# tobixdev/rdf-fusion

Hardware: AMD Instinct MI355X
Metric: solution bindings/sec + achieved HBM GB/s, BSBM Q5 at 1/2/4/8 GPUs (higher is better)
Workload: dtype u32 ids / i64 typed values; 1 GPU; BSBM-shaped store, 285000 products (98101452 triples), Explore Q5 (7 triple patterns -> scans, hash joins, FILTERs), 262144 instances per step, batched into one operator tree (shared scans); steady state: the join tables of the predicate slices are cached per store version (cold start and the no-cache step are under config.cold_start); mode=batched, triples_per_gpu=98100423, exchange_overlapped_with_next_step=False, bindings=56629082633

## Files before the change

include/rdfgpu.h:

```cpp
#ifndef RDFGPU_H
#define RDFGPU_H

#include <stddef.h>
#include <stdint.h>

#ifdef __cplusplus
extern "C" {
#endif

#define RDFGPU_ABI_VERSION 4u

typedef enum rdfgpu_status {
  RDFGPU_OK = 0,
  RDFGPU_END = 1,
  RDFGPU_ERR_INVALID = -1,
  RDFGPU_ERR_DEVICE = -2,
  RDFGPU_ERR_UNSUPPORTED = -3,
  RDFGPU_ERR_OOM = -4,
  RDFGPU_ERR_NO_DEVICE = -5
} rdfgpu_status;

const char* rdfgpu_last_error(void);
uint32_t rdfgpu_abi_version(void);

// ... 237 lines not shown
  uint32_t n_regexes;
  uint32_t reserved;
} rdfgpu_plan_desc;
#define RDFGPU_PLAN_ALLOW_OPAQUE 1u
#define RDFGPU_PLAN_AGG_COLUMNS 2u
#define RDFGPU_PLAN_VALUE_KEYS 4u

typedef struct rdfgpu_plan rdfgpu_plan;

typedef struct rdfgpu_metrics {
  uint64_t output_rows;
  uint64_t input_rows;
  uint64_t intermediate_rows;
  uint64_t device_bytes;
  double elapsed_compute_ms;
  uint32_t kernels_launched;
  uint32_t host_syncs;
  uint32_t exact_reruns;
  uint32_t device_mallocs;
  double device_malloc_ms;
  uint32_t tables_built;
  uint32_t reserved;
} rdfgpu_metrics;

int rdfgpu_plan_compile(rdfgpu_store* store, const rdfgpu_plan_desc* desc, rdfgpu_plan** out);
void rdfgpu_plan_destroy(rdfgpu_plan* plan);

int rdfgpu_plan_bind_table(rdfgpu_plan* plan, uint32_t slot, const uint32_t* const* cols,
                           uint32_t n_cols, uint64_t n_rows);

int rdfgpu_plan_execute(rdfgpu_plan* plan);

int rdfgpu_plan_result_info(rdfgpu_plan* plan, uint64_t* n_rows, uint32_t* n_cols);
int rdfgpu_plan_result_device(rdfgpu_plan* plan, const uint32_t** cols, uint32_t cap_cols);
int rdfgpu_plan_fetch(rdfgpu_plan* plan, uint32_t* const* host_cols, uint32_t n_cols);
typedef struct rdfgpu_agg_value {
  int64_t lo;
  int64_t hi;
  uint8_t tag;
  uint8_t reserved[7];
} rdfgpu_agg_value;
int rdfgpu_plan_agg_count(rdfgpu_plan* plan, uint32_t* n_aggs);
int rdfgpu_plan_agg_fetch(rdfgpu_plan* plan, uint32_t agg, rdfgpu_agg_value* host);
int rdfgpu_plan_agg_device(rdfgpu_plan* plan, uint32_t agg, const rdfgpu_agg_value** values);
int rdfgpu_plan_result_values(rdfgpu_plan* plan, uint32_t col, const rdfgpu_agg_value** values, uint64_t* n);
int rdfgpu_plan_result_values_fetch(rdfgpu_plan* plan, uint32_t col, rdfgpu_agg_value* host);
int rdfgpu_plan_next(rdfgpu_plan* plan, struct ArrowArray* out, struct ArrowSchema* schema);
int rdfgpu_plan_rewind(rdfgpu_plan* plan);
int rdfgpu_plan_metrics(rdfgpu_plan* plan, rdfgpu_metrics* out);
int rdfgpu_plan_selected_index(const rdfgpu_plan* plan, uint32_t node, uint32_t* components);
int rdfgpu_plan_stream(rdfgpu_plan* plan, void** hip_stream);
int rdfgpu_plan_decode_terms(rdfgpu_plan* plan, uint32_t col, uint64_t first_row, uint64_t n_rows,
                             struct ArrowArray* out, struct ArrowSchema* schema);

enum { RDFGPU_PUSH_UNSUPPORTED = 0,
       RDFGPU_PUSH_TRUE = 1,
       RDFGPU_PUSH_BINARY = 2,
       RDFGPU_PUSH_BETWEEN = 3 };
typedef struct rdfgpu_pushdown_filter {
  uint32_t kind;
  uint32_t var;
  uint32_t op;
  uint32_t value;
  uint32_t from, to;
} rdfgpu_pushdown_filter;
int rdfgpu_plan_pushdown_filters(rdfgpu_plan* plan, uint32_t node, const rdfgpu_pushdown_filter* filters, uint32_t n, uint8_t* pushed);
// ... 19 lines not shown
  RDFGPU_OPT_NO_FIRST_RUN_SPECULATION,
  RDFGPU_OPT_NO_STRING_VERDICTS,
  RDFGPU_OPT_NO_TABLE_CACHE,
  RDFGPU_OPT_NO_INDEX_JOIN,
  RDFGPU_OPT_NO_CHAIN_FUSION,
  RDFGPU_OPT_NO_VALUE_TABLES,
  RDFGPU_OPT_NO_RANGE_INDEX,
  RDFGPU_OPT_NO_FILTER_FUSION,
  RDFGPU_OPT_NO_LDS_JOIN,
  RDFGPU_OPT_NO_GLOBAL_TABLE_JOIN,
  RDFGPU_OPT_NO_DIRECT_TABLE,
  RDFGPU_OPT_NO_BAND_JOIN,
  RDFGPU_OPT_NO_PARTITIONED_JOIN,
  RDFGPU_OPT_NO_VALUE_VERDICTS,
  RDFGPU_OPT_NO_PRIMING,
  RDFGPU_OPT_NO_ORDERED_JOIN,
  RDFGPU_OPT_NO_BAND_PACK16,
  RDFGPU_OPT_NO_RUN_COPY,
  RDFGPU_OPT_NO_RANGE_PARTITION,
  RDFGPU_OPT_LDS_MAX_BUILD,
  RDFGPU_OPT_CSR_ROW_LANES_LOG2,
  RDFGPU_OPT_JOIN_WAVE_Q,
  RDFGPU_OPT_PARTITION_MIN_BUILD,
  RDFGPU_OPT_PARTITION_TWO_PASS_ROWS,
  RDFGPU_OPT_NO_OWN_PARTITION_PASS,
  RDFGPU_OPT_NO_BAND_COMPACT,
  RDFGPU_OPT_NO_PROBE_OUTER_JOIN,
  RDFGPU_OPT_NO_STREAM_JOIN,
  RDFGPU_OPT_PARTITION_ROWS,
  RDFGPU_OPT_PARTITION_SLOTS,
  RDFGPU_OPT_NO_SEMI_LDS,
  RDFGPU_OPT_NO_BAND_PAIR_COUNTS,
  RDFGPU_OPT_BAND_PAIR_COUNT_BLOCKS,
  RDFGPU_OPT_NO_BAND_ROW_CACHE,
  RDFGPU_OPT_NO_BAND_PAIR_LIST,
  RDFGPU_OPT_NO_BAND_PAIR_CACHE,
  RDFGPU_OPT_BAND_PAIR_CACHE_BLOCKS,
  RDFGPU_OPT_NO_AGG_LDS,
  RDFGPU_OPT__COUNT
};
int rdfgpu_store_set_option(rdfgpu_store* store, uint32_t option, uint64_t value);
int rdfgpu_store_get_option(const rdfgpu_store* store, uint32_t option, uint64_t* value);
int rdfgpu_plan_set_option(rdfgpu_plan* plan, uint32_t option, uint64_t value);
const char* rdfgpu_option_name(uint32_t option);

uint64_t rdfgpu_scan_score(const rdfgpu_scan_instruction instr[4]);
uint32_t rdfgpu_choose_index(const rdfgpu_scan_instruction gspo[4], uint32_t available);
int rdfgpu_band_row_cache_eligible(uint32_t in_place, uint32_t compact, uint32_t pack16, uint32_t option_set, uint32_t n_win,
                                   const uint32_t operand_src[4], const uint32_t operand_keyed_by_join_key[4]);
int rdfgpu_band_pair_cache_eligible(uint32_t row_windows, uint32_t neq_self, uint32_t pack16, uint32_t option_set, uint64_t n_blocks, uint64_t cap_blocks);
int rdfgpu_band_pair_list_eligible(uint32_t pair_cached, uint32_t option_set, uint64_t survivors, uint64_t n_blocks);
int rdfgpu_band_pair_count_eligible(uint32_t has_list, uint32_t option_set, uint64_t n_blocks, uint64_t min_blocks);
int rdfgpu_band_step_form(uint32_t row_static, uint32_t has_verdicts, uint32_t has_list, uint32_t list_option_set, uint32_t counts_option_set,
                          uint32_t n_row_cols, uint64_t n_blocks, uint64_t min_blocks);
int rdfgpu_oj_probe_form(uint32_t held, uint32_t in_place, uint32_t row_cache, uint32_t option_set, uint32_t row_static);
typedef struct rdfgpu_predicate {
  uint32_t pred;
  uint32_t from, to;
  const uint32_t* ids;
  uint32_t n_ids;
  uint32_t equal_to;
} rdfgpu_predicate;
int rdfgpu_predicate_and(const rdfgpu_predicate* lhs, const rdfgpu_predicate* rhs,
                         rdfgpu_predicate* out, uint32_t* out_ids);
enum { RDFGPU_OP_EQ = 0, RDFGPU_OP_GT = 1, RDFGPU_OP_GTEQ = 2, RDFGPU_OP_LT = 3, RDFGPU_OP_LTEQ = 4 };
int rdfgpu_pushdown_to_scan_predicate(uint32_t op, uint32_t value, rdfgpu_predicate* out);

int rdfgpu_regex_check(const char* pattern, uint32_t pattern_len, const char* flags, uint32_t flags_len, uint32_t* positions);

typedef struct rdfgpu_comm rdfgpu_comm;
#define RDFGPU_COMM_ID_BYTES 128
int rdfgpu_comm_unique_id(uint8_t id[RDFGPU_COMM_ID_BYTES]);
int rdfgpu_comm_create(const uint8_t id[RDFGPU_COMM_ID_BYTES], uint32_t rank, uint32_t world, int32_t device, rdfgpu_comm** out);
typedef int (*rdfgpu_host_alltoallv_fn)(void* ctx, const void* send, const uint64_t* send_bytes, void* recv, const uint64_t* recv_bytes);
int rdfgpu_comm_create_host(uint32_t rank, uint32_t world, int32_t device, rdfgpu_host_alltoallv_fn fn, void* ctx, rdfgpu_comm** out);
void rdfgpu_comm_destroy(rdfgpu_comm* comm);
int rdfgpu_exchange_allgatherv(rdfgpu_comm* comm, const uint32_t* const* cols, uint32_t n_cols, uint64_t n_rows,
                               const uint32_t** out_cols, uint64_t* out_rows);
int rdfgpu_exchange_repartition(rdfgpu_comm* comm, const uint32_t* const* cols, uint32_t n_cols, uint64_t n_rows, uint32_t key_col,
                                const uint32_t** out_cols, uint64_t* out_rows);
uint32_t rdfgpu_shard_of(uint32_t id, uint32_t world);

typedef struct rdfgpu_ntriples rdfgpu_ntriples;
int rdfgpu_ntriples_parse(int32_t device, const char* text, uint64_t text_bytes, uint32_t first_id, rdfgpu_ntriples** out);
int rdfgpu_ntriples_info(const rdfgpu_ntriples* nt, uint64_t* n_triples, uint32_t* n_terms, uint64_t* term_bytes);
int rdfgpu_ntriples_terms(const rdfgpu_ntriples* nt, uint64_t* offsets, uint8_t* bytes);
int rdfgpu_ntriples_decoded_info(const rdfgpu_ntriples* nt, uint64_t* lex_bytes, uint64_t* suffix_bytes);
int rdfgpu_ntriples_decoded(const rdfgpu_ntriples* nt, uint8_t* kind, uint64_t* lex_off, uint8_t* lex_bytes, uint64_t* suffix_off,
// ... 9 lines not shown
```

rdf-fusion_amd/__init__.py:

```python
from . import abi, plan
from .engine import (RdfGpuError, GpuQuadStore, GpuPlan, Comm, NTriples, load_library, library_path, kernel_source_sha16,
                     choose_index, scan_score, predicate_and, pushdown_to_scan_predicate, shard_of, band_row_cache_eligible,
                     band_pair_cache_eligible, band_pair_list_eligible, band_pair_count_eligible, band_step_form, BAND_FORMS, oj_probe_form, OJ_PROBE_FORMS)

__all__ = ["abi", "plan", "RdfGpuError", "GpuQuadStore", "GpuPlan", "Comm", "NTriples", "shard_of", "load_library", "library_path", "kernel_source_sha16",
           "choose_index", "scan_score", "predicate_and", "pushdown_to_scan_predicate", "band_row_cache_eligible", "band_pair_cache_eligible", "band_pair_list_eligible", "band_pair_count_eligible", "band_step_form", "BAND_FORMS", "oj_probe_form", "OJ_PROBE_FORMS"]
```

rdf-fusion_amd/abi.py:

```python
import ctypes as C

ABI_VERSION = 4

OK, END = 0, 1
ERR_INVALID, ERR_DEVICE, ERR_UNSUPPORTED, ERR_OOM, ERR_NO_DEVICE = -1, -2, -3, -4, -5

GSPO, GPOS, GOSP = 0, 1, 2
INDEX_NAMES = {GSPO: "GSPO", GPOS: "GPOS", GOSP: "GOSP"}

TRAVERSE, SCAN = 0, 1
PRED_NONE, PRED_FALSE, PRED_IN, PRED_BETWEEN, PRED_EQUAL_TO = 0, 1, 2, 3, 4

(TV_NULL, TV_NAMED_NODE, TV_BLANK_NODE, TV_STRING, TV_BOOLEAN, TV_FLOAT, TV_DOUBLE, TV_DECIMAL,
 TV_INT, TV_INTEGER, TV_DATE_TIME, TV_TIME, TV_DATE, TV_DURATION, TV_OTHER) = range(15)
TVF_EMPTY_STRING = 1
TVF_NEEDS_HOST = 0x80
NT_IRI, NT_BNODE, NT_SIMPLE, NT_LANG, NT_TYPED = 1, 2, 3, 4, 5

(EX_COLUMN, EX_LIT_ID, EX_LIT_TV, EX_ENC_TV, EX_GT, EX_LT, EX_GEQ, EX_LEQ, EX_EQ, EX_ADD, EX_SUB,
 EX_EBV, EX_ID_EQ, EX_ID_NEQ, EX_AND, EX_OR, EX_NOT, EX_IS_COMPATIBLE, EX_BOUND, EX_BOOL_AS_TV,
 EX_LIT_BOOL, EX_NEQ, EX_REGEX, EX_CONTAINS, EX_STRSTARTS, EX_STRENDS, EX_LANG_IN, EX_REGEX_VAR,
 EX_STR, EX_LIT_STR, EX_STRLEN, EX_SUBSTR, EX_UCASE, EX_LCASE, EX_STRBEFORE, EX_STRAFTER,
 EX_MUL, EX_DIV, EX_NEG, EX_PLUS, EX_ABS, EX_ROUND, EX_CEIL, EX_FLOOR, EX_CAST, EX_CAST_STRING, EX_CAST_LEX,
 EX_YEAR, EX_MONTH, EX_DAY, EX_HOURS, EX_MINUTES, EX_SECONDS) = range(1, 54)
# ... 2 lines not shown
CAST_TARGETS = (TV_BOOLEAN, TV_INT, TV_INTEGER, TV_DECIMAL, TV_FLOAT, TV_DOUBLE)

(NODE_DATA_SOURCE, NODE_FILTER, NODE_HASH_JOIN, NODE_CROSS_JOIN, NODE_NESTED_LOOP_JOIN,
 NODE_PROJECTION, NODE_TABLE, NODE_TOPK, NODE_UNION, NODE_CLOSURE, NODE_AGGREGATE) = range(1, 12)
NODE_SORT = 13
NODE_EXTEND = 12
(AGG_COUNT_STAR, AGG_COUNT, AGG_COUNT_DISTINCT, AGG_SUM, AGG_AVG, AGG_MIN, AGG_MAX, AGG_SAMPLE, AGG_GROUP_CONCAT,
 AGG_SUM_DISTINCT, AGG_AVG_DISTINCT, AGG_COUNT_DISTINCT_STAR) = range(1, 13)
AGG_NAMES = {AGG_COUNT_STAR: "COUNT(*)", AGG_COUNT: "COUNT", AGG_COUNT_DISTINCT: "COUNT(DISTINCT)", AGG_SUM: "SUM", AGG_AVG: "AVG",
             AGG_MIN: "MIN", AGG_MAX: "MAX", AGG_SAMPLE: "SAMPLE", AGG_GROUP_CONCAT: "GROUP_CONCAT", AGG_SUM_DISTINCT: "SUM(DISTINCT)",
             AGG_AVG_DISTINCT: "AVG(DISTINCT)", AGG_COUNT_DISTINCT_STAR: "COUNT(DISTINCT *)"}
MAX_AGGREGATES = 8
AGG_INPUT_EXPR = 0x80000000
SORT_BY_ID, SORT_BY_TERM, SORT_BY_DOUBLE = 0, 1, 2
SORT_BY_VALUE = 3
SORT_DESC = 0x100
JOIN_INNER, JOIN_LEFT, JOIN_LEFT_SEMI, JOIN_LEFT_ANTI = 0, 1, 2, 3
JOIN_LEFT_MARK = 4
MAX_KEYS = 4
MAX_GROUP_KEYS = 8
MAX_COLUMNS = 16
NO_PROJECTION = 0xFFFFFFFF
PLAN_ALLOW_OPAQUE = 1
PLAN_AGG_COLUMNS = 2

PLAN_VALUE_KEYS = 4

OP_EQ, OP_GT, OP_GTEQ, OP_LT, OP_LTEQ = range(5)

OPTION_NAMES = ["FORCE_GENERIC_VM", "NO_JOIN_REORDER", "NO_SPECULATION", "NO_FIRST_RUN_SPECULATION", "NO_STRING_VERDICTS",
                "NO_TABLE_CACHE", "NO_INDEX_JOIN", "NO_CHAIN_FUSION", "NO_VALUE_TABLES", "NO_RANGE_INDEX", "NO_FILTER_FUSION",
                "NO_LDS_JOIN", "NO_GLOBAL_TABLE_JOIN", "NO_DIRECT_TABLE", "NO_BAND_JOIN", "NO_PARTITIONED_JOIN", "NO_VALUE_VERDICTS", "NO_PRIMING", "NO_ORDERED_JOIN", "NO_BAND_PACK16", "NO_RUN_COPY", "NO_RANGE_PARTITION",
                "LDS_MAX_BUILD", "CSR_ROW_LANES_LOG2", "JOIN_WAVE_Q", "PARTITION_MIN_BUILD", "PARTITION_TWO_PASS_ROWS", "NO_OWN_PARTITION_PASS", "NO_BAND_COMPACT", "NO_PROBE_OUTER_JOIN", "NO_STREAM_JOIN", "PARTITION_ROWS", "PARTITION_SLOTS",
                "NO_SEMI_LDS", "NO_BAND_PAIR_COUNTS", "BAND_PAIR_COUNT_BLOCKS", "NO_BAND_ROW_CACHE", "NO_BAND_PAIR_LIST", "NO_BAND_PAIR_CACHE", "BAND_PAIR_CACHE_BLOCKS", "NO_AGG_LDS"]
OPTIONS = {name: i for i, name in enumerate(OPTION_NAMES)}


class Config(C.Structure):
    _fields_ = [("device", C.c_int32), ("batch_size", C.c_uint32), ("flags", C.c_uint32),
                ("reserved", C.c_uint32)]


class TypedValue(C.Structure):
    _fields_ = [("lo", C.c_int64), ("aux", C.c_uint32), ("tag", C.c_uint8), ("flags", C.c_uint8),
                ("tz_minutes", C.c_int16)]


class AggValue(C.Structure):
    _fields_ = [("lo", C.c_int64), ("hi", C.c_int64), ("tag", C.c_uint8), ("reserved", C.c_uint8 * 7)]


class ScanInstruction(C.Structure):
    _fields_ = [("kind", C.c_uint8), ("pred", C.c_uint8), ("reserved", C.c_uint16),
                ("var", C.c_uint32), ("a", C.c_uint32), ("b", C.c_uint32)]


class ExprNode(C.Structure):
    _fields_ = [("op", C.c_uint8), ("tag", C.c_uint8), ("flags", C.c_uint8), ("reserved", C.c_uint8),
                ("u", C.c_uint32), ("lo", C.c_int64), ("hi", C.c_int64)]


class PlanNode(C.Structure):
    _fields_ = [("kind", C.c_uint32), ("left", C.c_int32), ("right", C.c_int32),
                ("join_type", C.c_uint32), ("scan", ScanInstruction * 4), ("n_keys", C.c_uint32),
                ("left_keys", C.c_uint32 * MAX_KEYS), ("right_keys", C.c_uint32 * MAX_KEYS),
                ("expr_off", C.c_uint32), ("expr_len", C.c_uint32), ("proj_off", C.c_uint32),
                ("n_proj", C.c_uint32), ("table_slot", C.c_uint32), ("table_cols", C.c_uint32)]
# ... 46 lines not shown
    ("n_children", C.c_int64), ("children", C.POINTER(C.POINTER(ArrowSchema))),
    ("dictionary", C.POINTER(ArrowSchema)), ("release", C.c_void_p), ("private_data", C.c_void_p)]


class ArrowArray(C.Structure):
    pass


ArrowArray._fields_ = [
    ("length", C.c_int64), ("null_count", C.c_int64), ("offset", C.c_int64), ("n_buffers", C.c_int64),
    ("n_children", C.c_int64), ("buffers", C.POINTER(C.c_void_p)),
    ("children", C.POINTER(C.POINTER(ArrowArray))), ("dictionary", C.POINTER(ArrowArray)),
    ("release", C.c_void_p), ("private_data", C.c_void_p)]

assert C.sizeof(TypedValue) == 16
assert C.sizeof(ScanInstruction) == 16
assert C.sizeof(ExprNode) == 24
assert C.sizeof(AggValue) == 24

EXPORTED_SYMBOLS = [
    "rdfgpu_last_error", "rdfgpu_abi_version",
    "rdfgpu_store_create", "rdfgpu_store_destroy", "rdfgpu_store_extend", "rdfgpu_store_extend_device",
    "rdfgpu_store_remove", "rdfgpu_store_clear", "rdfgpu_store_drop_tables", "rdfgpu_store_remove_graph", "rdfgpu_store_len", "rdfgpu_store_set_typed_values", "rdfgpu_store_set_strings",
    "rdfgpu_store_read_index",
    "rdfgpu_plan_compile", "rdfgpu_plan_destroy", "rdfgpu_plan_bind_table", "rdfgpu_plan_execute",
    "rdfgpu_plan_result_info", "rdfgpu_plan_result_device", "rdfgpu_plan_fetch", "rdfgpu_plan_next",
    "rdfgpu_plan_agg_count", "rdfgpu_plan_agg_fetch", "rdfgpu_plan_agg_device",
    "rdfgpu_plan_result_values", "rdfgpu_plan_result_values_fetch",
    "rdfgpu_plan_rewind", "rdfgpu_plan_decode_terms", "rdfgpu_ntriples_parse", "rdfgpu_ntriples_info", "rdfgpu_ntriples_terms", "rdfgpu_ntriples_decoded_info", "rdfgpu_ntriples_decoded", "rdfgpu_ntriples_columns", "rdfgpu_ntriples_destroy", "rdfgpu_plan_metrics", "rdfgpu_plan_selected_index", "rdfgpu_plan_stream",
    "rdfgpu_plan_enable_kernel_timing", "rdfgpu_plan_kernel_stats",
    "rdfgpu_plan_pushdown_filters", "rdfgpu_plan_set_dynamic_filters", "rdfgpu_plan_source_predicate",
    "rdfgpu_store_set_option", "rdfgpu_store_get_option", "rdfgpu_plan_set_option", "rdfgpu_option_name",
    "rdfgpu_scan_score", "rdfgpu_choose_index", "rdfgpu_predicate_and", "rdfgpu_band_row_cache_eligible", "rdfgpu_band_pair_cache_eligible", "rdfgpu_band_pair_list_eligible", "rdfgpu_band_pair_count_eligible", "rdfgpu_band_step_form", "rdfgpu_oj_probe_form",
    "rdfgpu_pushdown_to_scan_predicate", "rdfgpu_regex_check",
    "rdfgpu_comm_unique_id", "rdfgpu_comm_create", "rdfgpu_comm_create_host", "rdfgpu_comm_destroy",
    "rdfgpu_exchange_allgatherv", "rdfgpu_exchange_repartition", "rdfgpu_shard_of",
]
COMM_ID_BYTES = 128
HOST_ALLTOALLV_FN = C.CFUNCTYPE(C.c_int, C.c_void_p, C.c_void_p, C.POINTER(C.c_uint64), C.c_void_p, C.POINTER(C.c_uint64))
```

rdf-fusion_amd/csrc/abi.cpp:

```cpp
#include <cstdlib>
#include <cstring>
#include <mutex>
#include <shared_mutex>
#include <string>

#include "exchange.hpp"
#include "host_logic.hpp"
#include "ntriples.hpp"
#include "plan.hpp"
#include "regex_compile.hpp"
#include "store.hpp"

namespace rdfgpu {
static thread_local std::string g_last_error;
void set_last_error(const std::string& msg) { g_last_error = msg; }
}

using namespace rdfgpu;

#define ABI_BEGIN try {
#define ABI_END                                              \
  }                                                          \
  catch (const Error& e) { set_last_error(e.what()); return e.status; } \
  catch (const std::bad_alloc&) { set_last_error("host allocation failed"); return RDFGPU_ERR_OOM; } \
// ... 101 lines not shown
  P(plan)->opt.v[option] = value;
  ABI_END
}
const char* rdfgpu_option_name(uint32_t option) { return engine_option_name(option); }

int rdfgpu_plan_compile(rdfgpu_store* store, const rdfgpu_plan_desc* desc, rdfgpu_plan** out) {
  ABI_BEGIN
  if (!out) fail(RDFGPU_ERR_INVALID, "null out pointer");
  *out = reinterpret_cast<rdfgpu_plan*>(plan_compile(S(store), desc));
  ABI_END
}
void rdfgpu_plan_destroy(rdfgpu_plan* plan) { delete reinterpret_cast<Plan*>(plan); }

int rdfgpu_plan_bind_table(rdfgpu_plan* plan, uint32_t slot, const uint32_t* const* cols, uint32_t n_cols, uint64_t n_rows) {
  ABI_BEGIN
  Plan* p = P(plan);
  if (slot >= p->tables.size()) fail(RDFGPU_ERR_INVALID, "plan has no table slot %u", slot);
  if (n_cols && !cols) fail(RDFGPU_ERR_INVALID, "null column array");
  BoundTable& b = p->tables[slot];
  b.cols.assign(cols, cols + n_cols);
  b.n_rows = n_rows; b.bound = true;
  ABI_END
}
int rdfgpu_plan_execute(rdfgpu_plan* plan) { ABI_BEGIN P(plan)->execute(); ABI_END }

int rdfgpu_plan_result_info(rdfgpu_plan* plan, uint64_t* n_rows, uint32_t* n_cols) {
  ABI_BEGIN
  Plan* p = P(plan);
  if (!p->executed) fail(RDFGPU_ERR_INVALID, "plan has not been executed");
  if (n_rows) *n_rows = p->result_rows;
  if (n_cols) *n_cols = p->result.n_cols;
  ABI_END
}
int rdfgpu_plan_result_device(rdfgpu_plan* plan, const uint32_t** cols, uint32_t cap_cols) {
  ABI_BEGIN
  Plan* p = P(plan);
  if (!p->executed) fail(RDFGPU_ERR_INVALID, "plan has not been executed");
  if (cap_cols < p->result.n_cols) fail(RDFGPU_ERR_INVALID, "room for %u columns, result has %u", cap_cols, p->result.n_cols);
  for (u32 c = 0; c < p->result.n_cols; c++) cols[c] = p->result_rows ? p->result.cols[c] : nullptr;
  ABI_END
}
int rdfgpu_plan_fetch(rdfgpu_plan* plan, uint32_t* const* host_cols, uint32_t n_cols) {
  ABI_BEGIN
  Plan* p = P(plan);
  if (!p->executed) fail(RDFGPU_ERR_INVALID, "plan has not been executed");
  if (n_cols != p->result.n_cols) fail(RDFGPU_ERR_INVALID, "caller passed %u columns, result has %u", n_cols, p->result.n_cols);
  p->store->activate();
  for (u32 c = 0; c < n_cols; c++)
    if (p->result_rows) RDFGPU_HIP(hipMemcpyAsync(host_cols[c], p->result.cols[c], p->result_rows * 4, hipMemcpyDeviceToHost, p->stream));
  RDFGPU_HIP(hipStreamSynchronize(p->stream));
  ABI_END
}

int rdfgpu_plan_agg_count(rdfgpu_plan* plan, uint32_t* n_aggs) {
  ABI_BEGIN
  Plan* p = P(plan);
  if (!p->executed) fail(RDFGPU_ERR_INVALID, "plan has not been executed");
  if (n_aggs) *n_aggs = (uint32_t)p->agg_out.size();
  ABI_END
}
int rdfgpu_plan_agg_fetch(rdfgpu_plan* plan, uint32_t agg, rdfgpu_agg_value* host) {
  ABI_BEGIN
  Plan* p = P(plan);
  if (!p->executed) fail(RDFGPU_ERR_INVALID, "plan has not been executed");
  if (agg >= p->agg_out.size()) fail(RDFGPU_ERR_INVALID, "aggregate %u of %zu", agg, p->agg_out.size());
  p->store->activate();
  if (p->result_rows) {
    if (!host) fail(RDFGPU_ERR_INVALID, "null host buffer");
    RDFGPU_HIP(hipMemcpyAsync(host, p->agg_out[agg], p->result_rows * sizeof(rdfgpu_agg_value), hipMemcpyDeviceToHost, p->stream));
  }
  RDFGPU_HIP(hipStreamSynchronize(p->stream));
  ABI_END
}
int rdfgpu_plan_result_values(rdfgpu_plan* plan, uint32_t col, const rdfgpu_agg_value** values, uint64_t* n) {
  ABI_BEGIN
  Plan* p = P(plan);
  if (!p->executed) fail(RDFGPU_ERR_INVALID, "plan has not been executed");
  if (col >= p->result.n_cols) fail(RDFGPU_ERR_INVALID, "column %u of a %u-column result", col, p->result.n_cols);
  if (!values) fail(RDFGPU_ERR_INVALID, "null out pointer");
  *values = p->result_values(col, n);
  ABI_END
}
int rdfgpu_plan_result_values_fetch(rdfgpu_plan* plan, uint32_t col, rdfgpu_agg_value* host) {
  ABI_BEGIN
  Plan* p = P(plan);
  if (!p->executed) fail(RDFGPU_ERR_INVALID, "plan has not been executed");
  if (col >= p->result.n_cols) fail(RDFGPU_ERR_INVALID, "column %u of a %u-column result", col, p->result.n_cols);
  if (!p->result_values(col, nullptr)) fail(RDFGPU_ERR_INVALID, "result column %u holds object ids, not aggregate values", col);
  p->ensure_host_copy();
  if (p->result_rows) {
    if (!host) fail(RDFGPU_ERR_INVALID, "null host buffer");
    std::memcpy(host, p->host_values[col].data(), p->result_rows * sizeof(rdfgpu_agg_value));
  }
  ABI_END
}
int rdfgpu_plan_agg_device(rdfgpu_plan* plan, uint32_t agg, const rdfgpu_agg_value** values) {
  ABI_BEGIN
  Plan* p = P(plan);
  if (!p->executed) fail(RDFGPU_ERR_INVALID, "plan has not been executed");
  if (agg >= p->agg_out.size()) fail(RDFGPU_ERR_INVALID, "aggregate %u of %zu", agg, p->agg_out.size());
  if (!values) fail(RDFGPU_ERR_INVALID, "null out pointer");
  *values = p->result_rows ? p->agg_out[agg] : nullptr;
  ABI_END
}

namespace {
struct ChildPriv { void* buffers[3] = {nullptr, nullptr, nullptr}; };
void release_child_array(struct ArrowArray* a) {
  if (!a || !a->release) return;
  ChildPriv* pr = static_cast<ChildPriv*>(a->private_data);
  std::free(pr->buffers[0]); std::free(pr->buffers[1]); std::free(pr->buffers[2]);
  delete pr;
  a->release = nullptr;
}
struct StructPriv { const void* buffers[1]; struct ArrowArray** children; u32 n; };
void release_struct_array(struct ArrowArray* a);
void release_agg_array(struct ArrowArray* a) {
  if (!a || !a->release) return;
  std::free(const_cast<void*>(static_cast<StructPriv*>(a->private_data)->buffers[0]));
  static_cast<StructPriv*>(a->private_data)->buffers[0] = nullptr;
  release_struct_array(a);
}
void release_struct_array(struct ArrowArray* a) {
  if (!a || !a->release) return;
  StructPriv* pr = static_cast<StructPriv*>(a->private_data);
  for (u32 i = 0; i < pr->n; i++) { if (pr->children[i]->release) pr->children[i]->release(pr->children[i]); delete pr->children[i]; }
  delete[] pr->children;
  delete pr;
  a->release = nullptr;
}
struct SchemaPriv { struct ArrowSchema** children; u32 n; std::string* names; };
void release_schema(struct ArrowSchema* s) {
// ... 92 lines not shown
      ch->release = release_child_array; ch->private_data = cp;
      sp->children[c] = ch;
    }
    std::memset(out, 0, sizeof *out);
    out->length = (int64_t)len; out->n_buffers = 1; out->buffers = sp->buffers;
    out->n_children = nc; out->children = sp->children;
    out->release = release_struct_array; out->private_data = sp;
    if (schema) {
      std::memset(schema, 0, sizeof *schema);
      SchemaPriv* pr = new SchemaPriv();
      pr->n = nc; pr->children = new ArrowSchema*[nc ? nc : 1]; pr->names = new std::string[nc ? nc : 1];
      for (u32 c = 0; c < nc; c++) {
        pr->names[c] = "c" + std::to_string(c);
        if (c >= nk || p->result_values(c, nullptr)) { pr->children[c] = agg_schema(pr->names[c].c_str()); continue; }
        ArrowSchema* cs = new ArrowSchema();
        std::memset(cs, 0, sizeof *cs);
        cs->format = "I"; cs->name = pr->names[c].c_str(); cs->flags = 2 ;
        cs->release = release_schema; cs->private_data = nullptr;
        pr->children[c] = cs;
      }
      schema->format = "+s"; schema->name = ""; schema->n_children = nc; schema->children = pr->children;
      schema->release = release_schema; schema->private_data = pr;
    }
    p->cursor += len;
    return RDFGPU_OK;
  } catch (const Error& e) { set_last_error(e.what()); return e.status; }
  catch (const std::exception& e) { set_last_error(e.what()); return RDFGPU_ERR_INVALID; }
}
int rdfgpu_plan_decode_terms(rdfgpu_plan* plan, uint32_t col, uint64_t first_row, uint64_t n_rows, struct ArrowArray* out, struct ArrowSchema* schema) {
  try {
    Plan* p = P(plan);
    if (!out) fail(RDFGPU_ERR_INVALID, "null out array");
    if (!p->executed) fail(RDFGPU_ERR_INVALID, "plan has not been executed");
    if (col >= p->result.n_cols) fail(RDFGPU_ERR_INVALID, "column %u of a %u-column result", col, p->result.n_cols);
    if (const ValueOrigin& o = p->nodes[p->root].origin[col]; o.node >= 0)
      fail(RDFGPU_ERR_UNSUPPORTED, "ENC_PT of result column %u: it is %s value column (%s %u of node %d), its entries are not object ids (rdfgpu_plan_result_values)", col, o.mark ? "a mark" : o.extend ? "a computed" : "an aggregate", o.mark ? "mark" : o.extend ? "expression" : "aggregate", o.agg, o.node);
    if (first_row > p->result_rows || n_rows > p->result_rows - first_row) fail(RDFGPU_ERR_INVALID, "rows %llu .. + %llu of a %llu-row result", (unsigned long long)first_row, (unsigned long long)n_rows, (unsigned long long)p->result_rows);
    Store* st = p->store;
    st->activate();
    std::shared_lock<std::shared_mutex> lock(st->mu);
    if (!st->str_off) fail(RDFGPU_ERR_INVALID, "ENC_PT needs the lexical forms (rdfgpu_store_set_strings)");
    const u64 n = n_rows;
    hipStream_t s = p->stream;
    DevicePool& pool = st->pool;
    std::vector<void*> dev;
    auto dalloc = [&](size_t bytes) { void* q = pool.alloc(bytes ? bytes : 4); dev.push_back(q); return q; };
    struct Guard { DevicePool& pool; std::vector<void*>& v; ~Guard() { for (void* q : v) pool.free(q); } } guard{pool, dev};
    DecodeArgs a{};
    a.ids = p->result.cols[col] + first_row; a.n = n; a.tt = st->typed_table();
    u32* len = static_cast<u32*>(dalloc((n + 1) * 4)); u32* off = static_cast<u32*>(dalloc((n + 1) * 4));
    a.len = len; a.off = off;
    a.term_type = static_cast<unsigned char*>(dalloc(n)); a.tag = static_cast<unsigned char*>(dalloc(n)); a.aux = static_cast<u32*>(dalloc(n * 4));
    RDFGPU_HIP(hipMemsetAsync(len + n, 0, 4, s));
    launch_decode_lengths(a, s);
    std::vector<u32> h_len(n + 1);
    RDFGPU_HIP(hipMemcpyAsync(h_len.data(), len, (n + 1) * 4, hipMemcpyDeviceToHost, s));
    RDFGPU_HIP(hipStreamSynchronize(s));
    u64 total = 0;
    for (u64 i = 0; i < n; i++) total += h_len[i];
    if (total > 0x7FFFFFFFull) fail(RDFGPU_ERR_UNSUPPORTED, "ENC_PT: %llu bytes of lexical forms in one call (utf8 offsets are int32): decode fewer rows", (unsigned long long)total);
    const size_t tb = scan_temp_bytes(n + 1);
    void* temp = dalloc(tb);
    exclusive_scan_u32(len, off, n + 1, temp, tb, s);
    a.bytes = static_cast<unsigned char*>(dalloc(total));
    launch_decode_bytes(a, s);
    auto halloc = [](size_t bytes) { void* q = std::malloc(bytes ? bytes : 1); if (!q) fail(RDFGPU_ERR_OOM, "host allocation of %zu bytes failed", bytes); return q; };
// ... 24 lines not shown
      return ch;
    };
    sp->children[0] = child(h_tt, nullptr, 2);
    sp->children[1] = child(h_off, h_bytes, 3);
    sp->children[2] = child(h_tag, nullptr, 2);
    sp->children[3] = child(h_aux, nullptr, 2);
    static_cast<ChildPriv*>(sp->children[0]->private_data)->buffers[2] = valid;
    sp->buffers[0] = nulls ? valid : nullptr;
    std::memset(out, 0, sizeof *out);
    out->length = (int64_t)n; out->null_count = nulls; out->n_buffers = 1; out->buffers = sp->buffers;
    out->n_children = 4; out->children = sp->children;
    out->release = release_struct_array; out->private_data = sp;
    if (schema) {
      std::memset(schema, 0, sizeof *schema);
      SchemaPriv* pr = new SchemaPriv();
      pr->n = 4; pr->children = new ArrowSchema*[4]; pr->names = new std::string[4];
      const char* names[4] = {"term_type", "value", "tag", "aux"};
      const char* formats[4] = {"C", "u", "C", "I"};
      for (u32 c = 0; c < 4; c++) {
        ArrowSchema* cs = new ArrowSchema();
        std::memset(cs, 0, sizeof *cs);
        pr->names[c] = names[c];
        cs->format = formats[c]; cs->name = pr->names[c].c_str(); cs->flags = 0;
        cs->release = release_schema; cs->private_data = nullptr;
        pr->children[c] = cs;
      }
      schema->format = "+s"; schema->name = ""; schema->flags = 2 ; schema->n_children = 4; schema->children = pr->children;
      schema->release = release_schema; schema->private_data = pr;
    }
    return RDFGPU_OK;
  } catch (const Error& e) { set_last_error(e.what()); return e.status; }
  catch (const std::exception& e) { set_last_error(e.what()); return RDFGPU_ERR_INVALID; }
}
int rdfgpu_plan_rewind(rdfgpu_plan* plan) { ABI_BEGIN P(plan)->cursor = 0; ABI_END }
int rdfgpu_plan_metrics(rdfgpu_plan* plan, rdfgpu_metrics* out) {
  ABI_BEGIN
  if (!out) fail(RDFGPU_ERR_INVALID, "null out pointer");
  *out = P(plan)->metrics;
  ABI_END
}
int rdfgpu_plan_selected_index(const rdfgpu_plan* plan, uint32_t node, uint32_t* components) {
  ABI_BEGIN
  const Plan* p = reinterpret_cast<const Plan*>(plan);
  if (!p) fail(RDFGPU_ERR_INVALID, "null plan handle");
  if (node >= p->nodes.size() || p->nodes[node].source < 0) fail(RDFGPU_ERR_INVALID, "node %u is not a data source", node);
  if (components) *components = p->sources[p->nodes[node].source].components;
  ABI_END
}
int rdfgpu_plan_pushdown_filters(rdfgpu_plan* plan, uint32_t node, const rdfgpu_pushdown_filter* filters, uint32_t n, uint8_t* pushed) {
  ABI_BEGIN
  if (n && !filters) fail(RDFGPU_ERR_INVALID, "null filter array");
  P(plan)->pushdown_filters(node, filters, n, pushed);
  ABI_END
}
int rdfgpu_plan_set_dynamic_filters(rdfgpu_plan* plan, uint32_t node, const rdfgpu_pushdown_filter* filters, uint32_t n) {
  ABI_BEGIN
  if (n && !filters) fail(RDFGPU_ERR_INVALID, "null filter array");
  P(plan)->set_dynamic_filters(node, filters, n);
  ABI_END
}
int rdfgpu_plan_source_predicate(const rdfgpu_plan* plan, uint32_t node, uint32_t level, rdfgpu_predicate* pred) {
  ABI_BEGIN
  const Plan* p = reinterpret_cast<const Plan*>(plan);
  if (!p || !pred) fail(RDFGPU_ERR_INVALID, "null pointer");
  if (node >= p->nodes.size() || p->nodes[node].source < 0 || level > 3) fail(RDFGPU_ERR_INVALID, "node %u level %u is not a data-source level", node, level);
  const SourceInfo& src = p->sources[p->nodes[node].source];
  ScanPredicate sp;
  for (int k = 0; k < 4; k++) if ((u32)PERM[src.components][k] == level) sp = src.ix.in[k].pred;
  std::memset(pred, 0, sizeof *pred);
  pred->pred = sp.kind; pred->from = sp.from; pred->to = sp.to; pred->equal_to = sp.equal_to;
  if (sp.kind == RDFGPU_PRED_IN) { pred->n_ids = (u32)sp.ids.size(); if (sp.ids.size() == 1) pred->from = pred->to = sp.ids[0]; }
  ABI_END
}
int rdfgpu_plan_stream(rdfgpu_plan* plan, void** hip_stream) {
  ABI_BEGIN
  if (!hip_stream) fail(RDFGPU_ERR_INVALID, "null out pointer");
  *hip_stream = P(plan)->stream;
  ABI_END
}

int rdfgpu_plan_enable_kernel_timing(rdfgpu_plan* plan, int on) {
  ABI_BEGIN
  Plan* p = P(plan);
  p->timing = on != 0;
  p->timing_focus = on >= 2 ? p->last_top_kc : -1;
  ABI_END
}
int rdfgpu_plan_kernel_stats(rdfgpu_plan* plan, rdfgpu_kernel_stat* out, uint32_t cap, uint32_t* n) {
  ABI_BEGIN
  Plan* p = P(plan);
  if (!n || (cap && !out)) fail(RDFGPU_ERR_INVALID, "null out pointer");
  u32 w = 0;
  for (int k = 0; k < KC__N; k++) {
    const KernelStat& s = p->kstats[k];
    if (!s.launches) continue;
    if (w < cap) { out[w].kernel = kernel_class_name(k); out[w].launches = s.launches; out[w].reserved = 0; out[w].total_ms = s.ms; out[w].algorithmic_bytes = s.bytes; out[w].rows_in = s.rows; }
    w++;
  }
  *n = w < cap ? w : cap;
  ABI_END
}

static void decode4(const rdfgpu_scan_instruction raw[4], ScanInstruction out[4]) {
  for (int i = 0; i < 4; i++) {
    rdfgpu_scan_instruction r = raw[i];
    if (r.pred == RDFGPU_PRED_IN) {
      out[i].kind = r.kind; out[i].var = r.var; out[i].pred.kind = RDFGPU_PRED_IN;
      out[i].pred.ids.clear();
      for (u32 q = 0; q < (r.b ? r.b : 1); q++) out[i].pred.ids.push_back(q);
    } else out[i] = decode_instruction(r, nullptr, 0);
  }
}
uint64_t rdfgpu_scan_score(const rdfgpu_scan_instruction instr[4]) {
  try { ScanInstruction in[4]; decode4(instr, in); return scan_score(in); }
  catch (const std::exception& e) { set_last_error(e.what()); return 0; }
}
uint32_t rdfgpu_choose_index(const rdfgpu_scan_instruction gspo[4], uint32_t available) {
  try {
    ScanInstructions g; g.components = RDFGPU_GSPO; decode4(gspo, g.in);
    return choose_index(g, available);
  } catch (const std::exception& e) { set_last_error(e.what()); return 0xFFFFFFFFu; }
}
int rdfgpu_band_row_cache_eligible(uint32_t in_place, uint32_t compact, uint32_t pack16, uint32_t option_set, uint32_t n_win,
// ... 5 lines not shown
    for (u32 w = 0; w < n_win; w++) {
      s.y0[w] = BandRowOperandShape{operand_src[2 * w], operand_keyed_by_join_key[2 * w] != 0};
      s.y1[w] = BandRowOperandShape{operand_src[2 * w + 1], operand_keyed_by_join_key[2 * w + 1] != 0};
    }
    return band_row_cache_eligible(s) ? 1 : 0;
  } catch (const Error& e) { set_last_error(e.what()); return e.status; }
}
int rdfgpu_band_pair_cache_eligible(uint32_t row_windows, uint32_t neq_self, uint32_t pack16, uint32_t option_set, uint64_t n_blocks, uint64_t cap_blocks) {
  BandPairCacheShape s;
  s.row_windows = row_windows != 0; s.neq_self = neq_self != 0; s.pack16 = pack16 != 0; s.option_off = option_set == 0; s.n_blocks = n_blocks; s.cap = cap_blocks;
  return band_pair_cache_eligible(s) ? 1 : 0;
}
int rdfgpu_band_pair_list_eligible(uint32_t pair_cached, uint32_t option_set, uint64_t survivors, uint64_t n_blocks) {
  BandPairListShape s;
  s.pair_cached = pair_cached != 0; s.option_off = option_set == 0; s.survivors = survivors; s.n_blocks = n_blocks;
  return band_pair_list_eligible(s) ? 1 : 0;
}
int rdfgpu_band_pair_count_eligible(uint32_t has_list, uint32_t option_set, uint64_t n_blocks, uint64_t min_blocks) {
  BandPairCountShape s;
  s.has_list = has_list != 0; s.option_off = option_set == 0; s.n_blocks = n_blocks; s.min_blocks = min_blocks;
  return band_pair_count_eligible(s) ? 1 : 0;
}
int rdfgpu_band_step_form(uint32_t row_static, uint32_t has_verdicts, uint32_t has_list, uint32_t list_option_set, uint32_t counts_option_set,
                          uint32_t n_row_cols, uint64_t n_blocks, uint64_t min_blocks) {
  BandStepShape s;
  s.row_static = row_static != 0; s.has_verdicts = has_verdicts != 0; s.has_list = has_list != 0; s.list_option_off = list_option_set == 0;
  s.counts_option_off = counts_option_set == 0; s.n_row_cols = n_row_cols; s.n_blocks = n_blocks; s.min_blocks = min_blocks;
  return (int)band_step_form(s);
}
int rdfgpu_oj_probe_form(uint32_t held, uint32_t in_place, uint32_t row_cache, uint32_t option_set, uint32_t row_static) {
  OjProbeShape s;
  s.held = held != 0; s.in_place = in_place != 0; s.row_cache = row_cache != 0; s.option_off = option_set == 0; s.row_static = row_static != 0;
  return (int)oj_probe_form(s);
}
static ScanPredicate from_abi(const rdfgpu_predicate* p) {
  ScanPredicate r; r.kind = p->pred; r.from = p->from; r.to = p->to; r.equal_to = p->equal_to;
  if (p->pred == RDFGPU_PRED_IN) { if (p->ids) r.ids.assign(p->ids, p->ids + p->n_ids); else r.ids = {p->from}; }
  return r;
}
int rdfgpu_predicate_and(const rdfgpu_predicate* lhs, const rdfgpu_predicate* rhs, rdfgpu_predicate* out, uint32_t* out_ids) {
  try {
    if (!lhs || !rhs || !out) fail(RDFGPU_ERR_INVALID, "null predicate");
    ScanPredicate r;
    if (!predicate_and(from_abi(lhs), from_abi(rhs), &r)) return 0;
    std::memset(out, 0, sizeof *out);
    out->pred = r.kind; out->from = r.from; out->to = r.to;
    if (r.kind == RDFGPU_PRED_IN) {
      if (!out_ids) fail(RDFGPU_ERR_INVALID, "null out_ids");
      for (size_t i = 0; i < r.ids.size(); i++) out_ids[i] = r.ids[i];
      out->ids = out_ids; out->n_ids = (u32)r.ids.size();
    }
    return 1;
  } catch (const Error& e) { set_last_error(e.what()); return e.status; }
}
int rdfgpu_pushdown_to_scan_predicate(uint32_t op, uint32_t value, rdfgpu_predicate* out) {
  try {
    if (!out) fail(RDFGPU_ERR_INVALID, "null out predicate");
    const ScanPredicate r = pushdown_to_scan_predicate(op, value);
    std::memset(out, 0, sizeof *out);
    out->pred = r.kind; out->from = r.from; out->to = r.to;
    if (r.kind == RDFGPU_PRED_IN) { out->from = out->to = r.ids[0]; out->n_ids = 1; }
    return 1;
  } catch (const Error& e) { set_last_error(e.what()); return e.status; }
}

static Comm* CM(rdfgpu_comm* c) { if (!c) fail(RDFGPU_ERR_INVALID, "null communicator"); return reinterpret_cast<Comm*>(c); }
// ... 95 lines not shown
```

rdf-fusion_amd/csrc/band_join.hip:

```cpp
#include <hip/hip_runtime.h>
#include <cstring>
#include <rocprim/rocprim.hpp>

#include "join_device.hpp"

namespace rdfgpu {

static inline dim3 grid256(u64 n) { const u64 g = (n + 255) / 256; return dim3((unsigned)(g ? g : 1)); }
constexpr u32 kBandInvalidLo = 0xFFFFFFFFu;

__global__ __launch_bounds__(256) void band_bounds_kernel(const u32* skey_sorted, u64 n, u32 kn, u32* poff) {
  const u64 i = (u64)blockIdx.x * blockDim.x + threadIdx.x;
  if (i > n) return;
  const u32 prev = i > 0 ? skey_sorted[i - 1] + 1u : 0u;
  const u32 cur = i < n ? skey_sorted[i] : kn;
  for (u32 k = prev; k <= cur && k <= kn; k++) poff[k] = (u32)i;
}

__device__ __forceinline__ bool band_window_of(const TypedTable& tt, const BandWin& w, u32 iy0, u32 iy1, long long& lo, long long& hi) {
  lo = INT64_MIN + 1; hi = INT64_MAX;
  if (tt.n_ids == 0 || iy0 == 0 || iy1 == 0 || iy0 >= tt.n_ids || iy1 >= tt.n_ids) return false;
  if (w.l0.tag != RDFGPU_TV_INTEGER || w.l1.tag != RDFGPU_TV_INTEGER) return false;
  const int4* tv = reinterpret_cast<const int4*>(tt.tv);
  const int4 r0 = tv[iy0];
// ... 863 lines not shown
    case 6: hipLaunchKernelGGL((band_emit_kernel<FORM, 6>), g, dim3(256), 0, s, b); return true;
  }
  return false;
}
static bool launch_band_emit_list(const BandArgs& b, dim3 g, hipStream_t s) {
  constexpr BandForm L = BandForm::VERDICTS_LIST;
  switch (b.n_out_cols * 2 + b.n_row_cols) {
    case 3: hipLaunchKernelGGL((band_emit_kernel<L, 1, 1>), g, dim3(256), 0, s, b); return true;
    case 5: hipLaunchKernelGGL((band_emit_kernel<L, 2, 2>), g, dim3(256), 0, s, b); return true;
    case 7: hipLaunchKernelGGL((band_emit_kernel<L, 3, 3>), g, dim3(256), 0, s, b); return true;
    case 9: hipLaunchKernelGGL((band_emit_kernel<L, 4, 4>), g, dim3(256), 0, s, b); return true;
    case 11: hipLaunchKernelGGL((band_emit_kernel<L, 5, 5>), g, dim3(256), 0, s, b); return true;
    case 2: hipLaunchKernelGGL((band_emit_kernel<L, 1, 2>), g, dim3(256), 0, s, b); return true;
    case 4: hipLaunchKernelGGL((band_emit_kernel<L, 2, 3>), g, dim3(256), 0, s, b); return true;
    case 6: hipLaunchKernelGGL((band_emit_kernel<L, 3, 4>), g, dim3(256), 0, s, b); return true;
    case 8: hipLaunchKernelGGL((band_emit_kernel<L, 4, 5>), g, dim3(256), 0, s, b); return true;
  }
  return false;
}
void launch_band_emit(const BandArgs& b, BandForm form, hipStream_t s) {
  band_form_check(b, form);
  const dim3 g = grid_waves(b.launch_blocks);
  bool launched = false;
  switch (form) {
    case BandForm::RECORDS: launched = launch_band_emit_cols<BandForm::RECORDS>(b, g, s); break;
    case BandForm::ROW_WINDOWS: launched = launch_band_emit_cols<BandForm::ROW_WINDOWS>(b, g, s); break;
    case BandForm::VERDICTS: launched = launch_band_emit_cols<BandForm::VERDICTS>(b, g, s); break;
    case BandForm::VERDICTS_LIST: case BandForm::COUNTS_LIST:
      launched = launch_band_emit_list(b, grid_waves((b.max_blocks + kBandEmitGroup - 1) / kBandEmitGroup), s); break;
  }
  if (!launched) fail(RDFGPU_ERR_INVALID, "band join: form %s with %u output columns (%u from the row)", band_form_name(form), b.n_out_cols, b.n_row_cols);
}

struct BandBlocksOfKey {
  const u32* csr_off; const u32* poff; u32 kn;
  __host__ __device__ u32 operator()(u32 k) const {
    if (k >= kn) return 0u;
    const u32 e = csr_off[k + 1] - csr_off[k], r = poff[k + 1] - poff[k];
    return (e && r) ? ((e + 63) >> 6) * ((r + 63) >> 6) : 0u;
  }
  __device__ __forceinline__ uint4 group(u32 g, u32 n) const {
    const u32 k = 4u * g;
    if (k + 4u <= kn && !((reinterpret_cast<uintptr_t>(csr_off) | reinterpret_cast<uintptr_t>(poff)) & 15u)) {
      const uint4 c = reinterpret_cast<const uint4*>(csr_off)[g], p = reinterpret_cast<const uint4*>(poff)[g];
      const u32 c4 = csr_off[k + 4u], p4 = poff[k + 4u];
      auto blocks = [](u32 e, u32 r) { return (e && r) ? ((e + 63u) >> 6) * ((r + 63u) >> 6) : 0u; };
      return make_uint4(blocks(c.y - c.x, p.y - p.x), blocks(c.z - c.y, p.z - p.y), blocks(c.w - c.z, p.w - p.z), blocks(c4 - c.w, p4 - p.w));
    }
    return make_uint4(k < n ? (*this)(k) : 0u, k + 1u < n ? (*this)(k + 1u) : 0u, k + 2u < n ? (*this)(k + 2u) : 0u, k + 3u < n ? (*this)(k + 3u) : 0u);
  }
};
size_t band_blocks_scan_temp_bytes(u32 kn) {
  size_t bytes = 0;
  auto in = rocprim::make_transform_iterator(rocprim::make_counting_iterator<u32>(0u), BandBlocksOfKey{nullptr, nullptr, kn});
  (void)rocprim::exclusive_scan(nullptr, bytes, in, (u32*)nullptr, 0u, (size_t)kn + 1, rocprim::plus<u32>());
  return bytes + 256;
}
void band_blocks_scan(const u32* csr_off, const u32* poff, u32 kn, u32* boff, void* temp, size_t temp_bytes, hipStream_t s) {
  if (launch_small_scan<false>(BandBlocksOfKey{csr_off, poff, kn}, boff, (u64)kn + 1, s)) return;
  auto in = rocprim::make_transform_iterator(rocprim::make_counting_iterator<u32>(0u), BandBlocksOfKey{csr_off, poff, kn});
  RDFGPU_HIP(rocprim::exclusive_scan(temp, temp_bytes, in, boff, 0u, (size_t)kn + 1, rocprim::plus<u32>(), s));
}

size_t sort_u32_temp_bytes(u64 n, u32 bits) {
  size_t bytes = 0;
  (void)rocprim::radix_sort_pairs(nullptr, bytes, (const u32*)nullptr, (u32*)nullptr, (const u32*)nullptr, (u32*)nullptr, (size_t)(n ? n : 1), 0, bits);
// ... 37 lines not shown
```

rdf-fusion_amd/csrc/host_logic.cpp:

```cpp
#include "host_logic.hpp"

#include <algorithm>

namespace rdfgpu {

ScanInstruction decode_instruction(const rdfgpu_scan_instruction& raw, const u32* pool, u32 n_pool) {
  ScanInstruction out;
  if (raw.kind != RDFGPU_TRAVERSE && raw.kind != RDFGPU_SCAN) fail(RDFGPU_ERR_INVALID, "scan instruction: bad kind %u", raw.kind);
  out.kind = raw.kind;
  out.var = raw.var;
  out.pred.kind = raw.pred;
  switch (raw.pred) {
    case RDFGPU_PRED_NONE: case RDFGPU_PRED_FALSE: break;
    case RDFGPU_PRED_IN:
      if (raw.b == 0) fail(RDFGPU_ERR_INVALID, "scan instruction: empty In set");
      if ((u64)raw.a + raw.b > n_pool) fail(RDFGPU_ERR_INVALID, "scan instruction: In set outside the pool");
      out.pred.ids.assign(pool + raw.a, pool + raw.a + raw.b);
      std::sort(out.pred.ids.begin(), out.pred.ids.end());
      out.pred.ids.erase(std::unique(out.pred.ids.begin(), out.pred.ids.end()), out.pred.ids.end());
      break;
    case RDFGPU_PRED_BETWEEN: out.pred.from = raw.a; out.pred.to = raw.b; break;
    case RDFGPU_PRED_EQUAL_TO: out.pred.equal_to = raw.a; break;
    default: fail(RDFGPU_ERR_INVALID, "scan instruction: bad predicate %u", raw.pred);
  }
// ... 126 lines not shown
      if (op->src < 2 || !op->stage_keyed_by_join_key) return false;
  return true;
}

bool band_pair_cache_eligible(const BandPairCacheShape& s) {
  if (!s.row_windows || !s.neq_self || !s.pack16 || !s.option_off) return false;
  return s.n_blocks <= (s.cap ? s.cap : kBandPairCacheBlocks);
}

bool band_pair_list_eligible(const BandPairListShape& s) {
  if (!s.pair_cached || !s.option_off || s.n_blocks >= kBandPairListBlocks) return false;
  return s.survivors <= 256 * s.n_blocks;
}

bool band_pair_count_eligible(const BandPairCountShape& s) {
  if (!s.has_list || !s.option_off) return false;
  return s.n_blocks >= (s.min_blocks ? s.min_blocks : kBandPairCountBlocks);
}

BandForm band_step_form(const BandStepShape& s) {
  if (!s.row_static) return BandForm::RECORDS;
  if (!s.has_verdicts) return BandForm::ROW_WINDOWS;
  if (!s.has_list || !s.list_option_off || s.n_row_cols > 1) return BandForm::VERDICTS;
  BandPairCountShape c;
  c.has_list = true; c.option_off = s.counts_option_off; c.n_blocks = s.n_blocks; c.min_blocks = s.min_blocks;
  return band_pair_count_eligible(c) ? BandForm::COUNTS_LIST : BandForm::VERDICTS_LIST;
}

OjProbeForm oj_probe_form(const OjProbeShape& s) {
  if (!s.held || !s.in_place || !s.row_cache || !s.option_off) return OjProbeForm::FULL;
  return s.row_static ? OjProbeForm::LEAN : OjProbeForm::FULL_NOW;
}

}
```

rdf-fusion_amd/csrc/host_logic.hpp:

```cpp
#pragma once
#include <vector>

#include "common.hpp"

namespace rdfgpu {

struct ScanPredicate {
  u32 kind = RDFGPU_PRED_NONE;
  std::vector<u32> ids;
  u32 from = 0, to = 0;
  u32 equal_to = 0;
};
struct ScanInstruction {
  u32 kind = RDFGPU_TRAVERSE;
  u32 var = 0;
  ScanPredicate pred;
};
struct ScanInstructions {
  u32 components = RDFGPU_GSPO;
  ScanInstruction in[4];
};

ScanInstruction decode_instruction(const rdfgpu_scan_instruction& raw, const u32* pool, u32 n_pool);
ScanInstructions make_gspo(const rdfgpu_scan_instruction raw[4], const u32* pool, u32 n_pool);
// ... 11 lines not shown
PrunePlan plan_pruning(const ScanInstructions& ix);

struct BandRowOperandShape { u32 src = 0; bool stage_keyed_by_join_key = false; };
struct BandRowCacheShape {
  bool in_place = false, compact = false, pack16 = false, option_off = false;
  u32 n_win = 0; BandRowOperandShape y0[2], y1[2];
};
bool band_row_cache_eligible(const BandRowCacheShape& s);
constexpr u64 kBandPairCacheBlocks = 1ull << 21;
struct BandPairCacheShape { bool row_windows = false, neq_self = false, pack16 = false, option_off = false; u64 n_blocks = 0, cap = 0; };
bool band_pair_cache_eligible(const BandPairCacheShape& s);
constexpr u64 kBandPairListBlocks = 1ull << 20;
struct BandPairListShape { bool pair_cached = false, option_off = false; u64 survivors = 0, n_blocks = 0; };
bool band_pair_list_eligible(const BandPairListShape& s);
constexpr u64 kBandPairCountBlocks = 1ull << 16;
struct BandPairCountShape { bool has_list = false, option_off = false; u64 n_blocks = 0, min_blocks = 0; };
bool band_pair_count_eligible(const BandPairCountShape& s);

enum class BandForm : u32 { RECORDS, ROW_WINDOWS, VERDICTS, VERDICTS_LIST, COUNTS_LIST };
constexpr const char* band_form_name(BandForm f) {
  return f == BandForm::RECORDS ? "RECORDS" : f == BandForm::ROW_WINDOWS ? "ROW_WINDOWS" : f == BandForm::VERDICTS ? "VERDICTS" : f == BandForm::VERDICTS_LIST ? "VERDICTS_LIST" : "COUNTS_LIST";
}
struct BandStepShape {
  bool row_static = false, has_verdicts = false, has_list = false, list_option_off = false, counts_option_off = false;
  u32 n_row_cols = 0; u64 n_blocks = 0, min_blocks = 0;
};
BandForm band_step_form(const BandStepShape& s);

enum class OjProbeForm : u32 { FULL, LEAN, FULL_NOW };
constexpr const char* oj_probe_form_name(OjProbeForm f) { return f == OjProbeForm::FULL ? "FULL" : f == OjProbeForm::LEAN ? "LEAN" : "FULL_NOW"; }
struct OjProbeShape { bool held = false, in_place = false, row_cache = false, option_off = false, row_static = false; };
OjProbeForm oj_probe_form(const OjProbeShape& s);

}
```

rdf-fusion_amd/csrc/kernels.hpp:

```cpp
#pragma once
#include <functional>
#include "common.hpp"
#include "expr_device.hpp"
#include "host_logic.hpp"

namespace rdfgpu {

constexpr u32 kNil = 0xFFFFFFFFu;
constexpr int kMaxCols = RDFGPU_MAX_COLUMNS;

struct DevTable {
  u32 n_cols = 0;
  const u32* cols[kMaxCols] = {};
  u64 cap = 0;
  const u64* n_dev = nullptr;
  u64 stable_id = 0;
  int sorted_col = -1;
  u32 key_min = 0, key_max = 0;
};

struct LocateJob {
  const u32* col[4];
  u64 n;
  u32 n_levels;
// ... 424 lines not shown
  ColRef entry_col[kBandMaxSideCols]; const u32* row_col[kBandMaxSideCols];
  u8 out_from_row[kMaxCols];
  u8 out_sel[kMaxCols];
  const uint2* row_win; const u32* row_val;
  u64* bvalid;
  const unsigned short* pair_list; const u32* pair_list_off;
  const unsigned char* pair_cnt;
};
struct BandPairListArgs { const u64* bits; u32 n_blocks; u32* counts; const u32* off; unsigned short* list; u64 cap; u32* total_out; unsigned char* pair_cnt; };
void launch_band_pair_list_count(const BandPairListArgs& a, hipStream_t s);
void launch_band_pair_list_write(const BandPairListArgs& a, hipStream_t s);
struct BandRowOperand { const u32* direct; u32 kmin, kn; const u32* val; };
struct BandRowWinArgs {
  BandRowOperand y0[2], y1[2];
  u32 kmin, kn; uint2* by_key;
  u32* slow_keys;
  const u32* build_key; u64 n_rows; uint2* row_win;
};
void launch_band_row_win_keys(const BandArgs& b, const BandRowWinArgs& w, hipStream_t s);
void launch_band_row_win_rows(const BandRowWinArgs& w, hipStream_t s);
void launch_band_pair_bits(const BandArgs& b, hipStream_t s);
void launch_band_pt(const BandArgs& b, hipStream_t s);
void launch_band_entries(const BandArgs& b, hipStream_t s);
void launch_band_rows(const BandArgs& b, hipStream_t s);
void launch_band_scatter(const BandArgs& b, hipStream_t s);
void launch_band_desc(const BandArgs& b, hipStream_t s);
void launch_band_decode(const BandArgs& b, hipStream_t s);
void launch_band_bounds(const u32* skey_sorted, u64 n, u32 kn, u32* poff, hipStream_t s);
size_t band_blocks_scan_temp_bytes(u32 kn);
void band_blocks_scan(const u32* csr_off, const u32* poff, u32 kn, u32* boff, void* temp, size_t temp_bytes, hipStream_t s);
void launch_band_mask(const BandArgs& b, BandForm form, hipStream_t s);
void launch_band_slow(const LdsJoinArgs* a_dev, const BandArgs& b, hipStream_t s);
void launch_band_emit(const BandArgs& b, BandForm form, hipStream_t s);
size_t sort_u32_temp_bytes(u64 n, u32 bits);
void sort_pairs_u32_u32(const u32* kin, u32* kout, const u32* vin, u32* vout, u64 n, u32 bits, void* temp, size_t temp_bytes, hipStream_t s);
void launch_val_minmax(const long long* val, u64 n, long long* out_minmax , hipStream_t s);
void launch_csr_max_group(const u32* off, u32 kn, u32* out_dev , hipStream_t s);
void launch_gjoin_build(const LdsJoinArgs& a, hipStream_t s);
int lds_join_items(u64 n_probe_cap, bool global);
enum { kJoinTableLds = 0, kJoinTableHash = 1, kJoinTableDirect = 2, kJoinTableCsr = 3 };
int lds_join_mode(const LdsJoinArgs& a);
void launch_minmax_u32(const u32* col, u64 n, u32* out_dev , hipStream_t s);
void launch_direct_values(const u32* keys, const u32* valcol, u64 n, u32 kmin, u32 kn, const TypedTable& tt, long long* val, u32* bad_dev, hipStream_t s);
void launch_fill_i64(long long* p, long long v, u64 n, hipStream_t s);
void launch_range_minmax(const u32* stage_key_col, const u32* csr_rows, u64 n, const long long* val, u32 vmin_key, u32 vn, long long* out_minmax , hipStream_t s);
void launch_range_keys(const u32* group_col, u32 gmin, const u32* stage_key_col, const u32* csr_rows, u64 n, const long long* val, u32 vmin_key, u32 vn,
                       long long vbase, u64* key64, u32* rows_in, hipStream_t s);
void launch_range_decode(const u64* key64_sorted, u64 n, u32* biased_vals_out, hipStream_t s);
void launch_gdirect_build(const u32* keys, u64 n, u32* direct , u32 kmin, u32 kn, u32* dup_dev, hipStream_t s);

struct TopkArgs {
  const u32* in[kMaxCols];
  const u64* n_in_dev; u64 n_in_cap;
  u32 has_group, group_col;
  u32 n_keys, key_col[4], key_by_term[4];
  u32 k, n_groups;
  TypedTable tt;
  u32* counts;
  u32* offsets;
  u32* cursor;
  u32* perm;
  u32* picked;
  u32* out_counts;
  u32* out_offsets;
  u32* out[kMaxCols]; u32 n_out_cols; u32 proj[kMaxCols];
  u64* n_out_dev;
// ... 50 lines not shown
```

rdf-fusion_amd/csrc/plan.cpp:

```cpp
#include "plan_exec.hpp"

#include <functional>

namespace rdfgpu {

void Plan::derive_source(SourceInfo& src, const ScanInstructions& gspo) {
  src.components = choose_index(gspo, 0b111);
  src.ix = reorder(gspo, src.components);
  src.prune = plan_pruning(src.ix);
  src.n_out = 0; src.has_residual = false;
  for (int k = 0; k < 4; k++) {
    if (gspo.in[k].kind != RDFGPU_SCAN) continue;
    bool first = true;
    for (int j = 0; j < k; j++) if (gspo.in[j].kind == RDFGPU_SCAN && gspo.in[j].var == gspo.in[k].var) first = false;
    if (!first) continue;
    for (int lvl = 0; lvl < 4; lvl++)
      if (src.ix.in[lvl].kind == RDFGPU_SCAN && src.ix.in[lvl].var == gspo.in[k].var) src.out_level[src.n_out] = lvl;
    src.n_out++;
  }
  for (int k = 0; k < 4; k++)
    if (src.ix.in[k].pred.kind != RDFGPU_PRED_NONE && !(src.prune.dropped_mask & (1u << k))) src.has_residual = true;
}
void Plan::upload_pool() {
  pool.clear();
// ... 43 lines not shown
    const bool yes = filters[i].kind != RDFGPU_PUSH_UNSUPPORTED;
    if (pushed) pushed[i] = yes ? 1 : 0;
    if (!yes) continue;
    any = true;
    ScanPredicate p;
    if (filter_to_predicate(filters[i], &p)) and_into_instructions(gspo, filters[i].var, p);
  }
  if (!any) return;
  src.gspo = gspo;
  derive_source(src, src.gspo);
  src.dynamic_dirty = !src.dynamic.empty();
  upload_pool();
  located_version = ~0ull;
  for (NodeInfo& nd : nodes) { nd.has_last = false; nd.last_rows = 0; }
}

void Plan::set_dynamic_filters(u32 node, const rdfgpu_pushdown_filter* filters, u32 n) {
  if (node >= nodes.size() || nodes[node].source < 0) fail(RDFGPU_ERR_INVALID, "node %u is not a data source", node);
  SourceInfo& src = sources[nodes[node].source];
  std::vector<std::pair<u32, ScanPredicate>> dyn;
  for (u32 i = 0; i < n; i++) {
    if (filters[i].kind == RDFGPU_PUSH_UNSUPPORTED) continue;
    ScanPredicate p;
    if (filter_to_predicate(filters[i], &p)) dyn.emplace_back(filters[i].var, p);
  }
  ScanInstructions probe = src.gspo;
  for (auto& d : dyn) and_into_instructions(probe, d.first, d.second);
  src.dynamic = dyn;
  src.dynamic_dirty = true;
}

Plan::~Plan() {
  if (store) (void)hipSetDevice(store->device);
  if (stream) (void)hipStreamSynchronize(stream);
  release_intermediates();
  if (pool_dev) (void)hipFree(pool_dev);
  if (regex_dev) (void)hipFree(regex_dev);
  if (str_consts_dev) (void)hipFree(str_consts_dev);
  if (mark_values_dev) (void)hipFree(mark_values_dev);

  if (store && ctx) store->release_context(ctx);
  if (store) store->release();
}

const char* kernel_class_name(int kc) {
  static const char* const fixed[KC_LDS_JOIN0] = {
      "rdfgpu::locate_kernel", "rdfgpu::scan_count_kernel", "rdfgpu::scan_write_kernel",
      "void rdfgpu::filter_kernel<1>", "void rdfgpu::filter_kernel<2>", "void rdfgpu::filter_kernel<0>",
      "rdfgpu::cross_kernel", "rdfgpu::join_build_kernel", "void rdfgpu::join_probe_kernel<false>",
      "void rdfgpu::join_probe_kernel<true>", "rdfgpu::join_left_unmatched_kernel", "void rdfgpu::nlj_kernel<false>",
      "void rdfgpu::nlj_kernel<true>", "rocprim device scan", "rdfgpu::gjoin_build_kernel", "rdfgpu::gdirect_build_kernel",
      "rdfgpu::minmax_u32_kernel", "rdfgpu::csr_rel_keys_kernel", "rocprim radix sort (CSR rows)",
      "rdfgpu::topk_max_kernel", "rdfgpu::topk_hist_kernel", "rdfgpu::topk_scatter_kernel", "rdfgpu::topk_select_kernel",
      "rdfgpu::topk_write_kernel", "void rdfgpu::filter_kernel<3>", "rdfgpu::regex_verdict_kernel", "rdfgpu::union_kernel",
      "rdfgpu::band_slow_kernel", "rocprim radix sort", "rdfgpu::band_bounds_kernel", "rdfgpu::band_blocks_kernel",
      "rdfgpu::band_decode_kernel", "void rdfgpu::band_mask_kernel", "void rdfgpu::band_emit_kernel", "rdfgpu::band_entries_kernel",
      "rdfgpu::band_desc_kernel", "rdfgpu::band_pt_kernel", "rdfgpu::band_rows_kernel",
      "void rdfgpu::filter_bits_kernel<1>", "void rdfgpu::filter_bits_kernel<2>", "void rdfgpu::filter_bits_kernel<3>", "void rdfgpu::filter_bits_kernel<4>", "rdfgpu::value_verdict_kernel",
      "rdfgpu::value_runs_kernel", "void rdfgpu::run_scan_kernel", "rdfgpu::run_copy_kernel",
      "rdfgpu::oj_probe_kernel", "rdfgpu::oj_count_kernel", "void rdfgpu::oj_write_kernel",
      "void rdfgpu::filter_write_kernel", "rdfgpu::part_keys_kernel", "void rdfgpu::part_join_kernel",
      "rdfgpu::oj_band_records_kernel", "rdfgpu::oj_write_band_kernel", "void rdfgpu::small_scan_kernel",
      "rdfgpu::part_pass (hist + scan + scatter)", "void rdfgpu::stream_join_kernel",
      "rdfgpu::oj_write_band_kernel(rdfgpu::OrderedJoinArgs, rdfgpu::OjBandFuse, rdfgpu::OjInPlace)", "void rdfgpu::semi_build_kernel",
      "void rdfgpu::semi_join_kernel<0, false", "void rdfgpu::semi_join_kernel<0, true", "void rdfgpu::semi_join_kernel<1, false",
      "void rdfgpu::semi_join_kernel<1, true", "void rdfgpu::semi_nested_kernel<false", "void rdfgpu::semi_nested_kernel<true",
      "rdfgpu::agg_groups_kernel", "void rdfgpu::agg_accum_kernel<false>", "void rdfgpu::agg_accum_kernel<true>", "rdfgpu::agg_final_kernel",
// ... 18 lines not shown
                                                       items[w] + ", " + std::to_string(m) + ", " + (c ? "true" : "false");
  });
  return names[kc - KC_LDS_JOIN0].c_str();
}

void Plan::resolve_timing() {
  for (KernelStat& k : kstats) k = KernelStat{};
  if (!timing) return;
  auto live = [&](const u64* dev, u64 fallback) -> u64 {
    if (!dev) return fallback;
    const u64 v = ctx->counters_host[dev - counters];
    return v < fallback || fallback == 0 ? v : fallback;
  };
  for (const PendingLaunch& p : pending) {
    float ms = 0;
    RDFGPU_HIP(hipEventElapsedTime(&ms, p.start, p.stop));
    KernelStat& k = kstats[p.kc];
    const u64 rows = live(p.rows_dev, p.rows_cap);
    const u64 out = p.out_dev ? ctx->counters_host[p.out_dev - counters] : p.out_rows;
    k.launches++; k.ms += ms; k.rows += rows;
    k.bytes += p.fixed_bytes + rows * p.bytes_per_row + out * p.bytes_per_out;
  }
  pending.clear();
  if (timing_focus < 0) {
    double top = 0;
    for (int kc = 0; kc < (int)(sizeof kstats / sizeof kstats[0]); kc++) if (kstats[kc].ms > top) { top = kstats[kc].ms; last_top_kc = kc; }
  }
}

void Plan::release_intermediates() {
  for (void* p : allocs) store->pool.free(p);
  allocs.clear();
}
const ExprProgram* Plan::upload_program(const ExprProgram& p) {
  if (progs_used >= ExecContext::kProgSlots) fail(RDFGPU_ERR_UNSUPPORTED, "plan needs more than %u device expression programs", ExecContext::kProgSlots);
  const u32 slot = progs_used++;
  ctx->progs_host[slot] = p;
  bind_values(ctx->progs_host[slot]);
  RDFGPU_HIP(hipMemcpyAsync(ctx->progs_dev + slot, ctx->progs_host + slot, sizeof(ExprProgram), hipMemcpyHostToDevice, stream));
  return ctx->progs_dev + slot;
}
void Plan::bind_values(ExprProgram& p) const {
  if (!agg_columns) return;
  for (u32 i = 0; i < p.n; i++) {
    rdfgpu_expr_node& e = p.nodes[i];
    if (e.op != kExAggValue) continue;
    const u32 node = e.u >> 8, agg = e.u & 0xffu;
    if (node >= nodes.size() || nodes[node].values_run != run) fail(RDFGPU_ERR_INVALID, "a value column of node %u is read before the node ran", node);
    e.lo = (int64_t)reinterpret_cast<uintptr_t>(nodes[node].values[agg]);
    e.hi = (int64_t)nodes[node].n_values;
  }
}
const rdfgpu_agg_value* Plan::result_values(u32 col, u64* n) const {
  const ValueOrigin& o = nodes[root].origin[col];
  if (n) *n = o.node < 0 ? 0 : nodes[o.node].n_values;
  return o.node < 0 ? nullptr : nodes[o.node].values[o.agg];
}
u64* Plan::new_counter() {
  if (counters_used >= 255) fail(RDFGPU_ERR_UNSUPPORTED, "plan needs more than 255 cardinality counters");
  return counters + counters_used++;
}
void Plan::read_back(void* host, const void* dev, size_t bytes) {
  RDFGPU_HIP(hipMemcpyAsync(host, dev, bytes, hipMemcpyDeviceToHost, stream));
  RDFGPU_HIP(hipStreamSynchronize(stream));
  metrics.host_syncs++;
}
// ... 20 lines not shown
    if (nd.d.kind == RDFGPU_NODE_TABLE) d = true;
    else if (nd.d.kind != RDFGPU_NODE_DATA_SOURCE) {
      const bool binary = is_binary(nd.d.kind);
      if (nd.d.left >= 0) d = depends((u32)nd.d.left);
      if (binary && nd.d.right >= 0) d = depends((u32)nd.d.right) || d;
    }
    dep[i] = d ? 1 : 0;
    return d;
  };
  const u64 ratio = (full + kPrimeRows - 1) / kPrimeRows;
  for (u32 i = 0; i < nodes.size(); i++) {
    NodeInfo& nd = nodes[i];
    if (nd.has_last && depends(i)) { nd.last_rows = nd.last_rows * ratio + 1024; nd.last_scaled = true; }
  }
}

bool Plan::record_band_history() {
  bool missed = false;
  for (const BandFeedback& f : band_feedback) {
    BandHistory& h = f.node->band;
    h.ran = true; h.blocks = f.known_blocks ? f.known_blocks : ctx->counters_host[f.blocks];
    h.slow_rows = ctx->counters_host[f.slow_rows] & 0xFFFFFFFFull; h.run_stats = ctx->counters_host[f.run_stats];
    if (f.slow_skipped && h.slow_rows) missed = true;
    if (f.multi_rows >= 0) h.multi_rows = ctx->counters_host[f.multi_rows] & 0xFFFFFFFFull;
    if (f.multi_rows >= 0 && f.in_place && h.multi_rows) missed = true;
  }
  return missed;
}

void Plan::execute() {
  if (!primed && !priming) prime();
  store->activate();
  std::shared_lock<std::shared_mutex> lock(store->mu);
  RDFGPU_HIP(hipStreamSynchronize(stream));
  release_intermediates();
  store->pool.trim_to(2 * std::max(std::max(scratch_hist[0], scratch_hist[1]), std::max(store->scratch_recent[0].load(), store->scratch_recent[1].load())) + (1ull << 30));
  held = store->gen;
  metrics = rdfgpu_metrics{};
  const u64 mallocs0 = store->pool.mallocs() + store->table_pool.mallocs();
  const double malloc_ms0 = store->pool.malloc_ms() + store->table_pool.malloc_ms();
  run++;
  counters_used = 0;
  progs_used = 0;
  arg_slots_used = 0;
  events_used = 2;
  pending.clear();
  host_valid = false; cursor = 0; executed = false;
  agg_out.clear();
  const hipEvent_t ev_start = ctx->event(0), ev_stop = ctx->event(1);
  RDFGPU_HIP(hipEventRecord(ev_start, stream));
  RDFGPU_HIP(hipMemsetAsync(counters, 0, 256 * sizeof(u64), stream));

  spec_checks.clear();
  pending_oj.active = false;
  band_feedback.clear();
  memo.assign(nodes.size(), DevTable{}); memo_valid.assign(nodes.size(), 0);
  speculative = allow_speculation && !opt.on(RDFGPU_OPT_NO_SPECULATION);

  refresh_dynamic_sources(lock);
  locate_sources();

  result = exec_node(root);
  flush_pending_oj();
  RDFGPU_HIP(hipMemcpyAsync(ctx->counters_host, counters, 256 * sizeof(u64), hipMemcpyDeviceToHost, stream));
  RDFGPU_HIP(hipEventRecord(ev_stop, stream));
  RDFGPU_HIP(hipStreamSynchronize(stream)); metrics.host_syncs++;
  RDFGPU_HIP(hipGetLastError());
  if (const u32 rt = (u32)(ctx->counters_host[255] & 0xFFFFFFFFull)) {
    if (rt & 1u) fail(RDFGPU_ERR_UNSUPPORTED, "REGEX with \\d \\w \\s or \\b over a string with non-ASCII characters needs the regex crate's Unicode tables (not restated)");
    if (rt & 8u) fail(RDFGPU_ERR_UNSUPPORTED, "a numeric CAST met a simple literal: the lexical forms of numbers are not parsed on the device");
    if (rt & kRtExtendKind) fail(RDFGPU_ERR_UNSUPPORTED, "a computed column (ProjectionExec with expressions) met a value that is a string, IRI, blank node, dateTime, date, time or duration: "
                                                         "its 24-byte value has no room for the language / datatype (numeric and boolean values are carried)");
    if (rt & kRtLexParse) fail(RDFGPU_ERR_UNSUPPORTED, "a lexical cast (RDFGPU_EX_CAST_LEX, xsd:float / xsd:double of a simple literal) met a literal the device cannot decide: "
                                                       "its value lies at a rounding boundary where Eisel-Lemire declines (the big-decimal path is not restated), or it is a signed NaN");
    if (rt & kRtMinMaxKind) fail(RDFGPU_ERR_UNSUPPORTED, "MIN / MAX met a bound value that is not numeric (a string, IRI, blank node, boolean, dateTime, date, time or duration): "
                                                         "the reference's order between those kinds is partial and its 24-byte value has no room for them (numeric values are answered)");
    if (rt & kRtSortTerm) fail(RDFGPU_ERR_UNSUPPORTED, "SortExec: SORT_BY_TERM over a column that is not all strings / IRIs / blank nodes");
    if (rt & 4u) fail(RDFGPU_ERR_UNSUPPORTED, "a string expression met what the device does not restate: UCASE / LCASE of a string with non-ASCII characters (Unicode case tables), "
                                               "a float / double / decimal SUBSTR position, or a comparison with a string that has no bytes on the device");
    fail(RDFGPU_ERR_UNSUPPORTED, "REGEX with a per-row pattern: a row's pattern literal was not announced in the plan's pattern table");
  }
  bool spec_failed = record_band_history();
  for (const SpecCheck& c : spec_checks) {
    if ((ctx->counters_host[c.counter + 1] & 0xFFFFFFFFull) != 0) spec_failed = true;
    else { c.node->last_rows = ctx->counters_host[c.counter]; c.node->has_last = true; c.node->last_scaled = false; }
  }
  if (spec_failed) {
    metrics.host_syncs++;
    lock.unlock();
    allow_speculation = false;
    try { execute(); } catch (...) { allow_speculation = true; throw; }
    allow_speculation = true;
    metrics.exact_reruns = 1;
    return;
  }
  result_rows = result.n_dev ? ctx->counters_host[result.n_dev - counters] : result.cap;
  if (result_rows > result.cap) result_rows = result.cap;
  for (NodeInfo& nd : nodes)
    if (nd.values_run == run && nd.n_values_dev) { nd.n_values = std::min<u64>(nd.n_values, ctx->counters_host[nd.n_values_dev - counters]); nd.n_values_dev = nullptr; }
  float ms = 0;
  RDFGPU_HIP(hipEventElapsedTime(&ms, ev_start, ev_stop));
  metrics.elapsed_compute_ms = ms;
  metrics.output_rows = result_rows;
  metrics.device_mallocs = (u32)(store->pool.mallocs() + store->table_pool.mallocs() - mallocs0);
  metrics.device_malloc_ms = store->pool.malloc_ms() + store->table_pool.malloc_ms() - malloc_ms0;
  resolve_timing();
  executed = true;
  scratch_hist[1] = scratch_hist[0]; scratch_hist[0] = metrics.device_bytes;
  store->scratch_recent[1] = store->scratch_recent[0].load(); store->scratch_recent[0] = metrics.device_bytes;
}

void Plan::refresh_dynamic_sources(std::shared_lock<std::shared_mutex>& lock) {
  bool changed = false;
  for (SourceInfo& s : sources) {
    if (!s.dynamic_dirty) continue;
    ScanInstructions eff = s.gspo;
    for (auto& dflt : s.dynamic) and_into_instructions(eff, dflt.first, dflt.second);
    derive_source(s, eff);
    s.dynamic_dirty = false;
    changed = true;
  }
  if (changed) {
    lock.unlock();
    upload_pool();
    lock.lock();
    located_version = ~0ull;
    for (NodeInfo& nd : nodes) { nd.has_last = false; nd.last_rows = 0; }
    speculative = false;
  }
}

void Plan::locate_sources() {
  if (!sources.empty() && located_version == store->version.load()) {
    for (const SourceInfo& s : sources) metrics.input_rows += s.hi - s.lo;
  } else if (!sources.empty()) {
    located_version = store->version.load();
    LocateJob* jobs = static_cast<LocateJob*>(ctx->jobs_host);
    for (size_t i = 0; i < sources.size(); i++) {
      const SourceInfo& s = sources[i];
      const Permutation& ix = store->idx[s.components];
      LocateJob& j = jobs[i];
      for (int k = 0; k < 4; k++) j.col[k] = ix.col[k];
// ... 195 lines not shown
  t.n_dev = n_out;
  return t;
}

constexpr int kExtendGuard = 0xA5;
DevTable Plan::exec_extend(NodeInfo& nd) {
  const DevTable in = exec_sub_plan((u32)nd.d.left);
  flush_pending_oj();
  if (in.cap >= 0xFFFFFFFFull) fail(RDFGPU_ERR_UNSUPPORTED, "ProjectionExec with expressions over %llu rows (fewer than 2^32 - 1)", (unsigned long long)in.cap);
  const u32 k = (u32)nd.agg_progs.size();
  DevTable t = project(in, nd);
  t.n_cols = nd.width;
  ExtendArgs a{};
  a.n_dev = in.n_dev; a.cap = in.cap;
  for (u32 c = 0; c < in.n_cols; c++) a.col[c] = in.cols[c];
  a.n_exprs = k;
  a.tt = typed_table();
  for (u32 q = 0; q < k; q++) {
    a.out[q] = scratch<rdfgpu_agg_value>(in.cap + 1); a.out_val[q] = scratch<u32>(in.cap + 1);
    RDFGPU_HIP(hipMemsetAsync(a.out[q] + in.cap, kExtendGuard, sizeof(rdfgpu_agg_value), stream));
    RDFGPU_HIP(hipMemsetAsync(a.out_val[q] + in.cap, kExtendGuard, sizeof(u32), stream));
    nd.values[q] = a.out[q]; t.cols[nd.n_proj + q] = a.out_val[q];
  }
  nd.n_values = in.cap; nd.n_values_dev = in.cap ? in.n_dev : nullptr; nd.values_run = run;
  if (in.cap == 0) return t;
  for (u32 q = 0; q < k; q++) a.prog[q] = upload_program(nd.agg_progs[q]);
  timed(KC_EXTEND, 0, in.cap, in.n_dev, 4ull * nd.n_cols_read + 16ull * nd.n_enc_tv + 28ull * k, nullptr, 0, 0, [&] { launch_extend(a, nd.lex, stream); });
  return t;
}

void Plan::ensure_host_copy() {
  if (host_valid) return;
  if (!executed) fail(RDFGPU_ERR_INVALID, "plan has not been executed");
  store->activate();
  host_cols.assign(result.n_cols, std::vector<u32>());
  for (u32 c = 0; c < result.n_cols; c++) {
    host_cols[c].resize(result_rows);
    if (result_rows) RDFGPU_HIP(hipMemcpyAsync(host_cols[c].data(), result.cols[c], result_rows * 4, hipMemcpyDeviceToHost, stream));
  }
  host_aggs.assign(agg_out.size(), std::vector<rdfgpu_agg_value>());
  for (size_t i = 0; i < agg_out.size(); i++) {
    host_aggs[i].resize(result_rows);
    if (result_rows) RDFGPU_HIP(hipMemcpyAsync(host_aggs[i].data(), agg_out[i], result_rows * sizeof(rdfgpu_agg_value), hipMemcpyDeviceToHost, stream));
  }
  RDFGPU_HIP(hipStreamSynchronize(stream));
  host_values.assign(result.n_cols, std::vector<rdfgpu_agg_value>());
  std::vector<const rdfgpu_agg_value*> origins; std::vector<std::vector<rdfgpu_agg_value>> copies;
  std::vector<int> copy_of(result.n_cols, -1);
  for (u32 c = 0; c < result.n_cols; c++) {
    u64 n = 0;
    const rdfgpu_agg_value* dev = result_values(c, &n);
    if (!dev) continue;
    const size_t at = std::find(origins.begin(), origins.end(), dev) - origins.begin();
    if (at == origins.size()) { origins.push_back(dev); copies.emplace_back(result_rows ? n : 0); }
    copy_of[c] = (int)at;
  }
  for (size_t i = 0; i < origins.size(); i++)
    if (!copies[i].empty()) RDFGPU_HIP(hipMemcpyAsync(copies[i].data(), origins[i], copies[i].size() * sizeof(rdfgpu_agg_value), hipMemcpyDeviceToHost, stream));
  if (!origins.empty()) RDFGPU_HIP(hipStreamSynchronize(stream));
  for (u32 c = 0; c < result.n_cols; c++) {
    if (copy_of[c] < 0) continue;
    const std::vector<rdfgpu_agg_value>& all = copies[copy_of[c]];
    host_values[c].assign(result_rows, rdfgpu_agg_value{});
    for (u64 r = 0; r < result_rows; r++) { const u32 id = host_cols[c][r]; if (id != 0 && id <= all.size()) host_values[c][r] = all[id - 1]; }
  }
  host_valid = true;
// ... 4 lines not shown
```

rdf-fusion_amd/csrc/plan.hpp:

```cpp
#pragma once
#include <memory>
#include <shared_mutex>
#include <string>
#include <vector>

#include "host_logic.hpp"
#include "kernels.hpp"
#include "store.hpp"

namespace rdfgpu {

struct SourceInfo {
  u32 node = 0;
  u32 components = RDFGPU_GSPO;
  ScanInstructions ix;
  PrunePlan prune;
  bool has_residual = false;
  u32 n_out = 0;
  u32 out_level[4] = {};
  u64 lo = 0, hi = 0;
  u32 sorted_level = 4, key_min = 0, key_max = 0;
  ScanInstructions gspo;
  std::vector<std::pair<u32, ScanPredicate>> dynamic;
  bool dynamic_dirty = false;
// ... 47 lines not shown

struct BoundTable { std::vector<const u32*> cols; u64 n_rows = 0; bool bound = false; };

enum class JoinTable {
  Lds,
  SliceCsr, SliceDirect, SliceHash,
  Partitioned,
  TransientDirect, ScratchHash
};

struct LdsJoin {
  NodeInfo& nd;
  const DevTable& L; const DevTable& R;
  const bool build_left;
  const DevTable& B; const DevTable& P;
  const NodeInfo* probe_filter;
  const NodeInfo* post_filter;
  const bool probe_outer, left_join;
  LdsJoinArgs a{};
  u32 build_keys[RDFGPU_MAX_KEYS] = {}, probe_keys[RDFGPU_MAX_KEYS] = {};
  u32 probe_cols = 0, build_payload = 0;
  u64 build_bytes = 0;
  u32 slots = 64;
  bool global_table = false;
  JoinTable table = JoinTable::Lds;
  SliceTable* slice = nullptr;
  PartArgs part{};
  u64 tail = 0;
  bool stream_values_tried = false;
  u64 stage_bytes = 0;
  std::vector<ColRef> chain_cols; SliceTable::ValueColumn chain_vc[kMaxChain] = {};
  BandArgs band{}; bool use_band = false;
  DevTable t;
  LdsJoin(NodeInfo& n, const DevTable& l, const DevTable& r, bool bl, const NodeInfo* pf, const NodeInfo* post)
      : nd(n), L(l), R(r), build_left(bl), B(bl ? l : r), P(bl ? r : l), probe_filter(pf), post_filter(post),
        probe_outer(n.d.join_type == RDFGPU_JOIN_LEFT && !bl), left_join(n.d.join_type == RDFGPU_JOIN_LEFT && bl) {}
};

struct BandJoin {
  LdsJoin& j; const u32 kn; const u64 np, nb, cmax;
  bool presorted = false;
  bool skip_slow = false;
  bool counting = false;
  bool fused = false;
  bool in_place = false;
  bool cache_entries = false;
  OjBandFuse fuse{};
  std::string ekey; SliceTable::BandEntries lay{};
  SliceTable::BandRowWindows rw{};
  BandForm form = BandForm::RECORDS;
  bool row_static() const { return form != BandForm::RECORDS; }
  u64 nrows = 0, max_blocks = 0;
  u32* skey = nullptr; u32* perm = nullptr; u32 sort_bits = 1; void* sort_temp = nullptr; size_t sort_temp_bytes = 0;
  BandJoin(LdsJoin& join) : j(join), kn(join.a.direct_n), np(join.P.cap), nb(join.B.cap), cmax((join.slice->csr_max_group + 63) / 64) {}
};

struct BandRowTiers { bool build_windows = false, build_verdicts = false, build_list = false, use_verdicts = false, use_list = false; };

enum KernelClass {
  KC_LOCATE, KC_SCAN_COUNT, KC_SCAN_WRITE, KC_FILTER_ID, KC_FILTER_TV, KC_FILTER_VM, KC_CROSS, KC_JOIN_BUILD,
  KC_JOIN_COUNT, KC_JOIN_WRITE, KC_LEFT_TAIL, KC_NLJ_COUNT, KC_NLJ_WRITE, KC_DEVICE_SCAN,
  KC_GJOIN_BUILD,
  KC_GDIRECT_BUILD, KC_MINMAX, KC_CSR_HIST, KC_CSR_SCATTER,
  KC_TOPK_MAX, KC_TOPK_HIST, KC_TOPK_SCATTER, KC_TOPK_SELECT, KC_TOPK_WRITE,
  KC_FILTER_VERDICT, KC_REGEX_VERDICTS, KC_UNION,
  KC_BAND_SLOW, KC_RADIX_SORT, KC_BAND_BOUNDS, KC_BAND_BLOCKS, KC_BAND_DECODE, KC_BAND_MASK, KC_BAND_EMIT, KC_BAND_ENTRIES, KC_BAND_DESC, KC_BAND_PT, KC_BAND_ROWS,
// ... 49 lines not shown
};

struct AggNode {
  NodeInfo& nd; const DevTable& in;
  AggArgs a{};
  bool wide = false; AggWideArgs w{};
  u64 slots = 64;
  u64 G = 1;
  u64 accum_row_bytes = 0, refine_row_bytes = 0;
  u64 group_row_bytes = 0;
  AggNode(NodeInfo& n, const DevTable& t) : nd(n), in(t) {}
};

struct Plan {
  Store* store = nullptr;
  EngineOptions opt;
  std::vector<NodeInfo> nodes;
  std::vector<SourceInfo> sources;
  std::vector<u32> pool;
  u32* pool_dev = nullptr;
  RegexProg* regex_dev = nullptr;
  unsigned char* str_consts_dev = nullptr;
  rdfgpu_agg_value* mark_values_dev = nullptr;
  std::vector<std::string> regex_strings; std::vector<rdfgpu_regex> regex_text;
  u32 root = 0;
  u64 run = 0;
  bool agg_columns = false;
  bool value_keys = false;
  ExecContext* ctx = nullptr;
  hipStream_t stream = nullptr;
  std::vector<BoundTable> tables;

  std::vector<void*> allocs;
  u64* counters = nullptr;
  u32 counters_used = 0;
  u32 progs_used = 0;
  u32 arg_slots_used = 0;
  DevTable result; u64 result_rows = 0; bool executed = false;
  std::shared_ptr<IndexGeneration> held;
  rdfgpu_metrics metrics{};
  bool timing = false;
  int timing_focus = -1;
  int last_top_kc = -1;
  u64 located_version = ~0ull;
  bool allow_speculation = true, speculative = false;
  u64 scratch_hist[2] = {0, 0};
  bool priming = false, primed = false;
  void prime();
  std::vector<SpecCheck> spec_checks;
  struct BandFeedback { NodeInfo* node; u32 blocks, slow_rows, run_stats; int multi_rows; bool slow_skipped, in_place; u64 known_blocks; };
  std::vector<BandFeedback> band_feedback;
  bool record_band_history();
  std::vector<PendingLaunch> pending;
  std::vector<DevTable> memo; std::vector<char> memo_valid;
  ChainRequest* pending_chain = nullptr;
  PendingOj pending_oj;
  void flush_pending_oj();
  void count_pending_oj();
  void count_ordered_join(OrderedJoinArgs& o);
  void probe_ordered_join(OrderedJoinArgs& o);
  u32 events_used = 0;
  KernelStat kstats[KC__N];
  std::vector<std::vector<u32>> host_cols; bool host_valid = false; u64 cursor = 0;
  std::vector<rdfgpu_agg_value*> agg_out; std::vector<std::vector<rdfgpu_agg_value>> host_aggs;
  std::vector<std::vector<rdfgpu_agg_value>> host_values;
  const rdfgpu_agg_value* result_values(u32 col, u64* n) const;
// ... 78 lines not shown
```

rdf-fusion_amd/csrc/plan_band.cpp:

```cpp
#include "plan_exec.hpp"

namespace rdfgpu {

namespace {
bool range_op(u8 op) { return op == RDFGPU_EX_GT || op == RDFGPU_EX_LT || op == RDFGPU_EX_GEQ || op == RDFGPU_EX_LEQ; }
}

bool Plan::plan_chain(NodeInfo& top, ChainRequest& req) {
  if (!speculative || !top.has_last || opt.on(RDFGPU_OPT_NO_CHAIN_FUSION) || opt.on(RDFGPU_OPT_NO_TABLE_CACHE)) return false;
  req.top = &top;
  std::vector<ChainLink> down;
  NodeInfo* cur = &top;
  while ((int)down.size() < kMaxChain) {
    const rdfgpu_plan_node& d = cur->d;
    if (d.kind != RDFGPU_NODE_HASH_JOIN || d.join_type != RDFGPU_JOIN_INNER || d.n_keys != 1) break;
    if (cur->prog.n != 0 && cur->shape != 2 && cur->shape != 3) break;
    bool found = false;
    for (int side = 0; side < 2 && !found; side++) {
      const u32 cs = (u32)(side == 0 ? d.left : d.right), co = (u32)(side == 0 ? d.right : d.left);
      const NodeInfo& sn = nodes[cs]; const NodeInfo& on = nodes[co];
      if (sn.d.kind != RDFGPU_NODE_DATA_SOURCE || sources[sn.source].has_residual) continue;
      if (on.d.kind != RDFGPU_NODE_HASH_JOIN || on.d.join_type > RDFGPU_JOIN_LEFT || on.refs != 1) continue;
      const DevTable S = exec_node(cs);
      if (S.cap == 0 || S.stable_id == 0) continue;
// ... 478 lines not shown
void Plan::band_blocks_and_emit(BandJoin& bj) {
  const LdsJoinArgs& a = bj.j.a; BandArgs& b = bj.j.band;
  const u32 kn = bj.kn; const u64 np = bj.np, max_blocks = bj.max_blocks;
  if (!bj.presorted && !bj.counting) timed(KC_RADIX_SORT, 0, np, nullptr, 0, nullptr, 0, 0, [&] { sort_pairs_u32_u32(b.skey_in, bj.skey, b.sval_in, bj.perm, np, bj.sort_bits, bj.sort_temp, bj.sort_temp_bytes, stream); });
  b.boff = bj.in_place ? bj.lay.boff : scratch<u32>((u64)kn + 1); b.n_blocks_out = new_counter();
  band_feedback.push_back({&bj.j.nd, (u32)(b.n_blocks_out - counters), (u32)(reinterpret_cast<u64*>(b.slow_rows) - counters), (u32)(reinterpret_cast<u64*>(b.run_stats) - counters),
                           bj.fused ? (int)(reinterpret_cast<u64*>(pending_oj.o.multi_rows) - counters) : -1, bj.skip_slow, bj.in_place, bj.in_place ? max_blocks : 0});
  const u64 hist = bj.j.nd.band.blocks; b.launch_blocks = (u32)(bj.in_place ? max_blocks : std::min<u64>(max_blocks, hist ? hist + hist / 4 + 1024 : max_blocks));
  b.bdesc = bj.in_place ? bj.lay.bdesc : scratch<uint4>(max_blocks);
  const size_t tb = std::max(scan_temp_bytes(std::max<u64>((u64)kn + 1, max_blocks + 1)), band_blocks_scan_temp_bytes(kn)); void* temp = scratch<unsigned char>(tb);
  if (bj.counting) {
    timed(scan_class((u64)kn + 1), 0, (u64)kn + 1, nullptr, 8, nullptr, 0, 0, [&] { exclusive_scan_u32(b.key_hist, b.poff, (u64)kn + 1, temp, tb, stream); });
    RDFGPU_HIP(hipMemcpyAsync(b.key_cursor, b.poff, ((size_t)kn + 1) * sizeof(u32), hipMemcpyDeviceToDevice, stream));
    timed(KC_BAND_ROWS, 0, np, bj.j.P.n_dev, 8 + 32 + 32, nullptr, 0, 0, [&] { launch_band_scatter(b, stream); });
  } else if (!bj.presorted) timed(KC_BAND_BOUNDS, 0, np, nullptr, 4, nullptr, 0, 0, [&] { launch_band_bounds(bj.skey, np, kn, b.poff, stream); });
  if (!bj.in_place) {
    timed(scan_class((u64)kn + 1), 12ull * kn, (u64)kn + 1, nullptr, 4, nullptr, 0, 0, [&] { band_blocks_scan(a.csr_off, b.poff, kn, b.boff, temp, tb, stream); });
    timed(KC_BAND_DESC, 12ull * kn, 0, nullptr, 0, nullptr, 0, 0, [&] { launch_band_desc(b, stream); });
  }
  if (!bj.presorted && !bj.counting) timed(KC_BAND_ROWS, 0, np, bj.j.P.n_dev, 4 + 32 + 32, nullptr, 0, 0, [&] { launch_band_rows(b, stream); });
  const u64* const nrows_dev = bj.in_place ? nullptr : bj.j.P.n_dev;
  const BandPassBytes bytes = band_pass_bytes(bj);
  timed(KC_BAND_MASK, bytes.mask_fixed, bj.nrows, nrows_dev, bytes.mask_row, nullptr, 0, 0, [&] { launch_band_mask(b, bj.form, stream); });
  if (!bj.skip_slow) {
    if (bj.row_static()) fail(RDFGPU_ERR_INVALID, "band join: the full-semantics pass over a step of form %s", band_form_name(bj.form));
    static_assert(sizeof(LdsJoinArgs) <= ExecContext::kArgBytes, "argument staging slot too small");
    const u32 slot = arg_slots_used++;
    LdsJoinArgs* a_host = reinterpret_cast<LdsJoinArgs*>(ctx->args_host + (size_t)slot * ExecContext::kArgBytes);
    LdsJoinArgs* a_dev = reinterpret_cast<LdsJoinArgs*>(ctx->args_dev + (size_t)slot * ExecContext::kArgBytes);
    *a_host = a; RDFGPU_HIP(hipMemcpyAsync(a_dev, a_host, sizeof(LdsJoinArgs), hipMemcpyHostToDevice, stream));
    timed(KC_BAND_SLOW, 0, 0, nullptr, 0, nullptr, 0, 0, [&] { launch_band_slow(a_dev, b, stream); });
  }
  timed(scan_class(max_blocks + 1), 0, max_blocks + 1, nullptr, 8, nullptr, 0, 0, [&] { exclusive_scan_u32(b.bcount, b.bofs, max_blocks + 1, temp, tb, stream); });
  timed(KC_BAND_EMIT, bytes.emit_fixed, bj.nrows, nrows_dev, 4 + 4ull * b.n_row_cols, a.n_out_dev, 0, 4ull * a.n_out_cols, [&] { launch_band_emit(b, bj.form, stream); });
}

}
```

rdf-fusion_amd/csrc/plan_exec.hpp:

```cpp
#pragma once
#include <algorithm>
#include <cstdlib>
#include <cstring>
#include <memory>
#include <mutex>
#include <shared_mutex>

#include "plan.hpp"

namespace rdfgpu {

inline bool is_binary(u32 kind) {
  return kind == RDFGPU_NODE_HASH_JOIN || kind == RDFGPU_NODE_CROSS_JOIN || kind == RDFGPU_NODE_NESTED_LOOP_JOIN || kind == RDFGPU_NODE_UNION;
}

inline u32 columns_read(const ExprProgram& p) {
  static_assert(2 * kMaxCols <= 32, "one bit per column of a join's two sides");
  u32 cols = 0;
  for (u32 i = 0; i < p.n; i++) if (p.nodes[i].op == RDFGPU_EX_COLUMN) cols |= 1u << p.nodes[i].u;
  return cols;
}

inline DevTable project(const DevTable& in, const NodeInfo& nd) {
  DevTable t;
  t.n_cols = nd.n_proj; t.cap = in.cap; t.n_dev = in.n_dev;
  for (u32 c = 0; c < nd.n_proj; c++) t.cols[c] = in.cols[nd.proj[c]];
  return t;
}

inline bool on_build_side(const LdsJoinArgs& a, u32 c) { return (c < a.n_left_cols) == (a.build_is_left != 0); }

inline TvLiteral window_literal(const rdfgpu_expr_node* e, u32 o) {
  TvLiteral l{};
  l.lo = e[o + 4].lo; l.hi = e[o + 4].hi; l.aux = e[o + 4].u; l.tag = e[o + 4].tag; l.flags = e[o + 4].flags;
  l.arith_sub = e[o + 5].op == RDFGPU_EX_SUB; l.cmp_op = e[o + 6].op;
  return l;
}

inline int scan_class(u64 n) { return n <= kSmallScanElems ? KC_SMALL_SCAN : KC_DEVICE_SCAN; }

template <class F>
void Plan::timed(int kc, u64 fixed_bytes, u64 rows_cap, const u64* rows_dev, u64 bytes_per_row,
                 const u64* out_dev, u64 out_rows, u64 bytes_per_out, F&& launch) {
  metrics.kernels_launched++;
  if (!timing || (timing_focus >= 0 && kc != timing_focus)) { launch(); return; }
  PendingLaunch p{kc, ctx->event(events_used), ctx->event(events_used + 1), fixed_bytes, rows_cap, rows_dev, bytes_per_row, out_dev, out_rows, bytes_per_out};
  events_used += 2;
  RDFGPU_HIP(hipEventRecord(p.start, stream));
  launch();
  RDFGPU_HIP(hipEventRecord(p.stop, stream));
  pending.push_back(p);
}

template <class T> T* Plan::scratch(u64 n) {
  void* p = store->pool.alloc((n ? n : 1) * sizeof(T));
  allocs.push_back(p);
  metrics.device_bytes += (n ? n : 1) * sizeof(T);
  return (T*)p;
}

template <class F> void Plan::device_minmax_i64(long long (&got)[2], F&& launch) {
  long long* mm = reinterpret_cast<long long*>(new_counter()); (void)new_counter();
  const long long init[2] = {INT64_MAX, INT64_MIN + 1};
  RDFGPU_HIP(hipMemcpyAsync(mm, init, sizeof init, hipMemcpyHostToDevice, stream));
  launch(mm);
  read_back(got, mm, sizeof got);
}

}
```

rdf-fusion_amd/csrc/plan_join.cpp:

```cpp
#include "plan_exec.hpp"

namespace rdfgpu {

namespace {
u32 pow2_at_least(u64 v) { u64 p = 1024; while (p < v && p < (1ull << 31)) p <<= 1; return (u32)p; }
}

bool Plan::keeps_pending_oj(const NodeInfo& nd, const DevTable& L, const DevTable& R, bool left_join, bool lf, bool rf) const {
  if (!nd.band.takes_records || nd.d.kind != RDFGPU_NODE_HASH_JOIN || left_join || lf || rf || opt.on(RDFGPU_OPT_NO_LDS_JOIN) || nd.lex) return false;
  const bool build_left = choose_build_left(nd, L, R, false, false, false);
  const DevTable& B = build_left ? L : R; const DevTable& P = build_left ? R : L;
  return (B.cap <= kLdsJoinMaxBuild || !opt.on(RDFGPU_OPT_NO_GLOBAL_TABLE_JOIN)) && P.cols[0] == pending_oj.first_col && B.cols[0] != pending_oj.first_col;
}

void Plan::flush_pending_oj() {
  if (!pending_oj.active) return;
  count_pending_oj();
  pending_oj.active = false;
  const OrderedJoinArgs& o = pending_oj.o;
  timed(KC_OJ_WRITE, 0, pending_oj.n_build, nullptr, 4, o.n_out_dev, 0, 8ull * o.n_out_cols, [&] { launch_ordered_join_write(o, stream); });
}

void Plan::probe_ordered_join(OrderedJoinArgs& o) {
  o.head = scratch<uint2>(o.kn); o.next = scratch<u32>(o.n_probe_cap);
// ... 566 lines not shown
  if (j.table == JoinTable::Partitioned) {
    timed(KC_PART_JOIN, j.build_bytes, P.cap, P.n_dev, 4ull * j.probe_cols + 8, a.n_out_dev, 0, out_bytes_per_row, [&] { launch_part_join(a, j.part, stream); });
    return;
  }
  const bool streamed = a.stream_direct && direct_stream_join_ok(a);
  if (streamed && !j.stream_values_tried && a.direct && a.has_filter == 3 && a.has_probe_filter == 0 && B.n_dev == nullptr && a.tt.n_ids != 0 &&
      direct_stream_join_items(P.cap) == 8 && P.cap >= (1ull << 22) && !opt.on(RDFGPU_OPT_NO_VALUE_TABLES)) {
    j.stream_values_tried = true;
    if (a.win.x0 == a.win.x1 && on_build_side(a, a.win.x0) && !on_build_side(a, a.win.y0) && !on_build_side(a, a.win.y1)) {
      long long* vals = scratch<long long>(a.direct_n);
      u32* bad = reinterpret_cast<u32*>(new_counter());
      launch_fill_i64(vals, INT64_MIN, a.direct_n, stream);
      launch_direct_values(a.build_key[0], a.cols[a.win.x0], B.cap, a.direct_min, a.direct_n, a.tt, vals, bad, stream);
      if (!read_back<u32>(bad)) {
        a.key_vals = vals; metrics.tables_built++;
        a.stream_need_build_row = (a.has_post && on_build_side(a, a.post.col)) ? 1u : 0u;
        for (u32 c = 0; c < j.nd.n_proj; c++) if (on_build_side(a, j.nd.proj[c])) a.stream_need_build_row = 1u;
      }
    }
  }
  const int kc = streamed ? (int)KC_STREAM_JOIN
                          : lds_join_class(a.has_filter, a.has_probe_filter, lds_join_items(P.cap << a.row_lanes_log2, j.global_table), lds_join_mode(a), a.n_chain != 0);
  timed(kc, (j.global_table ? 0 : j.build_bytes) + stage_bytes, P.cap, P.n_dev, 4ull * j.probe_cols + 8, a.n_out_dev, 0, out_bytes_per_row, [&] { launch_lds_join(a, stream); });
}

DevTable Plan::run_speculative(LdsJoin& j, u64 first_guess, NodeInfo& size_node) {
  LdsJoinArgs& a = j.a;
  DevTable& t = j.t;
  const u64 spec_cap = j.nd.has_last ? std::max<u64>(1024, size_node.last_rows + size_node.last_rows / (size_node.last_scaled ? 2 : 4) + 256)
                                     : std::max<u64>(1024, first_guess);
  a.out_cap = spec_cap;
  for (u32 c = 0; c < a.n_out_cols; c++) { a.out[c] = scratch<u32>(spec_cap + j.tail); t.cols[c] = a.out[c]; }
  if (j.left_join) RDFGPU_HIP(hipMemsetAsync(a.visited, 0, j.L.cap, stream));
  if (j.use_band) exec_band_join(j);
  else if (!run_ordered_join(j, size_node, spec_cap)) run_join_kernel(j, j.stage_bytes, 4ull * a.n_out_cols);
  const SpecCheck check{&size_node, (u32)(a.n_out_dev - counters), j.left_join};
  if (pending_oj.active && !pending_oj.counted && pending_oj.o.n_out_dev == a.n_out_dev) pending_oj.check = check;
  else spec_checks.push_back(check);
  t.cap = spec_cap + j.tail; t.n_dev = a.n_out_dev;
  if (j.left_join) left_join_tail(j.nd, j.L, j.R, a.out, a.visited, a.n_out_dev, spec_cap + j.tail);
  return t;
}

bool Plan::run_ordered_join(LdsJoin& j, const NodeInfo& size_node, u64 spec_cap) {
  const LdsJoinArgs& a = j.a;
  const DevTable& B = j.B; const DevTable& P = j.P;
  if (j.probe_outer || opt.on(RDFGPU_OPT_NO_ORDERED_JOIN) || !a.csr_off || a.range_rows || j.left_join || a.has_filter != 0 || a.has_probe_filter || a.has_post ||
      a.n_keys != 1 || B.sorted_col < 0 || (u32)B.sorted_col == j.build_keys[0] || B.n_dev || !B.stable_id || B.cap >= (1ull << 32) || P.cap > (1ull << 24) ||
      !size_node.has_last || size_node.last_rows * 8 < B.cap)
    return false;
  for (u32 s = 0; s < a.n_chain; s++) if (a.chain[s].key.src != 0 || a.chain[s].fs != 0) return false;
  u32 from_table = 0;
  for (u32 c = 0; c < a.n_out_cols; c++) from_table += a.n_chain ? a.chain_out[c].src != 1 : !on_build_side(a, a.proj[c]);
  if (from_table > 8 || a.n_out_cols > kOjMaxOutCols) return false;
  DevTable& t = j.t;
  OrderedJoinArgs o{};
  o.build_key = a.build_key[0]; o.n_build = B.cap;
  o.probe_key = a.probe_key[0]; o.n_probe_dev = P.n_dev; o.n_probe_cap = P.cap;
  o.kmin = a.direct_min; o.kn = a.direct_n;
  o.n_stages = a.n_chain;
  for (u32 s = 0; s < a.n_chain; s++) o.stage[s] = OrderedJoinStage{a.chain[s].key.ptr, a.chain[s].direct, a.chain[s].kmin, a.chain[s].kn, nullptr};
  o.n_out_cols = a.n_out_cols;
  u32 n_words = 0;
  for (u32 c = 0; c < a.n_out_cols; c++) {
    if (a.n_chain) o.out_ref[c] = a.chain_out[c];
    else { const u32 pc = a.proj[c]; o.out_ref[c] = ColRef{a.cols[pc], on_build_side(a, pc) ? 1u : 0u, 0u}; }
// ... 131 lines not shown
```

rdf-fusion_amd/csrc/store.cpp:

```cpp
#include "store.hpp"

#include <chrono>
#include <cstdlib>
#include <string>
#include <vector>

#include "kernels.hpp"

namespace rdfgpu {

static size_t bucket_of(size_t bytes) {
  size_t b = 256;
  while (b < bytes) b <<= 1;
  if (bytes > (64ull << 20)) b = (bytes + (16ull << 20) - 1) / (16ull << 20) * (16ull << 20);
  return b;
}
static std::mutex g_pools_mu;
static std::vector<DevicePool*> g_pools;
DevicePool::DevicePool() { std::lock_guard<std::mutex> g(g_pools_mu); g_pools.push_back(this); }
DevicePool::~DevicePool() {
  { std::lock_guard<std::mutex> g(g_pools_mu); for (size_t i = 0; i < g_pools.size(); i++) if (g_pools[i] == this) { g_pools.erase(g_pools.begin() + i); break; } }
  trim();
  for (auto& kv : live_) (void)hipFree(kv.first);
}
// ... 7 lines not shown
  if (it != free_.end()) { p = it->second.p; got = it->first; free_.erase(it); cached_ -= got; }
  else {
    const auto t0 = std::chrono::steady_clock::now();
    struct Tally { DevicePool* self; std::chrono::steady_clock::time_point t0; ~Tally() { self->n_mallocs_++; self->malloc_ns_ += (u64)std::chrono::duration_cast<std::chrono::nanoseconds>(std::chrono::steady_clock::now() - t0).count(); } } tally{this, t0};
    hipError_t e = hipMalloc(&p, b);
    if (e != hipSuccess) {
      for (auto& kv : free_) (void)hipFree(kv.second.p);
      free_.clear(); cached_ = 0;
      (void)hipGetLastError();
      e = hipMalloc(&p, b);
      if (e != hipSuccess) {
        (void)hipGetLastError();
        std::lock_guard<std::mutex> gp(g_pools_mu);
        for (DevicePool* other : g_pools) if (other != this && other->mu_.try_lock()) {
          for (auto& kv : other->free_) (void)hipFree(kv.second.p);
          other->free_.clear(); other->cached_ = 0;
          other->mu_.unlock();
        }
        e = hipMalloc(&p, b);
      }
      if (e != hipSuccess) {
        size_t free_b = 0, total_b = 0;
        (void)hipMemGetInfo(&free_b, &total_b);
        (void)hipGetLastError();
        fail(RDFGPU_ERR_OOM, "device allocation of %zu bytes failed (%s): %zu of %zu bytes free, %zu bytes held by this pool",
             b, hipGetErrorString(e), free_b, total_b, in_use_);
      }
    }
  }
  live_[p] = got;
  in_use_ += got;
  return p;
}
void DevicePool::free(void* p) {
  if (!p) return;
  std::lock_guard<std::mutex> g(mu_);
  auto it = live_.find(p);
  if (it == live_.end()) return;
  in_use_ -= it->second;
  cached_ += it->second;
  free_.emplace(it->second, Cached{p, epoch_});
  live_.erase(it);
}
void DevicePool::trim_to(u64 keep_bytes) {
  std::lock_guard<std::mutex> g(mu_);
  epoch_++;
  while (cached_ > keep_bytes && !free_.empty()) {
    auto victim = free_.begin();
    for (auto it = free_.begin(); it != free_.end(); ++it)
      if (it->second.epoch < victim->second.epoch || (it->second.epoch == victim->second.epoch && it->first > victim->first)) victim = it;
    (void)hipFree(victim->second.p);
    cached_ -= victim->first;
    free_.erase(victim);
  }
}
void DevicePool::trim() {
  std::lock_guard<std::mutex> g(mu_);
  cached_ = 0;
  for (auto& kv : free_) (void)hipFree(kv.second.p);
  free_.clear();
}

static const char* const kOptionNames[RDFGPU_OPT__COUNT] = {
    "FORCE_GENERIC_VM", "NO_JOIN_REORDER", "NO_SPECULATION", "NO_FIRST_RUN_SPECULATION", "NO_STRING_VERDICTS",
    "NO_TABLE_CACHE", "NO_INDEX_JOIN", "NO_CHAIN_FUSION", "NO_VALUE_TABLES", "NO_RANGE_INDEX", "NO_FILTER_FUSION",
    "NO_LDS_JOIN", "NO_GLOBAL_TABLE_JOIN", "NO_DIRECT_TABLE", "NO_BAND_JOIN", "NO_PARTITIONED_JOIN", "NO_VALUE_VERDICTS", "NO_PRIMING", "NO_ORDERED_JOIN", "NO_BAND_PACK16", "NO_RUN_COPY", "NO_RANGE_PARTITION",
    "LDS_MAX_BUILD", "CSR_ROW_LANES_LOG2", "JOIN_WAVE_Q", "PARTITION_MIN_BUILD", "PARTITION_TWO_PASS_ROWS", "NO_OWN_PARTITION_PASS", "NO_BAND_COMPACT", "NO_PROBE_OUTER_JOIN", "NO_STREAM_JOIN", "PARTITION_ROWS", "PARTITION_SLOTS",
    "NO_SEMI_LDS", "NO_BAND_PAIR_COUNTS", "BAND_PAIR_COUNT_BLOCKS", "NO_BAND_ROW_CACHE", "NO_BAND_PAIR_LIST", "NO_BAND_PAIR_CACHE", "BAND_PAIR_CACHE_BLOCKS", "NO_AGG_LDS"};
const char* engine_option_name(u32 option) { return option < RDFGPU_OPT__COUNT ? kOptionNames[option] : nullptr; }
const EngineOptions& default_engine_options() {
  static const EngineOptions defaults = [] {
    EngineOptions o;
    o.v[RDFGPU_OPT_LDS_MAX_BUILD] = 1024;
    o.v[RDFGPU_OPT_PARTITION_MIN_BUILD] = 1ull << 21;
    o.v[RDFGPU_OPT_PARTITION_TWO_PASS_ROWS] = 50ull << 20;
    for (u32 i = 0; i < RDFGPU_OPT__COUNT; i++) {
      const std::string name = std::string("RDFGPU_") + kOptionNames[i];
      if (const char* e = std::getenv(name.c_str())) {
        const bool is_value = i >= RDFGPU_OPT_LDS_MAX_BUILD;
        o.v[i] = is_value ? std::strtoull(e, nullptr, 10) + (i == RDFGPU_OPT_CSR_ROW_LANES_LOG2 ? 1 : 0) : 1;
      }
    }
    return o;
  }();
  return defaults;
}

Store* store_create(const rdfgpu_config* cfg) {
  int count = 0;
  hipError_t e = hipGetDeviceCount(&count);
  if (e != hipSuccess || count == 0) {
    (void)hipGetLastError();
    fail(RDFGPU_ERR_NO_DEVICE, "no usable HIP device (%s); this library has no CPU fallback",
         e != hipSuccess ? hipGetErrorString(e) : "device count is 0");
  }
  int dev = cfg ? cfg->device : -1;
  if (dev < 0) RDFGPU_HIP(hipGetDevice(&dev));
  if (dev >= count) fail(RDFGPU_ERR_NO_DEVICE, "device %d does not exist (%d devices)", dev, count);
  RDFGPU_HIP(hipSetDevice(dev));
  hipDeviceProp_t prop;
  RDFGPU_HIP(hipGetDeviceProperties(&prop, dev));
// ... 15 lines not shown
    preload_tu_kernels();
    preload_tu_band_join();
    preload_tu_ordered_join();
    preload_tu_ntriples();
    preload_tu_part_join();
    preload_tu_part_pass();
    preload_tu_stream_join();
    preload_tu_exchange();
    preload_tu_topk();
    preload_tu_closure();
    preload_tu_semi_join();
    preload_tu_aggregate();
    preload_tu_extend();
    preload_tu_sort();
    preload_tu_join_fs0();
    preload_tu_join_fs1();
    preload_tu_join_fs2();
    preload_tu_join_fs3();
  });
}

void Store::activate() const { RDFGPU_HIP(hipSetDevice(device)); }

hipEvent_t ExecContext::event(u32 i) {
  while (events.size() <= i) {
    hipEvent_t e;
    RDFGPU_HIP(hipEventCreate(&e));
    events.push_back(e);
  }
  return events[i];
}
ExecContext::~ExecContext() {
  for (hipEvent_t e : events) (void)hipEventDestroy(e);
  if (counters) (void)hipFree(counters);
  if (counters_host) (void)hipHostFree(counters_host);
  if (progs_dev) (void)hipFree(progs_dev);
  if (progs_host) (void)hipHostFree(progs_host);
  if (args_dev) (void)hipFree(args_dev);
  if (args_host) (void)hipHostFree(args_host);
  if (jobs_dev) (void)hipFree(jobs_dev);
  if (lohi_dev) (void)hipFree(lohi_dev);
  if (jobs_host) (void)hipHostFree(jobs_host);
  if (lohi_host) (void)hipHostFree(lohi_host);
  if (stream) (void)hipStreamDestroy(stream);
}
ExecContext* Store::acquire_context(u32 n_sources) {
  activate();
  ExecContext* c = nullptr;
  {
    std::lock_guard<std::mutex> g(ctx_mu);
    if (!free_ctx.empty()) { c = free_ctx.back(); free_ctx.pop_back(); }
  }
  if (!c) {
    c = new ExecContext();
    RDFGPU_HIP(hipStreamCreateWithFlags(&c->stream, hipStreamNonBlocking));
    RDFGPU_HIP(hipMalloc((void**)&c->counters, 256 * sizeof(u64)));
    RDFGPU_HIP(hipHostMalloc((void**)&c->counters_host, 256 * sizeof(u64), hipHostMallocDefault));
    RDFGPU_HIP(hipMalloc((void**)&c->progs_dev, ExecContext::kProgSlots * sizeof(ExprProgram)));
    RDFGPU_HIP(hipHostMalloc((void**)&c->progs_host, ExecContext::kProgSlots * sizeof(ExprProgram), hipHostMallocDefault));
    RDFGPU_HIP(hipMalloc((void**)&c->args_dev, (size_t)ExecContext::kArgSlots * ExecContext::kArgBytes));
    RDFGPU_HIP(hipHostMalloc((void**)&c->args_host, (size_t)ExecContext::kArgSlots * ExecContext::kArgBytes, hipHostMallocDefault));
  }
  const u32 need = n_sources ? n_sources : 1;
  if (c->job_cap < need) {
    if (c->jobs_dev) { (void)hipFree(c->jobs_dev); (void)hipFree(c->lohi_dev); (void)hipHostFree(c->jobs_host); (void)hipHostFree(c->lohi_host); }
    const u32 cap = need < 16 ? 16 : need;
    RDFGPU_HIP(hipMalloc(&c->jobs_dev, cap * 128));
    RDFGPU_HIP(hipMalloc((void**)&c->lohi_dev, cap * kLocateWords * sizeof(u64)));
    RDFGPU_HIP(hipHostMalloc(&c->jobs_host, cap * 128, hipHostMallocDefault));
    RDFGPU_HIP(hipHostMalloc((void**)&c->lohi_host, cap * kLocateWords * sizeof(u64), hipHostMallocDefault));
    c->job_cap = cap;
  }
  return c;
}
void Store::release_context(ExecContext* c) {
  if (!c) return;
  std::lock_guard<std::mutex> g(ctx_mu);
  free_ctx.push_back(c);
}

SliceTable* Store::slice_table(const SliceKey& k) {
  std::lock_guard<std::mutex> lock(slice_mu);
  return &slice_tables[k];
}
const SliceTable* Store::find_slice_table(const SliceKey& k) {
  std::lock_guard<std::mutex> lock(slice_mu);
  auto it = slice_tables.find(k);
  return it == slice_tables.end() ? nullptr : &it->second;
}
void Store::drop_slice_tables() {
  std::lock_guard<std::mutex> lock(slice_mu);
  for (auto& kv : slice_tables) {
    SliceTable& t = kv.second;
    table_free(t.direct); table_free(t.csr_off); table_free(t.csr_rows); table_free(t.slots);
    for (auto& v : t.values) table_free(v.val);
    for (auto& r : t.ranges) { table_free(r.rows); table_free(r.vals); table_free(r.link); }
    for (auto& e : t.band_entries) { table_free(e.et); for (u32* p : e.eo) table_free(p); table_free(e.boff); table_free(e.bdesc); }
    for (auto& e : t.band_row_windows) { table_free(e.row_win); table_free(e.pair_bits); table_free(e.pair_list); table_free(e.pair_list_off); table_free(e.pair_cnt); }
    for (auto& v : t.value_starts) table_free(v.lo);
  }
  slice_tables.clear();
}
void Store::drop_tables() {
  std::unique_lock<std::shared_mutex> lock(mu);
  activate();
  RDFGPU_HIP(hipDeviceSynchronize());
  version++;
  drop_slice_tables();
}

void Store::drop_string_verdicts() {
  std::lock_guard<std::mutex> lock(slice_mu);
  for (auto& kv : string_verdicts) if (kv.second) (void)hipFree(kv.second);
  string_verdicts.clear();
}

Store::~Store() {
  (void)hipSetDevice(device);
  drop_slice_tables();
  drop_string_verdicts();
  for (ExecContext* c : free_ctx) delete c;
  gen.reset();
  if (tv) (void)hipFree(tv);
  if (dec) (void)hipFree(dec);
  if (str_off) (void)hipFree(str_off);
  if (heap) (void)hipFree(heap);
  if (stream) (void)hipStreamDestroy(stream);
}

IndexGeneration::~IndexGeneration() {
  (void)hipSetDevice(device);
  for (auto& ix : idx) for (auto& c : ix.col) if (c) (void)hipFree(c);
}
void Store::adopt(std::shared_ptr<IndexGeneration> fresh) {
  version++;
  drop_slice_tables();
  gen = std::move(fresh);
  for (u32 k = 0; k < RDFGPU_N_INDEXES; k++) idx[k] = gen->idx[k];
}

void Store::clear() {
  std::unique_lock<std::shared_mutex> lock(mu);
  activate();
  auto fresh = std::make_shared<IndexGeneration>();
  fresh->device = device;
  adopt(fresh);
}

namespace {
struct Scratch {
  DevicePool& pool; std::vector<void*> ptrs;
  explicit Scratch(DevicePool& p) : pool(p) {}
  template <class T> T* get(u64 n) { void* p = pool.alloc((n ? n : 1) * sizeof(T)); ptrs.push_back(p); return (T*)p; }
  ~Scratch() { for (void* p : ptrs) pool.free(p); }
};
}

static u64 compact_columns(Store& st, Scratch& sc, u32* const src[4], const u32* flags, u64 n, Permutation& dst) {
  hipStream_t s = st.stream;
  u32* excl = sc.get<u32>(n);
  const size_t tb = scan_temp_bytes(n);
  void* temp = sc.get<u8>(tb);
  exclusive_scan_u32(flags, excl, n, temp, tb, s);
  u32 last_excl = 0, last_flag = 0;
  if (n) {
    RDFGPU_HIP(hipMemcpyAsync(&last_excl, excl + n - 1, 4, hipMemcpyDeviceToHost, s));
    RDFGPU_HIP(hipMemcpyAsync(&last_flag, flags + n - 1, 4, hipMemcpyDeviceToHost, s));
    RDFGPU_HIP(hipStreamSynchronize(s));
  }
  const u64 total = (u64)last_excl + (last_flag ? 1 : 0);
  for (int k = 0; k < 4; k++) {
    dst.col[k] = nullptr;
    if (total) {
      RDFGPU_HIP(hipMalloc((void**)&dst.col[k], total * sizeof(u32)));
      launch_scatter_if(src[k], flags, excl, dst.col[k], n, s);
    }
  }
  dst.n = total;
  RDFGPU_HIP(hipStreamSynchronize(s));
  return total;
}

u64 Store::extend_device(const u32* g, const u32* s_, const u32* p, const u32* o, u64 n) {
  std::unique_lock<std::shared_mutex> lock(mu);
  activate();
  if (n == 0) return 0;
  const u32* in[4] = {g, s_, p, o};
  hipStream_t s = stream;
  u64 inserted = 0;
  auto fresh_gen = std::make_shared<IndexGeneration>();
  fresh_gen->device = device;
  for (u32 comp = 0; comp < RDFGPU_N_INDEXES; comp++) {
    const Permutation& ix = idx[comp];
    const u64 N = ix.n + n;
    if (N >= 0xFFFFFFFFull) fail(RDFGPU_ERR_UNSUPPORTED, "index would exceed 2^32-1 rows");
    Scratch sc(pool);
    u32* cat[4];
    for (int k = 0; k < 4; k++) {
      cat[k] = sc.get<u32>(N);
      if (ix.n) RDFGPU_HIP(hipMemcpyAsync(cat[k], ix.col[k], ix.n * 4, hipMemcpyDeviceToDevice, s));
      RDFGPU_HIP(hipMemcpyAsync(cat[k] + ix.n, in[PERM[comp][k]], n * 4, hipMemcpyDeviceToDevice, s));
    }
    u64* key_a = sc.get<u64>(N); u64* key_b = sc.get<u64>(N);
    u32* idx_a = sc.get<u32>(N); u32* idx_b = sc.get<u32>(N);
    const size_t tb = sort_temp_bytes(N);
    void* temp = sc.get<u8>(tb);
    launch_iota_u32(idx_a, N, s);
    launch_pack_key(cat[2], cat[3], nullptr, key_a, N, s);
    sort_pairs_u64_u32(key_a, key_b, idx_a, idx_b, N, temp, tb, s);
    launch_pack_key(cat[0], cat[1], idx_b, key_a, N, s);
    sort_pairs_u64_u32(key_a, key_b, idx_b, idx_a, N, temp, tb, s);
    u32* sorted[4];
    for (int k = 0; k < 4; k++) { sorted[k] = sc.get<u32>(N); launch_gather_u32(cat[k], idx_a, sorted[k], N, s); }
    u32* flags = sc.get<u32>(N);
    launch_unique_flags(sorted[0], sorted[1], sorted[2], sorted[3], flags, N, s);
    const u64 total = compact_columns(*this, sc, sorted, flags, N, fresh_gen->idx[comp]);
    if (comp && total - ix.n != inserted) fail(RDFGPU_ERR_DEVICE, "extend: the permutations disagree on the number of new quads (%llu vs %llu)", (unsigned long long)(total - ix.n), (unsigned long long)inserted);
    inserted = total - ix.n;
  }
  adopt(fresh_gen);
  pool.trim();
  return inserted;
}

u64 Store::extend_host(const u32* g, const u32* s_, const u32* p, const u32* o, u64 n) {
  activate();
  if (n == 0) return 0;
  u32* d[4];
  const u32* h[4] = {g, s_, p, o};
  for (int k = 0; k < 4; k++) {
    d[k] = (u32*)pool.alloc(n * 4);
    RDFGPU_HIP(hipMemcpy(d[k], h[k], n * 4, hipMemcpyHostToDevice));
  }
  u64 r = 0;
  try { r = extend_device(d[0], d[1], d[2], d[3], n); } catch (...) { for (auto q : d) pool.free(q); throw; }
  for (auto q : d) pool.free(q);
  pool.trim();
  return r;
}

u64 Store::remove_host(const u32* g, const u32* s_, const u32* p, const u32* o, u64 n) {
  std::unique_lock<std::shared_mutex> lock(mu);
  activate();
  if (n == 0 || idx[0].n == 0) return 0;
  hipStream_t s = stream;
  const u32* h[4] = {g, s_, p, o};
  u64 removed = 0;
  auto fresh_gen = std::make_shared<IndexGeneration>();
  fresh_gen->device = device;
  for (u32 comp = 0; comp < RDFGPU_N_INDEXES; comp++) {
    const Permutation& ix = idx[comp];
    Scratch sc(pool);
    u32* rm[4];
    for (int k = 0; k < 4; k++) {
      rm[k] = sc.get<u32>(n);
      RDFGPU_HIP(hipMemcpyAsync(rm[k], h[PERM[comp][k]], n * 4, hipMemcpyHostToDevice, s));
    }
    u32* keep = sc.get<u32>(ix.n);
    launch_fill_u32(keep, 1u, ix.n, s);
    const u32* ixc[4] = {ix.col[0], ix.col[1], ix.col[2], ix.col[3]};
    const u32* rmc[4] = {rm[0], rm[1], rm[2], rm[3]};
    launch_mark_removed(ixc, ix.n, rmc, n, keep, s);
    const u64 total = compact_columns(*this, sc, ix.col, keep, ix.n, fresh_gen->idx[comp]);
    if (comp && ix.n - total != removed) fail(RDFGPU_ERR_DEVICE, "remove: the permutations disagree on the number of removed quads");
    removed = ix.n - total;
  }
  adopt(fresh_gen);
  pool.trim();
  return removed;
}

u64 Store::remove_graph(u32 graph) {
  std::unique_lock<std::shared_mutex> lock(mu);
  activate();
  if (idx[0].n == 0) return 0;
  hipStream_t s = stream;
  u64 removed = 0;
  auto fresh_gen = std::make_shared<IndexGeneration>();
  fresh_gen->device = device;
  for (u32 comp = 0; comp < RDFGPU_N_INDEXES; comp++) {
    const Permutation& ix = idx[comp];
    Scratch sc(pool);
    u32* keep = sc.get<u32>(ix.n);
    launch_mark_not_equal(ix.col[0], graph, keep, ix.n, s);
    const u64 total = compact_columns(*this, sc, ix.col, keep, ix.n, fresh_gen->idx[comp]);
    if (comp && ix.n - total != removed) fail(RDFGPU_ERR_DEVICE, "remove_graph: the permutations disagree on the number of removed quads");
    removed = ix.n - total;
  }
  if (removed) adopt(fresh_gen);
  pool.trim();
  return removed;
}

void Store::set_typed_values(const rdfgpu_typed_value* v, u64 n, const int64_t* d, u64 nd) {
  std::unique_lock<std::shared_mutex> lock(mu);
  activate();
  drop_string_verdicts();
  drop_slice_tables();
  if (tv) { RDFGPU_HIP(hipFree(tv)); tv = nullptr; }
  if (dec) { RDFGPU_HIP(hipFree(dec)); dec = nullptr; }
  n_ids = n; n_dec = nd;
  if (n) {
    RDFGPU_HIP(hipMalloc((void**)&tv, n * sizeof(rdfgpu_typed_value)));
    RDFGPU_HIP(hipMemcpy(tv, v, n * sizeof(rdfgpu_typed_value), hipMemcpyHostToDevice));
  }
  if (nd) {
    RDFGPU_HIP(hipMalloc((void**)&dec, nd * 16));
    RDFGPU_HIP(hipMemcpy(dec, d, nd * 16, hipMemcpyHostToDevice));
  }
}

void Store::set_strings(const u64* offsets, u64 n, const unsigned char* heap_host, u64 heap_bytes) {
  std::unique_lock<std::shared_mutex> lock(mu);
  activate();
  drop_string_verdicts();
  if (n && !offsets) fail(RDFGPU_ERR_INVALID, "set_strings: null offsets");
  for (u64 i = 0; i < n; i++) if (offsets[i] > offsets[i + 1] || offsets[i + 1] > heap_bytes) fail(RDFGPU_ERR_INVALID, "set_strings: offsets of id %llu are not monotone / inside the heap", (unsigned long long)i);
  if (str_off) { RDFGPU_HIP(hipFree(str_off)); str_off = nullptr; }
  if (heap) { RDFGPU_HIP(hipFree(heap)); heap = nullptr; }
  n_str_ids = n;
  if (!n) return;
  RDFGPU_HIP(hipMalloc((void**)&str_off, (n + 1) * sizeof(u64)));
  RDFGPU_HIP(hipMemcpy(str_off, offsets, (n + 1) * sizeof(u64), hipMemcpyHostToDevice));
  RDFGPU_HIP(hipMalloc((void**)&heap, heap_bytes ? heap_bytes : 1));
  if (heap_bytes) RDFGPU_HIP(hipMemcpy(heap, heap_host, heap_bytes, hipMemcpyHostToDevice));
}

}
```

rdf-fusion_amd/csrc/store.hpp:

```cpp
#pragma once
#include <atomic>
#include <map>
#include <memory>
#include <mutex>
#include <shared_mutex>
#include <string>
#include <vector>

#include "common.hpp"
#include "expr_device.hpp"

namespace rdfgpu {

class DevicePool {
 public:
  DevicePool();
  ~DevicePool();
  void* alloc(size_t bytes);
  void free(void* p);
  void trim();
  void trim_to(u64 keep_bytes);
  u64 bytes_in_use() const { return in_use_; }
  u64 bytes_cached() const { return cached_; }
  u64 mallocs() const { return n_mallocs_.load(); }
  double malloc_ms() const { return (double)malloc_ns_.load() * 1e-6; }

 private:
  std::mutex mu_;
  struct Cached { void* p; u64 epoch; };
  std::multimap<size_t, Cached> free_;
  u64 epoch_ = 0;
  std::map<void*, size_t> live_;
  u64 in_use_ = 0, cached_ = 0;
  std::atomic<u64> n_mallocs_{0}, malloc_ns_{0};
};

struct ExecContext {
  hipStream_t stream = nullptr;
  std::vector<hipEvent_t> events;
  u64* counters = nullptr;
  u64* counters_host = nullptr;
  void* jobs_dev = nullptr; u64* lohi_dev = nullptr; u32 job_cap = 0;
  void* jobs_host = nullptr; u64* lohi_host = nullptr;
  static constexpr u32 kProgSlots = 16;
  ExprProgram* progs_dev = nullptr; ExprProgram* progs_host = nullptr;
  static constexpr u32 kArgSlots = 4, kArgBytes = 4096;
  unsigned char* args_dev = nullptr; unsigned char* args_host = nullptr;
  hipEvent_t event(u32 i);
  ~ExecContext();
};

struct EngineOptions {
  u64 v[RDFGPU_OPT__COUNT] = {};
  bool on(int o) const { return v[o] != 0; }
};
const EngineOptions& default_engine_options();
const char* engine_option_name(u32 option);

struct Permutation {
  u32* col[4] = {nullptr, nullptr, nullptr, nullptr};
  u64 n = 0;
};
struct IndexGeneration {
  Permutation idx[RDFGPU_N_INDEXES];
  int device = 0;
  ~IndexGeneration();
};

struct SliceTable {
  bool dense_tried = false, dense_failed = false;
  u32* direct = nullptr; u32 kmin = 0, kn = 0;
  u32* csr_off = nullptr; u32* csr_rows = nullptr;
  u32 csr_max_group = 0;
  void* slots = nullptr; u32 mask = 0;
// ... 9 lines not shown
    u8* pair_cnt = nullptr;
  };
  std::vector<BandRowWindows> band_row_windows;
  struct ValueStarts { u32 first; u64 span; u32* lo; };
  std::vector<ValueStarts> value_starts;
};
struct SliceKey {
  const u32* key[RDFGPU_MAX_KEYS] = {}; u32 n_keys = 0; u64 rows = 0;
  bool operator<(const SliceKey& o) const {
    if (n_keys != o.n_keys) return n_keys < o.n_keys;
    if (rows != o.rows) return rows < o.rows;
    for (u32 i = 0; i < RDFGPU_MAX_KEYS; i++) if (key[i] != o.key[i]) return key[i] < o.key[i];
    return false;
  }
};

struct Store {
  int device = 0;
  u32 batch_size = 8192;
  EngineOptions opt = default_engine_options();
  std::shared_ptr<IndexGeneration> gen;
  Permutation idx[RDFGPU_N_INDEXES];
  void adopt(std::shared_ptr<IndexGeneration> fresh);
  rdfgpu_typed_value* tv = nullptr; u64 n_ids = 0;
  int64_t* dec = nullptr; u64 n_dec = 0;
  u64* str_off = nullptr; unsigned char* heap = nullptr; u64 n_str_ids = 0;
  DevicePool pool;
  std::atomic<u64> scratch_recent[2] = {{0}, {0}};
  DevicePool table_pool;
  template <class T> T* table_alloc(u64 n) { return static_cast<T*>(table_pool.alloc((n ? n : 1) * sizeof(T))); }
  void table_free(void* p) { table_pool.free(p); }
  hipStream_t stream = nullptr;
  std::shared_mutex mu;
  std::atomic<int> refs{1};
  void retain() { refs.fetch_add(1); }
  void release() { if (refs.fetch_sub(1) == 1) delete this; }
  std::atomic<u64> version{0};
  std::mutex slice_mu, slice_build_mu;
  std::map<SliceKey, SliceTable> slice_tables;
  std::map<std::string, unsigned char*> string_verdicts;
  void drop_string_verdicts();
  SliceTable* slice_table(const SliceKey& k);
  const SliceTable* find_slice_table(const SliceKey& k);
  void drop_slice_tables();
  void drop_tables();
  std::mutex ctx_mu;
  std::vector<ExecContext*> free_ctx;
  ExecContext* acquire_context(u32 n_sources);
  void release_context(ExecContext* c);

  ~Store();
  void activate() const;
  u64 extend_device(const u32* g, const u32* s, const u32* p, const u32* o, u64 n);
  u64 extend_host(const u32* g, const u32* s, const u32* p, const u32* o, u64 n);
  u64 remove_host(const u32* g, const u32* s, const u32* p, const u32* o, u64 n);
  u64 remove_graph(u32 graph);
  void clear();
  void set_typed_values(const rdfgpu_typed_value* v, u64 n_ids, const int64_t* dec, u64 n_dec);
  void set_strings(const u64* offsets, u64 n_ids, const unsigned char* heap_host, u64 heap_bytes);
  TypedTable typed_table() const { return TypedTable{tv, n_ids, dec, n_dec, str_off, heap, n_str_ids, nullptr}; }
};

Store* store_create(const rdfgpu_config* cfg);

}
```

rdf-fusion_amd/engine.py:

```python
import ctypes as C
import os

import numpy as np

from . import abi

_LIB = None
_HERE = os.path.dirname(os.path.abspath(__file__))


class RdfGpuError(RuntimeError):
    def __init__(self, status, message):
        super().__init__(f"rdfgpu status {status}: {message}")
        self.status = status


def library_path():
    return os.path.join(_HERE, "lib", "librdfgpu.so")


def kernel_source_sha16():
    import glob
    import hashlib
    h = hashlib.sha256()
# ... 60 lines not shown
    lib.rdfgpu_plan_decode_terms.argtypes = [vp, C.c_uint32, C.c_uint64, C.c_uint64, C.POINTER(abi.ArrowArray), C.POINTER(abi.ArrowSchema)]
    lib.rdfgpu_plan_metrics.argtypes = [vp, C.POINTER(abi.Metrics)]
    lib.rdfgpu_plan_selected_index.argtypes = [vp, C.c_uint32, u32p]
    lib.rdfgpu_plan_stream.argtypes = [vp, C.POINTER(vp)]
    lib.rdfgpu_plan_enable_kernel_timing.argtypes = [vp, C.c_int]
    lib.rdfgpu_plan_kernel_stats.argtypes = [vp, C.POINTER(abi.KernelStat), C.c_uint32, u32p]
    lib.rdfgpu_plan_pushdown_filters.argtypes = [vp, C.c_uint32, C.POINTER(abi.PushdownFilter), C.c_uint32, C.POINTER(C.c_uint8)]
    lib.rdfgpu_plan_set_dynamic_filters.argtypes = [vp, C.c_uint32, C.POINTER(abi.PushdownFilter), C.c_uint32]
    lib.rdfgpu_plan_source_predicate.argtypes = [vp, C.c_uint32, C.c_uint32, C.POINTER(abi.Predicate)]
    lib.rdfgpu_store_set_option.argtypes = [vp, C.c_uint32, C.c_uint64]
    lib.rdfgpu_store_get_option.argtypes = [vp, C.c_uint32, u64p]
    lib.rdfgpu_plan_set_option.argtypes = [vp, C.c_uint32, C.c_uint64]
    lib.rdfgpu_option_name.argtypes = [C.c_uint32]
    lib.rdfgpu_option_name.restype = C.c_char_p
    lib.rdfgpu_comm_unique_id.argtypes = [C.c_void_p]
    lib.rdfgpu_comm_create.argtypes = [C.c_void_p, C.c_uint32, C.c_uint32, C.c_int32, C.POINTER(vp)]
    lib.rdfgpu_comm_create_host.argtypes = [C.c_uint32, C.c_uint32, C.c_int32, abi.HOST_ALLTOALLV_FN, C.c_void_p, C.POINTER(vp)]
    lib.rdfgpu_comm_destroy.argtypes = [vp]
    lib.rdfgpu_comm_destroy.restype = None
    lib.rdfgpu_exchange_allgatherv.argtypes = [vp, C.POINTER(vp), C.c_uint32, C.c_uint64, C.POINTER(vp), u64p]
    lib.rdfgpu_exchange_repartition.argtypes = [vp, C.POINTER(vp), C.c_uint32, C.c_uint64, C.c_uint32, C.POINTER(vp), u64p]
    lib.rdfgpu_shard_of.argtypes = [C.c_uint32, C.c_uint32]
    lib.rdfgpu_shard_of.restype = C.c_uint32
    lib.rdfgpu_scan_score.argtypes = [C.POINTER(abi.ScanInstruction)]
    lib.rdfgpu_scan_score.restype = C.c_uint64
    lib.rdfgpu_choose_index.argtypes = [C.POINTER(abi.ScanInstruction), C.c_uint32]
    lib.rdfgpu_choose_index.restype = C.c_uint32
    lib.rdfgpu_band_row_cache_eligible.argtypes = [C.c_uint32] * 5 + [u32p, u32p]
    lib.rdfgpu_band_pair_cache_eligible.argtypes = [C.c_uint32] * 4 + [C.c_uint64] * 2
    lib.rdfgpu_band_pair_list_eligible.argtypes = [C.c_uint32] * 2 + [C.c_uint64] * 2
    lib.rdfgpu_band_pair_count_eligible.argtypes = [C.c_uint32] * 2 + [C.c_uint64] * 2
    lib.rdfgpu_band_step_form.argtypes = [C.c_uint32] * 6 + [C.c_uint64] * 2
    lib.rdfgpu_oj_probe_form.argtypes = [C.c_uint32] * 5
    lib.rdfgpu_predicate_and.argtypes = [C.POINTER(abi.Predicate), C.POINTER(abi.Predicate),
                                         C.POINTER(abi.Predicate), u32p]
    lib.rdfgpu_pushdown_to_scan_predicate.argtypes = [C.c_uint32, C.c_uint32, C.POINTER(abi.Predicate)]
    lib.rdfgpu_regex_check.argtypes = [C.c_char_p, C.c_uint32, C.c_char_p, C.c_uint32, C.POINTER(C.c_uint32)]
    if lib.rdfgpu_abi_version() != abi.ABI_VERSION:
        raise RdfGpuError(abi.ERR_INVALID, "ABI version mismatch between abi.py and librdfgpu.so")
    _LIB = lib
    return lib


def _check(status):
    if status < 0:
        raise RdfGpuError(status, load_library().rdfgpu_last_error().decode("utf-8", "replace"))
    return status


def _u32(a):
    a = np.ascontiguousarray(a, dtype=np.uint32)
    return a, a.ctypes.data_as(C.c_void_p)


def _instr_array(builder_instrs):
    arr = (abi.ScanInstruction * 4)(*builder_instrs)
    return arr


def scan_score(instrs):
    return int(load_library().rdfgpu_scan_score(_instr_array(instrs)))


def choose_index(gspo_instrs, available=0b111):
    return int(load_library().rdfgpu_choose_index(_instr_array(gspo_instrs), available))

# ... 1 lines not shown
def band_row_cache_eligible(operands, in_place=True, compact=True, pack16=True, option_set=False):
    flat = [op for window in operands for op in window]
    n = max(4, len(flat))
    src = (C.c_uint32 * n)(*[int(s) for s, _ in flat])
    keyed = (C.c_uint32 * n)(*[int(bool(k)) for _, k in flat])
    return bool(_check(load_library().rdfgpu_band_row_cache_eligible(int(in_place), int(compact), int(pack16), int(option_set), len(operands), src, keyed)))


def band_pair_cache_eligible(n_blocks, row_windows=True, neq_self=True, pack16=True, option_set=False, cap_blocks=0):
    return bool(_check(load_library().rdfgpu_band_pair_cache_eligible(int(row_windows), int(neq_self), int(pack16), int(option_set), int(n_blocks), int(cap_blocks))))


def band_pair_list_eligible(survivors, n_blocks, pair_cached=True, option_set=False):
    return bool(_check(load_library().rdfgpu_band_pair_list_eligible(int(pair_cached), int(option_set), int(survivors), int(n_blocks))))


def band_pair_count_eligible(n_blocks, has_list=True, option_set=False, min_blocks=0):
    return bool(_check(load_library().rdfgpu_band_pair_count_eligible(int(has_list), int(option_set), int(n_blocks), int(min_blocks))))


BAND_FORMS = ("RECORDS", "ROW_WINDOWS", "VERDICTS", "VERDICTS_LIST", "COUNTS_LIST")


def band_step_form(n_blocks, row_static=True, has_verdicts=True, has_list=True, list_option_set=False, counts_option_set=False, n_row_cols=1, min_blocks=0):
    return BAND_FORMS[_check(load_library().rdfgpu_band_step_form(int(row_static), int(has_verdicts), int(has_list), int(list_option_set), int(counts_option_set),
                                                                   int(n_row_cols), int(n_blocks), int(min_blocks)))]


OJ_PROBE_FORMS = ("FULL", "LEAN", "FULL_NOW")


def oj_probe_form(held=True, in_place=True, row_cache=True, option_set=False, row_static=True):
    return OJ_PROBE_FORMS[_check(load_library().rdfgpu_oj_probe_form(int(held), int(in_place), int(row_cache), int(option_set), int(row_static)))]


def _pred_struct(p, keep):
    s = abi.Predicate()
    s.pred = p.kind
    if p.kind == abi.PRED_IN:
        ids = (C.c_uint32 * len(p.ids))(*p.ids)
        keep.append(ids)
        s.ids, s.n_ids = ids, len(p.ids)
    elif p.kind == abi.PRED_BETWEEN:
        s.from_, s.to = p.lo, p.hi
    elif p.kind == abi.PRED_EQUAL_TO:
        s.equal_to = 0
    return s


def _pred_from_struct(s, ids_buf):
    from .plan import MemIndexScanPredicate as P
    if s.pred == abi.PRED_FALSE:
        return P.false()
    if s.pred == abi.PRED_IN:
        if s.n_ids == 1 and not ids_buf:
            return P.in_([s.from_])
        return P.in_([ids_buf[i] for i in range(s.n_ids)])
    if s.pred == abi.PRED_BETWEEN:
        return P.between(s.from_, s.to)
    return None


def predicate_and(lhs, rhs, lib_fn=None):
    keep = []
    a, b, out = _pred_struct(lhs, keep), _pred_struct(rhs, keep), abi.Predicate()
    n = max(1, len(lhs.ids or []), len(rhs.ids or []))
# ... 241 lines not shown

    def __init__(self, store, description):
        self._lib = store._lib
        self._store = store
        self._desc = description
        self._h = C.c_void_p()
        self._keep = []
        _check(self._lib.rdfgpu_plan_compile(store._h, C.byref(description.desc), C.byref(self._h)))

    def close(self):
        if self._h:
            self._lib.rdfgpu_plan_destroy(self._h)
            self._h = C.c_void_p()

    def __del__(self):
        try:
            self.close()
        except Exception:
            pass

    def bind_table(self, slot, device_ptrs, n_rows):
        arr = (C.c_void_p * len(device_ptrs))(*device_ptrs)
        _check(self._lib.rdfgpu_plan_bind_table(self._h, slot, arr, len(device_ptrs), n_rows))

    def execute(self):
        _check(self._lib.rdfgpu_plan_execute(self._h))
        return self

    def result_info(self):
        n, c = C.c_uint64(), C.c_uint32()
        _check(self._lib.rdfgpu_plan_result_info(self._h, C.byref(n), C.byref(c)))
        return n.value, c.value

    def result_device(self):
        n, c = self.result_info()
        ptrs = (C.c_void_p * max(1, c))()
        _check(self._lib.rdfgpu_plan_result_device(self._h, ptrs, c))
        return [ptrs[i] or 0 for i in range(c)], n

    def fetch(self):
        n, c = self.result_info()
        cols = [np.empty(n, np.uint32) for _ in range(c)]
        ptrs = (C.c_void_p * max(1, c))(*[x.ctypes.data_as(C.c_void_p) for x in cols])
        _check(self._lib.rdfgpu_plan_fetch(self._h, ptrs, c))
        return cols

    def agg_count(self):
        n = C.c_uint32()
        _check(self._lib.rdfgpu_plan_agg_count(self._h, C.byref(n)))
        return n.value

    def fetch_aggregate(self, agg):
        n, _ = self.result_info()
        out = np.zeros(n, AGG_DTYPE)
        _check(self._lib.rdfgpu_plan_agg_fetch(self._h, agg, out.ctypes.data_as(C.c_void_p)))
        return out

    def aggregate_device(self, agg):
        p = C.c_void_p()
        _check(self._lib.rdfgpu_plan_agg_device(self._h, agg, C.byref(p)))
        return p.value or 0

    def aggregate_values(self, agg):
        return [agg_value(int(v["tag"]), int(v["lo"]), int(v["hi"])) for v in self.fetch_aggregate(agg)]

    def result_values(self, col):
# ... 120 lines not shown
```

Measured before the change: 144.2 billion bindings/s.

## Return early once the root band join's result count is known, deferring tail completion

```diff
diff --git a/include/rdfgpu.h b/include/rdfgpu.h
--- a/include/rdfgpu.h
+++ b/include/rdfgpu.h
@@ -293,6 +293,7 @@
 int rdfgpu_plan_execute(rdfgpu_plan* plan);
 
 int rdfgpu_plan_result_info(rdfgpu_plan* plan, uint64_t* n_rows, uint32_t* n_cols);
+int rdfgpu_plan_tail_pending(rdfgpu_plan* plan, uint32_t* out);
 int rdfgpu_plan_result_device(rdfgpu_plan* plan, const uint32_t** cols, uint32_t cap_cols);
 int rdfgpu_plan_fetch(rdfgpu_plan* plan, uint32_t* const* host_cols, uint32_t n_cols);
 typedef struct rdfgpu_agg_value {
@@ -378,6 +379,7 @@
   RDFGPU_OPT_NO_SEMI_LDS,
   RDFGPU_OPT_NO_BAND_PAIR_COUNTS,
   RDFGPU_OPT_BAND_PAIR_COUNT_BLOCKS,
+  RDFGPU_OPT_NO_EARLY_RESULT_COUNT,
   RDFGPU_OPT_NO_BAND_ROW_CACHE,
   RDFGPU_OPT_NO_BAND_PAIR_LIST,
   RDFGPU_OPT_NO_BAND_PAIR_CACHE,
@@ -400,6 +402,7 @@
 int rdfgpu_band_step_form(uint32_t row_static, uint32_t has_verdicts, uint32_t has_list, uint32_t list_option_set, uint32_t counts_option_set,
                           uint32_t n_row_cols, uint64_t n_blocks, uint64_t min_blocks);
 int rdfgpu_oj_probe_form(uint32_t held, uint32_t in_place, uint32_t row_cache, uint32_t option_set, uint32_t row_static);
+int rdfgpu_early_count_eligible(uint32_t is_root, uint32_t result_is_output, uint32_t form, uint32_t skip_slow, uint32_t speculative, uint32_t priming, uint32_t timing, uint32_t option_set);
 typedef struct rdfgpu_predicate {
   uint32_t pred;
   uint32_t from, to;
diff --git a/rdf-fusion_amd/__init__.py b/rdf-fusion_amd/__init__.py
--- a/rdf-fusion_amd/__init__.py
+++ b/rdf-fusion_amd/__init__.py
@@ -1,7 +1,8 @@
 from . import abi, plan
 from .engine import (RdfGpuError, GpuQuadStore, GpuPlan, Comm, NTriples, load_library, library_path, kernel_source_sha16,
                      choose_index, scan_score, predicate_and, pushdown_to_scan_predicate, shard_of, band_row_cache_eligible,
-                     band_pair_cache_eligible, band_pair_list_eligible, band_pair_count_eligible, band_step_form, BAND_FORMS, oj_probe_form, OJ_PROBE_FORMS)
+                     band_pair_cache_eligible, band_pair_list_eligible, band_pair_count_eligible, band_step_form, BAND_FORMS, oj_probe_form, OJ_PROBE_FORMS,
+                     early_count_eligible)
 
 __all__ = ["abi", "plan", "RdfGpuError", "GpuQuadStore", "GpuPlan", "Comm", "NTriples", "shard_of", "load_library", "library_path", "kernel_source_sha16",
-           "choose_index", "scan_score", "predicate_and", "pushdown_to_scan_predicate", "band_row_cache_eligible", "band_pair_cache_eligible", "band_pair_list_eligible", "band_pair_count_eligible", "band_step_form", "BAND_FORMS", "oj_probe_form", "OJ_PROBE_FORMS"]
+           "choose_index", "scan_score", "predicate_and", "pushdown_to_scan_predicate", "band_row_cache_eligible", "band_pair_cache_eligible", "band_pair_list_eligible", "band_pair_count_eligible", "band_step_form", "BAND_FORMS", "oj_probe_form", "OJ_PROBE_FORMS", "early_count_eligible"]
diff --git a/rdf-fusion_amd/abi.py b/rdf-fusion_amd/abi.py
--- a/rdf-fusion_amd/abi.py
+++ b/rdf-fusion_amd/abi.py
@@ -58,7 +58,7 @@
                 "NO_TABLE_CACHE", "NO_INDEX_JOIN", "NO_CHAIN_FUSION", "NO_VALUE_TABLES", "NO_RANGE_INDEX", "NO_FILTER_FUSION",
                 "NO_LDS_JOIN", "NO_GLOBAL_TABLE_JOIN", "NO_DIRECT_TABLE", "NO_BAND_JOIN", "NO_PARTITIONED_JOIN", "NO_VALUE_VERDICTS", "NO_PRIMING", "NO_ORDERED_JOIN", "NO_BAND_PACK16", "NO_RUN_COPY", "NO_RANGE_PARTITION",
                 "LDS_MAX_BUILD", "CSR_ROW_LANES_LOG2", "JOIN_WAVE_Q", "PARTITION_MIN_BUILD", "PARTITION_TWO_PASS_ROWS", "NO_OWN_PARTITION_PASS", "NO_BAND_COMPACT", "NO_PROBE_OUTER_JOIN", "NO_STREAM_JOIN", "PARTITION_ROWS", "PARTITION_SLOTS",
-                "NO_SEMI_LDS", "NO_BAND_PAIR_COUNTS", "BAND_PAIR_COUNT_BLOCKS", "NO_BAND_ROW_CACHE", "NO_BAND_PAIR_LIST", "NO_BAND_PAIR_CACHE", "BAND_PAIR_CACHE_BLOCKS", "NO_AGG_LDS"]
+                "NO_SEMI_LDS", "NO_BAND_PAIR_COUNTS", "BAND_PAIR_COUNT_BLOCKS", "NO_EARLY_RESULT_COUNT", "NO_BAND_ROW_CACHE", "NO_BAND_PAIR_LIST", "NO_BAND_PAIR_CACHE", "BAND_PAIR_CACHE_BLOCKS", "NO_AGG_LDS"]
 OPTIONS = {name: i for i, name in enumerate(OPTION_NAMES)}
 
 
@@ -171,6 +171,7 @@
     "rdfgpu_plan_pushdown_filters", "rdfgpu_plan_set_dynamic_filters", "rdfgpu_plan_source_predicate",
     "rdfgpu_store_set_option", "rdfgpu_store_get_option", "rdfgpu_plan_set_option", "rdfgpu_option_name",
     "rdfgpu_scan_score", "rdfgpu_choose_index", "rdfgpu_predicate_and", "rdfgpu_band_row_cache_eligible", "rdfgpu_band_pair_cache_eligible", "rdfgpu_band_pair_list_eligible", "rdfgpu_band_pair_count_eligible", "rdfgpu_band_step_form", "rdfgpu_oj_probe_form",
+    "rdfgpu_early_count_eligible", "rdfgpu_plan_tail_pending",
     "rdfgpu_pushdown_to_scan_predicate", "rdfgpu_regex_check",
     "rdfgpu_comm_unique_id", "rdfgpu_comm_create", "rdfgpu_comm_create_host", "rdfgpu_comm_destroy",
     "rdfgpu_exchange_allgatherv", "rdfgpu_exchange_repartition", "rdfgpu_shard_of",
diff --git a/rdf-fusion_amd/csrc/abi.cpp b/rdf-fusion_amd/csrc/abi.cpp
--- a/rdf-fusion_amd/csrc/abi.cpp
+++ b/rdf-fusion_amd/csrc/abi.cpp
@@ -157,10 +157,17 @@
   if (n_cols) *n_cols = p->result.n_cols;
   ABI_END
 }
+int rdfgpu_plan_tail_pending(rdfgpu_plan* plan, uint32_t* out) {
+  ABI_BEGIN
+  if (!out) fail(RDFGPU_ERR_INVALID, "null out pointer");
+  *out = P(plan)->tail_pending ? 1u : 0u;
+  ABI_END
+}
 int rdfgpu_plan_result_device(rdfgpu_plan* plan, const uint32_t** cols, uint32_t cap_cols) {
   ABI_BEGIN
   Plan* p = P(plan);
   if (!p->executed) fail(RDFGPU_ERR_INVALID, "plan has not been executed");
+  p->complete();
   if (cap_cols < p->result.n_cols) fail(RDFGPU_ERR_INVALID, "room for %u columns, result has %u", cap_cols, p->result.n_cols);
   for (u32 c = 0; c < p->result.n_cols; c++) cols[c] = p->result_rows ? p->result.cols[c] : nullptr;
   ABI_END
@@ -169,6 +176,7 @@
   ABI_BEGIN
   Plan* p = P(plan);
   if (!p->executed) fail(RDFGPU_ERR_INVALID, "plan has not been executed");
+  p->complete();
   if (n_cols != p->result.n_cols) fail(RDFGPU_ERR_INVALID, "caller passed %u columns, result has %u", n_cols, p->result.n_cols);
   p->store->activate();
   for (u32 c = 0; c < n_cols; c++)
@@ -188,6 +196,7 @@
   ABI_BEGIN
   Plan* p = P(plan);
   if (!p->executed) fail(RDFGPU_ERR_INVALID, "plan has not been executed");
+  p->complete();
   if (agg >= p->agg_out.size()) fail(RDFGPU_ERR_INVALID, "aggregate %u of %zu", agg, p->agg_out.size());
   p->store->activate();
   if (p->result_rows) {
@@ -201,6 +210,7 @@
   ABI_BEGIN
   Plan* p = P(plan);
   if (!p->executed) fail(RDFGPU_ERR_INVALID, "plan has not been executed");
+  p->complete();
   if (col >= p->result.n_cols) fail(RDFGPU_ERR_INVALID, "column %u of a %u-column result", col, p->result.n_cols);
   if (!values) fail(RDFGPU_ERR_INVALID, "null out pointer");
   *values = p->result_values(col, n);
@@ -210,6 +220,7 @@
   ABI_BEGIN
   Plan* p = P(plan);
   if (!p->executed) fail(RDFGPU_ERR_INVALID, "plan has not been executed");
+  p->complete();
   if (col >= p->result.n_cols) fail(RDFGPU_ERR_INVALID, "column %u of a %u-column result", col, p->result.n_cols);
   if (!p->result_values(col, nullptr)) fail(RDFGPU_ERR_INVALID, "result column %u holds object ids, not aggregate values", col);
   p->ensure_host_copy();
@@ -223,6 +234,7 @@
   ABI_BEGIN
   Plan* p = P(plan);
   if (!p->executed) fail(RDFGPU_ERR_INVALID, "plan has not been executed");
+  p->complete();
   if (agg >= p->agg_out.size()) fail(RDFGPU_ERR_INVALID, "aggregate %u of %zu", agg, p->agg_out.size());
   if (!values) fail(RDFGPU_ERR_INVALID, "null out pointer");
   *values = p->result_rows ? p->agg_out[agg] : nullptr;
@@ -381,6 +393,7 @@
     Plan* p = P(plan);
     if (!out) fail(RDFGPU_ERR_INVALID, "null out array");
     if (!p->executed) fail(RDFGPU_ERR_INVALID, "plan has not been executed");
+    p->complete();
     if (col >= p->result.n_cols) fail(RDFGPU_ERR_INVALID, "column %u of a %u-column result", col, p->result.n_cols);
     if (const ValueOrigin& o = p->nodes[p->root].origin[col]; o.node >= 0)
       fail(RDFGPU_ERR_UNSUPPORTED, "ENC_PT of result column %u: it is %s value column (%s %u of node %d), its entries are not object ids (rdfgpu_plan_result_values)", col, o.mark ? "a mark" : o.extend ? "a computed" : "an aggregate", o.mark ? "mark" : o.extend ? "expression" : "aggregate", o.agg, o.node);
@@ -471,10 +484,11 @@
   } catch (const Error& e) { set_last_error(e.what()); return e.status; }
   catch (const std::exception& e) { set_last_error(e.what()); return RDFGPU_ERR_INVALID; }
 }
-int rdfgpu_plan_rewind(rdfgpu_plan* plan) { ABI_BEGIN P(plan)->cursor = 0; ABI_END }
+int rdfgpu_plan_rewind(rdfgpu_plan* plan) { ABI_BEGIN P(plan)->complete(); P(plan)->cursor = 0; ABI_END }
 int rdfgpu_plan_metrics(rdfgpu_plan* plan, rdfgpu_metrics* out) {
   ABI_BEGIN
   if (!out) fail(RDFGPU_ERR_INVALID, "null out pointer");
+  P(plan)->complete();
   *out = P(plan)->metrics;
   ABI_END
 }
@@ -528,6 +542,7 @@
 int rdfgpu_plan_kernel_stats(rdfgpu_plan* plan, rdfgpu_kernel_stat* out, uint32_t cap, uint32_t* n) {
   ABI_BEGIN
   Plan* p = P(plan);
+  p->complete();
   if (!n || (cap && !out)) fail(RDFGPU_ERR_INVALID, "null out pointer");
   u32 w = 0;
   for (int k = 0; k < KC__N; k++) {
@@ -599,6 +614,13 @@
   OjProbeShape s;
   s.held = held != 0; s.in_place = in_place != 0; s.row_cache = row_cache != 0; s.option_off = option_set == 0; s.row_static = row_static != 0;
   return (int)oj_probe_form(s);
+}
+int rdfgpu_early_count_eligible(uint32_t is_root, uint32_t result_is_output, uint32_t form, uint32_t skip_slow, uint32_t speculative, uint32_t priming, uint32_t timing, uint32_t option_set) {
+  if (form > (uint32_t)BandForm::COUNTS_LIST) { set_last_error("early count: unknown band form"); return RDFGPU_ERR_INVALID; }
+  EarlyCountShape s;
+  s.is_root = is_root != 0; s.result_is_output = result_is_output != 0; s.form = (BandForm)form; s.skip_slow = skip_slow != 0;
+  s.speculative = speculative != 0; s.priming = priming != 0; s.timing = timing != 0; s.option_off = option_set == 0;
+  return early_count_eligible(s) ? 1 : 0;
 }
 static ScanPredicate from_abi(const rdfgpu_predicate* p) {
   ScanPredicate r; r.kind = p->pred; r.from = p->from; r.to = p->to; r.equal_to = p->equal_to;
diff --git a/rdf-fusion_amd/csrc/band_join.hip b/rdf-fusion_amd/csrc/band_join.hip
--- a/rdf-fusion_amd/csrc/band_join.hip
+++ b/rdf-fusion_amd/csrc/band_join.hip
@@ -919,6 +919,14 @@
   if (!launched) fail(RDFGPU_ERR_INVALID, "band join: form %s with %u output columns (%u from the row)", band_form_name(form), b.n_out_cols, b.n_row_cols);
 }
 
+__global__ __launch_bounds__(256) void band_count_point_kernel(const u64* counters, const u32* total, u64* mirror) {
+  mirror[threadIdx.x] = counters[threadIdx.x];
+  if (threadIdx.x == 0) mirror[256] = *total;
+}
+void launch_band_count_point(const u64* counters, const u32* total, u64* mirror, hipStream_t s) {
+  hipLaunchKernelGGL(band_count_point_kernel, dim3(1), dim3(256), 0, s, counters, total, mirror);
+}
+
 struct BandBlocksOfKey {
   const u32* csr_off; const u32* poff; u32 kn;
   __host__ __device__ u32 operator()(u32 k) const {
diff --git a/rdf-fusion_amd/csrc/host_logic.cpp b/rdf-fusion_amd/csrc/host_logic.cpp
--- a/rdf-fusion_amd/csrc/host_logic.cpp
+++ b/rdf-fusion_amd/csrc/host_logic.cpp
@@ -182,4 +182,9 @@
   return s.row_static ? OjProbeForm::LEAN : OjProbeForm::FULL_NOW;
 }
 
+bool early_count_eligible(const EarlyCountShape& s) {
+  if (!s.is_root || !s.result_is_output || !s.skip_slow || !s.speculative || s.priming || s.timing || !s.option_off) return false;
+  return s.form == BandForm::VERDICTS_LIST || s.form == BandForm::COUNTS_LIST;
 }
+
+}
diff --git a/rdf-fusion_amd/csrc/host_logic.hpp b/rdf-fusion_amd/csrc/host_logic.hpp
--- a/rdf-fusion_amd/csrc/host_logic.hpp
+++ b/rdf-fusion_amd/csrc/host_logic.hpp
@@ -67,4 +67,7 @@
 struct OjProbeShape { bool held = false, in_place = false, row_cache = false, option_off = false, row_static = false; };
 OjProbeForm oj_probe_form(const OjProbeShape& s);
 
+struct EarlyCountShape { bool is_root = false, result_is_output = false, skip_slow = false, speculative = false, priming = false, timing = false, option_off = false; BandForm form = BandForm::RECORDS; };
+bool early_count_eligible(const EarlyCountShape& s);
+
 }
diff --git a/rdf-fusion_amd/csrc/kernels.hpp b/rdf-fusion_amd/csrc/kernels.hpp
--- a/rdf-fusion_amd/csrc/kernels.hpp
+++ b/rdf-fusion_amd/csrc/kernels.hpp
@@ -480,6 +480,7 @@
 void launch_band_mask(const BandArgs& b, BandForm form, hipStream_t s);
 void launch_band_slow(const LdsJoinArgs* a_dev, const BandArgs& b, hipStream_t s);
 void launch_band_emit(const BandArgs& b, BandForm form, hipStream_t s);
+void launch_band_count_point(const u64* counters , const u32* total, u64* mirror , hipStream_t s);
 size_t sort_u32_temp_bytes(u64 n, u32 bits);
 void sort_pairs_u32_u32(const u32* kin, u32* kout, const u32* vin, u32* vout, u64 n, u32 bits, void* temp, size_t temp_bytes, hipStream_t s);
 void launch_val_minmax(const long long* val, u64 n, long long* out_minmax , hipStream_t s);
diff --git a/rdf-fusion_amd/csrc/plan.cpp b/rdf-fusion_amd/csrc/plan.cpp
--- a/rdf-fusion_amd/csrc/plan.cpp
+++ b/rdf-fusion_amd/csrc/plan.cpp
@@ -99,7 +99,9 @@
 
 Plan::~Plan() {
   if (store) (void)hipSetDevice(store->device);
+  try { complete(); } catch (...) {}
   if (stream) (void)hipStreamSynchronize(stream);
+  if (store) { store->tails.remove(this); tail_waited(); }
   release_intermediates();
   if (pool_dev) (void)hipFree(pool_dev);
   if (regex_dev) (void)hipFree(regex_dev);
@@ -184,6 +186,22 @@
   for (void* p : allocs) store->pool.free(p);
   allocs.clear();
 }
+void Plan::tail_waited() {
+  retired.release([&](void* p) { store->pool.free(p); });
+  retired_held.reset();
+}
+void Plan::complete() {
+  if (!tail_pending) return;
+  store->activate();
+  RDFGPU_HIP(hipStreamSynchronize(stream));
+  tail_pending = false;
+  store->tails.remove(this);
+  tail_waited();
+  float ms = 0;
+  if (executed && hipEventElapsedTime(&ms, ctx->event(0), ctx->event(1)) == hipSuccess) metrics.elapsed_compute_ms = ms;
+  else (void)hipGetLastError();
+  resolve_timing();
+}
 const ExprProgram* Plan::upload_program(const ExprProgram& p) {
   if (progs_used >= ExecContext::kProgSlots) fail(RDFGPU_ERR_UNSUPPORTED, "plan needs more than %u device expression programs", ExecContext::kProgSlots);
   const u32 slot = progs_used++;
@@ -270,8 +288,23 @@
   if (!primed && !priming) prime();
   store->activate();
   std::shared_lock<std::shared_mutex> lock(store->mu);
-  RDFGPU_HIP(hipStreamSynchronize(stream));
-  release_intermediates();
+  struct TailGuard {
+    Plan* p; bool done = false;
+    ~TailGuard() {
+      if (done || !p->tail_pending) return;
+      (void)hipStreamSynchronize(p->stream);
+      p->tail_pending = false; p->store->tails.remove(p); p->tail_waited();
+    }
+  } tail_guard{this};
+  const bool behind_tail = tail_pending;
+  if (behind_tail) {
+    for (void* p : allocs) retired.retire(p, store->pool.block_bytes(p));
+    allocs.clear();
+    retired_held = held;
+  } else {
+    RDFGPU_HIP(hipStreamSynchronize(stream));
+    release_intermediates();
+  }
   store->pool.trim_to(2 * std::max(std::max(scratch_hist[0], scratch_hist[1]), std::max(store->scratch_recent[0].load(), store->scratch_recent[1].load())) + (1ull << 30));
   held = store->gen;
   metrics = rdfgpu_metrics{};
@@ -290,6 +323,7 @@
   RDFGPU_HIP(hipMemsetAsync(counters, 0, 256 * sizeof(u64), stream));
 
   spec_checks.clear();
+  count_point = CountPoint{};
   pending_oj.active = false;
   band_feedback.clear();
   memo.assign(nodes.size(), DevTable{}); memo_valid.assign(nodes.size(), 0);
@@ -300,11 +334,23 @@
 
   result = exec_node(root);
   flush_pending_oj();
-  RDFGPU_HIP(hipMemcpyAsync(ctx->counters_host, counters, 256 * sizeof(u64), hipMemcpyDeviceToHost, stream));
+  const bool early = count_point.armed && result.n_dev == count_point.n_out_dev && !pending_oj.active;
+  if (!early) RDFGPU_HIP(hipMemcpyAsync(ctx->counters_host, counters, 256 * sizeof(u64), hipMemcpyDeviceToHost, stream));
   RDFGPU_HIP(hipEventRecord(ev_stop, stream));
-  RDFGPU_HIP(hipStreamSynchronize(stream)); metrics.host_syncs++;
+  if (early) RDFGPU_HIP(hipEventSynchronize(ctx->count_event)); else RDFGPU_HIP(hipStreamSynchronize(stream));
+  metrics.host_syncs++;
   RDFGPU_HIP(hipGetLastError());
+  if (behind_tail) tail_waited();
+  if (early) {
+    const u64 total = ctx->counters_host[256];
+    ctx->counters_host[count_point.n_out] = total;
+    if (total > count_point.out_cap) ctx->counters_host[count_point.overflow] |= 1ull;
+    tail_pending = true;
+    store->tails.add(this, ev_stop);
+  } else if (behind_tail) { tail_pending = false; store->tails.remove(this); }
+  auto settle = [&] { if (early) complete(); };
   if (const u32 rt = (u32)(ctx->counters_host[255] & 0xFFFFFFFFull)) {
+    settle();
     if (rt & 1u) fail(RDFGPU_ERR_UNSUPPORTED, "REGEX with \\d \\w \\s or \\b over a string with non-ASCII characters needs the regex crate's Unicode tables (not restated)");
     if (rt & 8u) fail(RDFGPU_ERR_UNSUPPORTED, "a numeric CAST met a simple literal: the lexical forms of numbers are not parsed on the device");
     if (rt & kRtExtendKind) fail(RDFGPU_ERR_UNSUPPORTED, "a computed column (ProjectionExec with expressions) met a value that is a string, IRI, blank node, dateTime, date, time or duration: "
@@ -324,6 +370,8 @@
     else { c.node->last_rows = ctx->counters_host[c.counter]; c.node->has_last = true; c.node->last_scaled = false; }
   }
   if (spec_failed) {
+    settle();
+    tail_guard.done = true;
     metrics.host_syncs++;
     lock.unlock();
     allow_speculation = false;
@@ -337,7 +385,7 @@
   for (NodeInfo& nd : nodes)
     if (nd.values_run == run && nd.n_values_dev) { nd.n_values = std::min<u64>(nd.n_values, ctx->counters_host[nd.n_values_dev - counters]); nd.n_values_dev = nullptr; }
   float ms = 0;
-  RDFGPU_HIP(hipEventElapsedTime(&ms, ev_start, ev_stop));
+  if (!early) RDFGPU_HIP(hipEventElapsedTime(&ms, ev_start, ev_stop));
   metrics.elapsed_compute_ms = ms;
   metrics.output_rows = result_rows;
   metrics.device_mallocs = (u32)(store->pool.mallocs() + store->table_pool.mallocs() - mallocs0);
@@ -346,6 +394,7 @@
   executed = true;
   scratch_hist[1] = scratch_hist[0]; scratch_hist[0] = metrics.device_bytes;
   store->scratch_recent[1] = store->scratch_recent[0].load(); store->scratch_recent[0] = metrics.device_bytes;
+  tail_guard.done = true;
 }
 
 void Plan::refresh_dynamic_sources(std::shared_lock<std::shared_mutex>& lock) {
@@ -607,6 +656,7 @@
 void Plan::ensure_host_copy() {
   if (host_valid) return;
   if (!executed) fail(RDFGPU_ERR_INVALID, "plan has not been executed");
+  complete();
   store->activate();
   host_cols.assign(result.n_cols, std::vector<u32>());
   for (u32 c = 0; c < result.n_cols; c++) {
diff --git a/rdf-fusion_amd/csrc/plan.hpp b/rdf-fusion_amd/csrc/plan.hpp
--- a/rdf-fusion_amd/csrc/plan.hpp
+++ b/rdf-fusion_amd/csrc/plan.hpp
@@ -103,6 +103,7 @@
   std::vector<ColRef> chain_cols; SliceTable::ValueColumn chain_vc[kMaxChain] = {};
   BandArgs band{}; bool use_band = false;
   DevTable t;
+  const NodeInfo* out_node = nullptr;
   LdsJoin(NodeInfo& n, const DevTable& l, const DevTable& r, bool bl, const NodeInfo* pf, const NodeInfo* post)
       : nd(n), L(l), R(r), build_left(bl), B(bl ? l : r), P(bl ? r : l), probe_filter(pf), post_filter(post),
         probe_outer(n.d.join_type == RDFGPU_JOIN_LEFT && !bl), left_join(n.d.join_type == RDFGPU_JOIN_LEFT && bl) {}
@@ -218,6 +219,12 @@
   std::vector<BoundTable> tables;
 
   std::vector<void*> allocs;
+  struct CountPoint { bool armed = false; const u64* n_out_dev = nullptr; u32 n_out = 0, overflow = 0; u64 out_cap = 0; };
+  CountPoint count_point;
+  bool tail_pending = false;
+  RetiredBlocks retired; std::shared_ptr<IndexGeneration> retired_held;
+  void complete();
+  void tail_waited();
   u64* counters = nullptr;
   u32 counters_used = 0;
   u32 progs_used = 0;
diff --git a/rdf-fusion_amd/csrc/plan_band.cpp b/rdf-fusion_amd/csrc/plan_band.cpp
--- a/rdf-fusion_amd/csrc/plan_band.cpp
+++ b/rdf-fusion_amd/csrc/plan_band.cpp
@@ -534,6 +534,17 @@
     timed(KC_BAND_SLOW, 0, 0, nullptr, 0, nullptr, 0, 0, [&] { launch_band_slow(a_dev, b, stream); });
   }
   timed(scan_class(max_blocks + 1), 0, max_blocks + 1, nullptr, 8, nullptr, 0, 0, [&] { exclusive_scan_u32(b.bcount, b.bofs, max_blocks + 1, temp, tb, stream); });
+  const NodeInfo* top = &nodes[root];
+  while (top->d.kind == RDFGPU_NODE_PROJECTION) top = &nodes[top->d.left];
+  EarlyCountShape early;
+  early.is_root = bj.j.out_node == top; early.result_is_output = !bj.j.left_join && !pending_oj.active; early.skip_slow = bj.skip_slow; early.form = bj.form;
+  early.speculative = speculative; early.priming = priming; early.timing = timing; early.option_off = !opt.on(RDFGPU_OPT_NO_EARLY_RESULT_COUNT);
+  if (early_count_eligible(early)) {
+    launch_band_count_point(counters, b.bofs + max_blocks, ctx->counters_host_dev, stream);
+    RDFGPU_HIP(hipEventRecord(ctx->count_event, stream));
+    count_point.armed = true; count_point.n_out_dev = b.n_out_dev; count_point.n_out = (u32)(b.n_out_dev - counters);
+    count_point.overflow = (u32)(reinterpret_cast<u64*>(b.overflow) - counters); count_point.out_cap = b.out_cap;
+  }
   timed(KC_BAND_EMIT, bytes.emit_fixed, bj.nrows, nrows_dev, 4 + 4ull * b.n_row_cols, a.n_out_dev, 0, 4ull * a.n_out_cols, [&] { launch_band_emit(b, bj.form, stream); });
 }
 
diff --git a/rdf-fusion_amd/csrc/plan_exec.hpp b/rdf-fusion_amd/csrc/plan_exec.hpp
--- a/rdf-fusion_amd/csrc/plan_exec.hpp
+++ b/rdf-fusion_amd/csrc/plan_exec.hpp
@@ -53,7 +53,15 @@
 }
 
 template <class T> T* Plan::scratch(u64 n) {
-  void* p = store->pool.alloc((n ? n : 1) * sizeof(T));
+  const size_t bytes = (n ? n : 1) * sizeof(T);
+  void* p = nullptr;
+  if (!retired.empty()) {
+    const size_t b = DevicePool::bucket(bytes);
+    p = retired.take_exact(b);
+    if (!p) p = store->pool.alloc_exact(bytes);
+    if (!p) p = retired.take(b);
+  }
+  if (!p) p = store->pool.alloc(bytes);
   allocs.push_back(p);
   metrics.device_bytes += (n ? n : 1) * sizeof(T);
   return (T*)p;
diff --git a/rdf-fusion_amd/csrc/plan_join.cpp b/rdf-fusion_amd/csrc/plan_join.cpp
--- a/rdf-fusion_amd/csrc/plan_join.cpp
+++ b/rdf-fusion_amd/csrc/plan_join.cpp
@@ -622,6 +622,7 @@
   a.out_cap = spec_cap;
   for (u32 c = 0; c < a.n_out_cols; c++) { a.out[c] = scratch<u32>(spec_cap + j.tail); t.cols[c] = a.out[c]; }
   if (j.left_join) RDFGPU_HIP(hipMemsetAsync(a.visited, 0, j.L.cap, stream));
+  j.out_node = &size_node;
   if (j.use_band) exec_band_join(j);
   else if (!run_ordered_join(j, size_node, spec_cap)) run_join_kernel(j, j.stage_bytes, 4ull * a.n_out_cols);
   const SpecCheck check{&size_node, (u32)(a.n_out_dev - counters), j.left_join};
diff --git a/rdf-fusion_amd/csrc/store.cpp b/rdf-fusion_amd/csrc/store.cpp
--- a/rdf-fusion_amd/csrc/store.cpp
+++ b/rdf-fusion_amd/csrc/store.cpp
@@ -63,6 +63,22 @@
   in_use_ += got;
   return p;
 }
+size_t DevicePool::bucket(size_t bytes) { return bucket_of(bytes ? bytes : 1); }
+size_t DevicePool::block_bytes(void* p) {
+  std::lock_guard<std::mutex> g(mu_);
+  auto it = live_.find(p);
+  return it == live_.end() ? 0 : it->second;
+}
+void* DevicePool::alloc_exact(size_t bytes) {
+  const size_t b = bucket_of(bytes ? bytes : 1);
+  std::lock_guard<std::mutex> g(mu_);
+  auto it = free_.find(b);
+  if (it == free_.end()) return nullptr;
+  void* p = it->second.p;
+  free_.erase(it); cached_ -= b;
+  live_[p] = b; in_use_ += b;
+  return p;
+}
 void DevicePool::free(void* p) {
   if (!p) return;
   std::lock_guard<std::mutex> g(mu_);
@@ -97,7 +113,7 @@
     "NO_TABLE_CACHE", "NO_INDEX_JOIN", "NO_CHAIN_FUSION", "NO_VALUE_TABLES", "NO_RANGE_INDEX", "NO_FILTER_FUSION",
     "NO_LDS_JOIN", "NO_GLOBAL_TABLE_JOIN", "NO_DIRECT_TABLE", "NO_BAND_JOIN", "NO_PARTITIONED_JOIN", "NO_VALUE_VERDICTS", "NO_PRIMING", "NO_ORDERED_JOIN", "NO_BAND_PACK16", "NO_RUN_COPY", "NO_RANGE_PARTITION",
     "LDS_MAX_BUILD", "CSR_ROW_LANES_LOG2", "JOIN_WAVE_Q", "PARTITION_MIN_BUILD", "PARTITION_TWO_PASS_ROWS", "NO_OWN_PARTITION_PASS", "NO_BAND_COMPACT", "NO_PROBE_OUTER_JOIN", "NO_STREAM_JOIN", "PARTITION_ROWS", "PARTITION_SLOTS",
-    "NO_SEMI_LDS", "NO_BAND_PAIR_COUNTS", "BAND_PAIR_COUNT_BLOCKS", "NO_BAND_ROW_CACHE", "NO_BAND_PAIR_LIST", "NO_BAND_PAIR_CACHE", "BAND_PAIR_CACHE_BLOCKS", "NO_AGG_LDS"};
+    "NO_SEMI_LDS", "NO_BAND_PAIR_COUNTS", "BAND_PAIR_COUNT_BLOCKS", "NO_EARLY_RESULT_COUNT", "NO_BAND_ROW_CACHE", "NO_BAND_PAIR_LIST", "NO_BAND_PAIR_CACHE", "BAND_PAIR_CACHE_BLOCKS", "NO_AGG_LDS"};
 const char* engine_option_name(u32 option) { return option < RDFGPU_OPT__COUNT ? kOptionNames[option] : nullptr; }
 const EngineOptions& default_engine_options() {
   static const EngineOptions defaults = [] {
@@ -179,6 +195,7 @@
 }
 ExecContext::~ExecContext() {
   for (hipEvent_t e : events) (void)hipEventDestroy(e);
+  if (count_event) (void)hipEventDestroy(count_event);
   if (counters) (void)hipFree(counters);
   if (counters_host) (void)hipHostFree(counters_host);
   if (progs_dev) (void)hipFree(progs_dev);
@@ -202,7 +219,9 @@
     c = new ExecContext();
     RDFGPU_HIP(hipStreamCreateWithFlags(&c->stream, hipStreamNonBlocking));
     RDFGPU_HIP(hipMalloc((void**)&c->counters, 256 * sizeof(u64)));
-    RDFGPU_HIP(hipHostMalloc((void**)&c->counters_host, 256 * sizeof(u64), hipHostMallocDefault));
+    RDFGPU_HIP(hipHostMalloc((void**)&c->counters_host, ExecContext::kMirrorWords * sizeof(u64), hipHostMallocDefault));
+    RDFGPU_HIP(hipHostGetDevicePointer((void**)&c->counters_host_dev, c->counters_host, 0));
+    RDFGPU_HIP(hipEventCreate(&c->count_event));
     RDFGPU_HIP(hipMalloc((void**)&c->progs_dev, ExecContext::kProgSlots * sizeof(ExprProgram)));
     RDFGPU_HIP(hipHostMalloc((void**)&c->progs_host, ExecContext::kProgSlots * sizeof(ExprProgram), hipHostMallocDefault));
     RDFGPU_HIP(hipMalloc((void**)&c->args_dev, (size_t)ExecContext::kArgSlots * ExecContext::kArgBytes));
@@ -251,6 +270,7 @@
 void Store::drop_tables() {
   std::unique_lock<std::shared_mutex> lock(mu);
   activate();
+  wait_for_tails();
   RDFGPU_HIP(hipDeviceSynchronize());
   version++;
   drop_slice_tables();
@@ -262,8 +282,15 @@
   string_verdicts.clear();
 }
 
+void Store::wait_for_tails() {
+  hipError_t first = hipSuccess;
+  tails.wait_all([&](void* ev) { const hipError_t e = hipEventSynchronize(static_cast<hipEvent_t>(ev)); if (first == hipSuccess) first = e; });
+  RDFGPU_HIP(first);
+}
+
 Store::~Store() {
   (void)hipSetDevice(device);
+  tails.wait_all([](void* ev) { (void)hipEventSynchronize(static_cast<hipEvent_t>(ev)); });
   drop_slice_tables();
   drop_string_verdicts();
   for (ExecContext* c : free_ctx) delete c;
@@ -289,6 +316,7 @@
 void Store::clear() {
   std::unique_lock<std::shared_mutex> lock(mu);
   activate();
+  wait_for_tails();
   auto fresh = std::make_shared<IndexGeneration>();
   fresh->device = device;
   adopt(fresh);
@@ -331,6 +359,7 @@
 u64 Store::extend_device(const u32* g, const u32* s_, const u32* p, const u32* o, u64 n) {
   std::unique_lock<std::shared_mutex> lock(mu);
   activate();
+  wait_for_tails();
   if (n == 0) return 0;
   const u32* in[4] = {g, s_, p, o};
   hipStream_t s = stream;
@@ -389,6 +418,7 @@
 u64 Store::remove_host(const u32* g, const u32* s_, const u32* p, const u32* o, u64 n) {
   std::unique_lock<std::shared_mutex> lock(mu);
   activate();
+  wait_for_tails();
   if (n == 0 || idx[0].n == 0) return 0;
   hipStream_t s = stream;
   const u32* h[4] = {g, s_, p, o};
@@ -420,6 +450,7 @@
 u64 Store::remove_graph(u32 graph) {
   std::unique_lock<std::shared_mutex> lock(mu);
   activate();
+  wait_for_tails();
   if (idx[0].n == 0) return 0;
   hipStream_t s = stream;
   u64 removed = 0;
@@ -442,6 +473,7 @@
 void Store::set_typed_values(const rdfgpu_typed_value* v, u64 n, const int64_t* d, u64 nd) {
   std::unique_lock<std::shared_mutex> lock(mu);
   activate();
+  wait_for_tails();
   drop_string_verdicts();
   drop_slice_tables();
   if (tv) { RDFGPU_HIP(hipFree(tv)); tv = nullptr; }
@@ -460,6 +492,7 @@
 void Store::set_strings(const u64* offsets, u64 n, const unsigned char* heap_host, u64 heap_bytes) {
   std::unique_lock<std::shared_mutex> lock(mu);
   activate();
+  wait_for_tails();
   drop_string_verdicts();
   if (n && !offsets) fail(RDFGPU_ERR_INVALID, "set_strings: null offsets");
   for (u64 i = 0; i < n; i++) if (offsets[i] > offsets[i + 1] || offsets[i + 1] > heap_bytes) fail(RDFGPU_ERR_INVALID, "set_strings: offsets of id %llu are not monotone / inside the heap", (unsigned long long)i);
diff --git a/rdf-fusion_amd/csrc/store.hpp b/rdf-fusion_amd/csrc/store.hpp
--- a/rdf-fusion_amd/csrc/store.hpp
+++ b/rdf-fusion_amd/csrc/store.hpp
@@ -9,6 +9,7 @@
 
 #include "common.hpp"
 #include "expr_device.hpp"
+#include "tail_lifetime.hpp"
 
 namespace rdfgpu {
 
@@ -17,7 +18,10 @@
   DevicePool();
   ~DevicePool();
   void* alloc(size_t bytes);
+  void* alloc_exact(size_t bytes);
   void free(void* p);
+  static size_t bucket(size_t bytes);
+  size_t block_bytes(void* p);
   void trim();
   void trim_to(u64 keep_bytes);
   u64 bytes_in_use() const { return in_use_; }
@@ -39,7 +43,10 @@
   hipStream_t stream = nullptr;
   std::vector<hipEvent_t> events;
   u64* counters = nullptr;
+  static constexpr u32 kMirrorWords = 257;
   u64* counters_host = nullptr;
+  u64* counters_host_dev = nullptr;
+  hipEvent_t count_event = nullptr;
   void* jobs_dev = nullptr; u64* lohi_dev = nullptr; u32 job_cap = 0;
   void* jobs_host = nullptr; u64* lohi_host = nullptr;
   static constexpr u32 kProgSlots = 16;
@@ -115,6 +122,8 @@
   void table_free(void* p) { table_pool.free(p); }
   hipStream_t stream = nullptr;
   std::shared_mutex mu;
+  TailRegistry tails;
+  void wait_for_tails();
   std::atomic<int> refs{1};
   void retain() { refs.fetch_add(1); }
   void release() { if (refs.fetch_sub(1) == 1) delete this; }
diff --git a/rdf-fusion_amd/csrc/tail_lifetime.hpp b/rdf-fusion_amd/csrc/tail_lifetime.hpp
--- /dev/null
+++ b/rdf-fusion_amd/csrc/tail_lifetime.hpp
@@ -0,0 +1,64 @@
+#pragma once
+#include <cstddef>
+#include <mutex>
+#include <vector>
+
+namespace rdfgpu {
+
+class RetiredBlocks {
+ public:
+  void retire(void* p, size_t bytes) { if (p) blocks_.push_back(Block{p, bytes}); }
+  void* take_exact(size_t bytes) {
+    for (size_t i = 0; i < blocks_.size(); i++) if (blocks_[i].bytes == bytes) return remove(i);
+    return nullptr;
+  }
+  void* take(size_t bytes) {
+    size_t best = blocks_.size();
+    for (size_t i = 0; i < blocks_.size(); i++) {
+      const size_t b = blocks_[i].bytes;
+      if (b < bytes || b > bytes + bytes / 2) continue;
+      if (best == blocks_.size() || b < blocks_[best].bytes) best = i;
+    }
+    return best == blocks_.size() ? nullptr : remove(best);
+  }
+  template <class Free> void release(Free&& free) {
+    std::vector<Block> gone;
+    gone.swap(blocks_);
+    for (const Block& b : gone) free(b.p);
+  }
+  bool empty() const { return blocks_.empty(); }
+  size_t size() const { return blocks_.size(); }
+
+ private:
+  struct Block { void* p; size_t bytes; };
+  void* remove(size_t i) { void* p = blocks_[i].p; blocks_[i] = blocks_.back(); blocks_.pop_back(); return p; }
+  std::vector<Block> blocks_;
+};
+
+class TailRegistry {
+ public:
+  void add(const void* owner, void* event) {
+    std::lock_guard<std::mutex> g(mu_);
+    for (Entry& e : tails_) if (e.owner == owner) { e.event = event; return; }
+    tails_.push_back(Entry{owner, event});
+  }
+  void remove(const void* owner) {
+    std::lock_guard<std::mutex> g(mu_);
+    for (size_t i = 0; i < tails_.size(); i++) if (tails_[i].owner == owner) { tails_[i] = tails_.back(); tails_.pop_back(); return; }
+  }
+  template <class Wait> void wait_all(Wait&& wait) {
+    std::lock_guard<std::mutex> g(mu_);
+    for (const Entry& e : tails_) wait(e.event);
+  }
+  size_t pending() {
+    std::lock_guard<std::mutex> g(mu_);
+    return tails_.size();
+  }
+
+ private:
+  struct Entry { const void* owner; void* event; };
+  std::mutex mu_;
+  std::vector<Entry> tails_;
+};
+
+}
diff --git a/rdf-fusion_amd/engine.py b/rdf-fusion_amd/engine.py
--- a/rdf-fusion_amd/engine.py
+++ b/rdf-fusion_amd/engine.py
@@ -116,6 +116,8 @@
     lib.rdfgpu_band_pair_count_eligible.argtypes = [C.c_uint32] * 2 + [C.c_uint64] * 2
     lib.rdfgpu_band_step_form.argtypes = [C.c_uint32] * 6 + [C.c_uint64] * 2
     lib.rdfgpu_oj_probe_form.argtypes = [C.c_uint32] * 5
+    lib.rdfgpu_early_count_eligible.argtypes = [C.c_uint32] * 8
+    lib.rdfgpu_plan_tail_pending.argtypes = [vp, u32p]
     lib.rdfgpu_predicate_and.argtypes = [C.POINTER(abi.Predicate), C.POINTER(abi.Predicate),
                                          C.POINTER(abi.Predicate), u32p]
     lib.rdfgpu_pushdown_to_scan_predicate.argtypes = [C.c_uint32, C.c_uint32, C.POINTER(abi.Predicate)]
@@ -183,6 +185,11 @@
 
 def oj_probe_form(held=True, in_place=True, row_cache=True, option_set=False, row_static=True):
     return OJ_PROBE_FORMS[_check(load_library().rdfgpu_oj_probe_form(int(held), int(in_place), int(row_cache), int(option_set), int(row_static)))]
+
+
+def early_count_eligible(form="COUNTS_LIST", is_root=True, result_is_output=True, skip_slow=True, speculative=True, priming=False, timing=False, option_set=False):
+    return bool(_check(load_library().rdfgpu_early_count_eligible(int(is_root), int(result_is_output), BAND_FORMS.index(form), int(skip_slow), int(speculative),
+                                                                   int(priming), int(timing), int(option_set))))
 
 
 def _pred_struct(p, keep):
@@ -490,6 +497,11 @@
         _check(self._lib.rdfgpu_plan_result_info(self._h, C.byref(n), C.byref(c)))
         return n.value, c.value
 
+    def tail_pending(self):
+        out = C.c_uint32()
+        _check(self._lib.rdfgpu_plan_tail_pending(self._h, C.byref(out)))
+        return out.value
+
     def result_device(self):
         n, c = self.result_info()
         ptrs = (C.c_void_p * max(1, c))()
```

Measured after the change: 158.5 billion bindings/s (median of 6 runs). 1.1x the previous value.
